# highfem/tqdne

Measured on AMD Instinct MI355X. Metric: waveforms/sec (train step + 18-step EDM sample), 3ch x 4096, higher is better.
Workload: dtype f32 (contractions on MFMA with fp32 accumulate: bf16x3, and fp16 + block-scaled-fp6 corrections on the 128/256-channel forward convs; sampler state f64)

## Files before the change

include/tqdne_hip.h:

```cpp
#ifndef TQDNE_HIP_H
#define TQDNE_HIP_H

#include <stddef.h>
#include <stdint.h>

#ifdef __cplusplus
extern "C" {
#endif

#ifndef __HIP__
typedef struct ihipStream_t* hipStream_t;
#endif

#define TQ_ABI_VERSION 8

#define TQ_ERR_ARG (-1)
#define TQ_ERR_SHAPE (-2)

#define TQ_CONV_GN 1
#define TQ_CONV_SILU 2
#define TQ_CONV_EMB 4
#define TQ_CONV_RES 8
#define TQ_CONV_STATS 16
#define TQ_CONV_DROPOUT 32
#define TQ_CONV_POLY2 64
#define TQ_CONV_CH_TILES 128
#define TQ_CONV_WIDE_TABLE 256

#define TQ_WFMT_BF16X3 0
#define TQ_WFMT_F16_MX8 1
#define TQ_WFMT_F16_MX6 2

typedef struct TqGnFold {
    const float* stats0;
    const float* stats1;
    int32_t slot0, slot1;
    const float* gamma;
    const float* beta;
    float* mean_rstd;
} TqGnFold;

typedef struct TqConvDesc {
    int32_t B, T_in, T_out;
    int32_t C_in0, C_in1;
    int32_t C_out;
    int32_t ktaps, stride, pad;
    int32_t upsample;
    int32_t flags;
    int32_t emb_stride;
    uint32_t dropout_site;
    float dropout_p;
    uint64_t dropout_seed;
    int32_t C_skip0, C_skip1;
    int32_t wfmt;
    int32_t* range_flag;
    const void* reserved1;
    int32_t t_tile;
    int32_t reserved2;
    const TqGnFold* gn_fold;
} TqConvDesc;

#define TQ_BWD_GN 1
#define TQ_BWD_SILU 2
#define TQ_BWD_DROPOUT 4
#define TQ_BWD_ACCUM 8
#define TQ_BWD_STATS 16

typedef struct TqConvBwdDesc {
    int32_t B, T;
    int32_t C_dy;
    int32_t C_dx0, C_dx1;
    int32_t ktaps;
    int32_t flags;
    uint32_t dropout_site;
    float dropout_p;
    uint64_t dropout_seed;
    int32_t wfmt;
    int32_t reserved;
    const uint32_t* dy_amax;
} TqConvBwdDesc;

int tq_abi_version(void);
int tq_build_flags(void);

size_t tq_conv_weight_pack_bytes(int C_out, int C_in, int K, int mode);
int tq_pack_conv_weight(const float* w, int C_out, int C_in, int K, int mode, void* packed, hipStream_t stream);
int tq_conv_tile_co(int C_out);
int tq_conv1d_max_cin(int wfmt, int C_out);
int tq_conv1d_max_cout(void);
size_t tq_conv1d_wide_lds_bytes(int ktaps, int t_tile, int C_out);
int tq_conv1d_gn_table_entries(int wide);
int tq_conv1d_gn_fold_max_cin(int wfmt, int t_tile, int C_out);
int tq_colsum_max_channels(void);
typedef struct TqPackJob {
    const void* src;
    void* dst;
    int32_t C_out, C_in, K, mode;
    int32_t block_begin;
    int32_t reserved;
} TqPackJob;
int tq_pack_job_blocks(int C_out, int C_in, int K, int mode);
int tq_pack_jobs(const TqPackJob* jobs_device, int njobs, int total_blocks, hipStream_t stream);

int tq_conv1d_fwd(const TqConvDesc* desc, const float* x0, const float* x1, const float* gscale, const float* gshift,
                  const void* packed_w, const float* bias, const float* emb, const float* residual, float* y,
                  float* stats_partial, hipStream_t stream);

int tq_conv1d_fwd_skip(const TqConvDesc* desc, const float* x0, const float* x1, const float* gscale, const float* gshift,
                       const void* packed_w_main_then_skip, const float* bias, const float* emb, const float* skip_x0,
                       const float* skip_x1, const float* skip_bias, float* y, float* stats_partial, hipStream_t stream);

#define TQ_KV_V_BF16 0
#define TQ_KV_V_F16 1
int tq_conv1d_fwd_qkv(const TqConvDesc* desc, const float* x, const float* gscale, const float* gshift, const void* packed_w,
                      const float* bias, float* qkv, void* kv_planes, int H, int D, int v_format, hipStream_t stream);

int tq_conv1d_bwd_data(const TqConvBwdDesc* desc, const float* dy, const void* packed_w_t, const float* x0, const float* x1,
                       const float* gscale, const float* gshift, float* dx0, float* dx1, float* gstats_partial,
                       hipStream_t stream);

size_t tq_conv1d_bwd_weight_workspace(const TqConvDesc* desc);
int tq_conv1d_bwd_weight(const TqConvDesc* desc, const float* dy, const float* x0, const float* x1, const float* gscale,
                         const float* gshift, float* dw, void* workspace, size_t ws_bytes, hipStream_t stream);
int tq_conv1d_bwd_weight_colsum(const TqConvDesc* desc, const float* dy, const float* x0, const float* x1, const float* gscale,
                                const float* gshift, float* dw, void* workspace, size_t ws_bytes, float* colsum_bc, int bc_stride,
                                float* colsum_c, float* colsum_c2, hipStream_t stream);

size_t tq_stem_conv_lds_bytes(int C_in, int C_out, int ktaps);
int tq_stem_conv_fwd(const float* x_nct, const float* in_scale, const float* w, const float* bias, float* y,
                     float* stats_partial, int B, int C_in, int T, int C_out, int ktaps, hipStream_t stream);

size_t tq_head_conv_lds_bytes(int C_in, int C_out, int ktaps);
int tq_head_conv_fwd(const float* x, const float* gscale, const float* gshift, const float* w, const float* bias,
                     const float* c_out, const float* c_skip, const float* skip_src, float* y_nct, int B, int T, int C_in,
                     int C_out, int ktaps, hipStream_t stream);

int tq_gn_finalize(const float* stats0, int C0, const float* stats1, int C1, int B, int T, const float* gamma,
                   const float* beta, float* gscale, float* gshift, float* mean_rstd, int slot0, int slot1, hipStream_t stream);

int tq_gn_bwd_finalize(const float* gstats_partial, const float* mean_rstd, const float* gamma, int B, int C, int T,
                       float* coef_a, float* coef_b, float* coef_c, float* dgamma, float* dbeta, hipStream_t stream);
int tq_gn_bwd_apply(const float* g, const float* x, const float* r, const float* coef_a, const float* coef_b,
                    const float* coef_c, float* dx, int B, int T, int C_src, int C_total, int c_offset, int accumulate,
                    hipStream_t stream);
int tq_gn_bwd_apply_colsum(const float* g, const float* x, const float* r, const float* coef_a, const float* coef_b,
                           const float* coef_c, float* dx, int B, int T, int C_src, int C_total, int c_offset, int accumulate,
                           float* colsum_bc, int bc_stride, float* colsum_c, float* colsum_c2, uint32_t* amax_out,
                           hipStream_t stream);
typedef struct TqGemmJob {
    const float* A;
    const float* B;
    float* C;
    const float* U;
    int32_t M, N, K;
    int32_t sam, sak, sbk, sbn, ldc, ldu;
    int32_t pre_b;
    int32_t tile_begin;
} TqGemmJob;
int tq_gemm_tiles(int M, int N);
int tq_gemm_f32_jobs(const TqGemmJob* jobs_device, int njobs, int total_tiles, hipStream_t stream);
int tq_fourier_features(const float* t, const float* W, float* out, int B, int half, hipStream_t stream);

#define TQ_AMAX_WAYS 16
#define TQ_AMAX_STRIDE 32
#define TQ_AMAX_WORDS (TQ_AMAX_WAYS * TQ_AMAX_STRIDE)
int tq_colsum(const float* dy, int B, int T, int C, float* out_bc, int bc_stride, float* out_c, float* out_c2,
              const float* bscale, uint32_t* amax_out, hipStream_t stream);
int tq_zero_stuff(const float* dy, float* out, int B, int T_out, int T_in, int C, hipStream_t stream);
int tq_pair_sum(const float* d_up, float* dx, int B, int T, int C, int accumulate, hipStream_t stream);
int tq_upsample_poly_wgrad_fold(const float* dw2, float* dw, int C_out, int C_in, hipStream_t stream);
int tq_stem_conv_bwd_weight(const float* dy, const float* x_nct, const float* in_scale, float* dw, int B, int C_in, int T,
                            int C_out, int ktaps, hipStream_t stream);
size_t tq_stem_head_bwd_workspace(void);
int tq_stem_conv_bwd_weight_ws(const float* dy, const float* x_nct, const float* in_scale, float* dw, int B, int C_in, int T,
                               int C_out, int ktaps, void* workspace, size_t ws_bytes, hipStream_t stream);
int tq_head_conv_bwd_ws(const float* dpred_nct, const float* c_out, const float* x, const float* gscale, const float* gshift,
                        const float* w, float* g_out, float* gstats_partial, float* dw, float* db, int B, int T, int C_in,
                        int C_out, int ktaps, void* workspace, size_t ws_bytes, hipStream_t stream);
size_t tq_head_conv_bwd_lds_bytes(int C_in, int C_out, int ktaps);
int tq_head_conv_bwd(const float* dpred_nct, const float* c_out, const float* x, const float* gscale, const float* gshift,
                     const float* w, float* g_out, float* gstats_partial, float* dw, float* db, int B, int T, int C_in,
                     int C_out, int ktaps, hipStream_t stream);

int tq_embed_fwd(const float* t, const float* cond, const float* fourier_w, const float* w0, const float* b0,
                 const float* w2, const float* b2, const float* cw0, const float* cb0, const float* cw2, const float* cb2,
                 float* emb, float* silu_emb, float* hidden ,
                 int B, int mc, int ncond, hipStream_t stream);

int tq_linear_fwd(const float* x, const float* w, const float* bias, float* out, int B, int E, int N, hipStream_t stream);

size_t tq_attention_workspace_bytes(int B, int T, int H, int D);
int tq_attention_fwd(const float* qkv, float* out, float* lse ,
                     void* workspace , int B, int T,
                     int H, int D, hipStream_t stream);
int tq_attention_fwd_presplit(const float* qkv, const void* kv_planes, float* out, int B, int T, int H, int D, int v_format,
                              hipStream_t stream);
int tq_attention_bwd(const float* qkv, const float* out, const float* dout, const float* lse, float* delta, float* dqkv, int B,
                     int T, int H, int D, hipStream_t stream);
int tq_attention_bwd_ws(const float* qkv, const float* out, const float* dout, const float* lse, float* delta, float* dqkv,
                        void* workspace, int B, int T, int H, int D, hipStream_t stream);
int tq_attention_bwd_ws_kv(const float* qkv, const float* out, const float* dout, const float* lse, float* delta, float* dqkv,
                           void* workspace, const void* kv_planes, int B, int T, int H, int D, hipStream_t stream);

int tq_attention_head_tile(int D);
size_t tq_attention_hd_lds_bytes(int D, int pass);
size_t tq_attention_hd_workspace_bytes(int B, int T, int H, int D);
int tq_attention_fwd_hd(const float* qkv, float* out, float* lse, void* workspace, int B, int T, int H, int D, hipStream_t stream);
int tq_attention_bwd_hd(const float* qkv, const float* out, const float* dout, const float* lse, float* delta, float* dqkv,
                        void* workspace, int B, int T, int H, int D, hipStream_t stream);

int tq_edm_scalars(const float* sigma, int sigma_stride, float sigma_data, float* c_in, float* c_out, float* c_skip,
                   float* c_noise, float* lweight, int B, hipStream_t stream);
int tq_cm_scalars(const float* sigma, int sigma_stride, float sigma_data, float sigma_min, float* c_out, float* c_skip,
                  int B, hipStream_t stream);
int tq_edm_noise_inject(const float* y, const float* unit_noise, const float* eps, float P_mean, float P_std,
                        float* sigma, float* x_noisy, int B, int n_per_sample, hipStream_t stream);
int tq_edm_loss(const float* pred, const float* y, const float* lweight, float* loss_out, float* dpred, int B,
                int n_per_sample, hipStream_t stream);
int tq_heun_euler(const double* x, const float* denoised, const float* sigma, const float* sigma_next, double* d_cur,
                  double* x_next, float* x32, size_t n, hipStream_t stream);
int tq_heun_correct(const double* x, const double* x_next, const float* denoised_next, const double* d_cur,
                    const float* sigma, const float* sigma_next, double* x_out, float* x32, size_t n, hipStream_t stream);
int tq_sampler_init(const double* unit_noise, const float* sigma0, double* x, float* x32, size_t n, hipStream_t stream);

int tq_heun_churn(const double* x, const double* unit_noise, const float* coef, double s_noise, double* x_hat, float* x32,
                  size_t n, hipStream_t stream);

int tq_axpy_sigma(const float* x, const float* noise, const float* sigma, float* out, int B, int n_per_sample,
                  hipStream_t stream);

int tq_scale_add2(const float* x, const float* y, const float* a, const float* c, float* out, int B, int n_per_sample,
// ... 51 lines not shown
```

tqdne_amd/_lib.py:

```python

from __future__ import annotations

import ctypes as C
import os
from typing import Optional

from . import _build

_LIB = None

c_f32p = C.c_void_p
VP = C.c_void_p
I = C.c_int
F = C.c_float
SZ = C.c_size_t

TQ_CONV_GN, TQ_CONV_SILU, TQ_CONV_EMB, TQ_CONV_RES, TQ_CONV_STATS, TQ_CONV_DROPOUT = 1, 2, 4, 8, 16, 32
TQ_CONV_POLY2 = 64
TQ_CONV_CH_TILES = 128
TQ_CONV_WIDE_TABLE = 256
TQ_WFMT_BF16X3, TQ_WFMT_F16_MX8, TQ_WFMT_F16_MX6 = 0, 1, 2
TQ_KV_V_BF16, TQ_KV_V_F16 = 0, 1
PACK_MODE = {TQ_WFMT_BF16X3: 0, TQ_WFMT_F16_MX8: 2, TQ_WFMT_F16_MX6: 3}
PACK_MODE_T = {TQ_WFMT_BF16X3: 1, TQ_WFMT_F16_MX6: 5}
# ... 22 lines not shown
WIDE_MX6 = os.environ.get("TQDNE_WIDE_MX6", "1") != "0"


def conv_max_cin(wfmt: int, C_out: int = 0) -> int:
    return load().tq_conv1d_max_cin(wfmt, C_out)


def forward_wfmt(C_out: int, sources, stride: int = 1, upsample: bool = False, k5_act: bool = False,
                 gn: Optional[bool] = None) -> int:
    v = requested_scheme()
    co_ok = C_out % 128 == 0 or (C_out % 64 == 0 and k5_act and not upsample and v == "f16mx6" and MX6_C64)
    ok = stride == 1 and co_ok and all(c % 64 == 0 for c in sources if c)
    if not ok or v == "bf16x3":
        return TQ_WFMT_BF16X3
    fmt = TQ_WFMT_F16_MX6 if v == "f16mx6" else TQ_WFMT_F16_MX8
    cin = sum(c for c in list(sources)[:2] if c)
    if gn is None or gn:
        if cin > conv_max_cin(fmt, C_out) or (cin > load().tq_conv1d_gn_table_entries(0) and not WIDE_MX6):
            return TQ_WFMT_BF16X3
    return fmt
TQ_BWD_GN, TQ_BWD_SILU, TQ_BWD_DROPOUT, TQ_BWD_ACCUM, TQ_BWD_STATS = 1, 2, 4, 8, 16
STAT_SLOT = 128
TQ_AMAX_WAYS, TQ_AMAX_STRIDE = 16, 32
TQ_AMAX_WORDS = TQ_AMAX_WAYS * TQ_AMAX_STRIDE


class TqGnFold(C.Structure):
    _fields_ = [("stats0", C.c_void_p), ("stats1", C.c_void_p), ("slot0", C.c_int32), ("slot1", C.c_int32),
                ("gamma", C.c_void_p), ("beta", C.c_void_p), ("mean_rstd", C.c_void_p)]


class TqConvDesc(C.Structure):
    _fields_ = [
        ("B", C.c_int32), ("T_in", C.c_int32), ("T_out", C.c_int32),
        ("C_in0", C.c_int32), ("C_in1", C.c_int32), ("C_out", C.c_int32),
        ("ktaps", C.c_int32), ("stride", C.c_int32), ("pad", C.c_int32),
        ("upsample", C.c_int32), ("flags", C.c_int32), ("emb_stride", C.c_int32),
        ("dropout_site", C.c_uint32), ("dropout_p", C.c_float), ("dropout_seed", C.c_uint64),
        ("C_skip0", C.c_int32), ("C_skip1", C.c_int32), ("wfmt", C.c_int32),
        ("range_flag", C.c_void_p), ("reserved1", C.c_void_p), ("t_tile", C.c_int32), ("reserved2", C.c_int32),
        ("gn_fold", C.POINTER(TqGnFold)),
    ]


class TqAdamChunk(C.Structure):
    _fields_ = [("p", C.c_void_p), ("g", C.c_void_p), ("m", C.c_void_p), ("v", C.c_void_p), ("ema", C.c_void_p),
                ("n", C.c_int32), ("reserved", C.c_int32)]


TQ_ADAM_CHUNK = 4096


class TqGemmJob(C.Structure):
    _fields_ = [("A", C.c_void_p), ("B", C.c_void_p), ("C", C.c_void_p), ("U", C.c_void_p),
                ("M", C.c_int32), ("N", C.c_int32), ("K", C.c_int32),
                ("sam", C.c_int32), ("sak", C.c_int32), ("sbk", C.c_int32), ("sbn", C.c_int32), ("ldc", C.c_int32), ("ldu", C.c_int32),
                ("pre_b", C.c_int32), ("tile_begin", C.c_int32)]


class TqPackJob(C.Structure):
    _fields_ = [("src", C.c_void_p), ("dst", C.c_void_p), ("C_out", C.c_int32), ("C_in", C.c_int32), ("K", C.c_int32),
                ("mode", C.c_int32), ("block_begin", C.c_int32), ("reserved", C.c_int32)]


class TqConvBwdDesc(C.Structure):
    _fields_ = [
        ("B", C.c_int32), ("T", C.c_int32), ("C_dy", C.c_int32), ("C_dx0", C.c_int32), ("C_dx1", C.c_int32),
        ("ktaps", C.c_int32), ("flags", C.c_int32), ("dropout_site", C.c_uint32), ("dropout_p", C.c_float),
        ("dropout_seed", C.c_uint64), ("wfmt", C.c_int32), ("reserved", C.c_int32), ("dy_amax", C.c_void_p),
    ]


_PROTOS = {
    "tq_abi_version": (I, []),
    "tq_build_flags": (I, []),
    "tq_conv_weight_pack_bytes": (SZ, [I, I, I, I]),
    "tq_pack_conv_weight": (I, [VP, I, I, I, I, VP, VP]),
    "tq_conv_tile_co": (I, [I]),
    "tq_conv1d_max_cin": (I, [I, I]),
    "tq_conv1d_max_cout": (I, []),
    "tq_conv1d_gn_table_entries": (I, [I]),
    "tq_conv1d_wide_lds_bytes": (SZ, [I, I, I]),
    "tq_conv1d_gn_fold_max_cin": (I, [I, I, I]),
    "tq_colsum_max_channels": (I, []),
    "tq_conv1d_fwd": (I, [C.POINTER(TqConvDesc)] + [VP] * 11),
    "tq_conv1d_fwd_skip": (I, [C.POINTER(TqConvDesc)] + [VP] * 13),
    "tq_stem_conv_fwd": (I, [VP] * 6 + [I] * 5 + [VP]),
    "tq_head_conv_fwd": (I, [VP] * 9 + [I] * 5 + [VP]),
    "tq_head_conv_lds_bytes": (SZ, [I, I, I]),
    "tq_stem_conv_lds_bytes": (SZ, [I, I, I]),
    "tq_head_conv_bwd_lds_bytes": (SZ, [I, I, I]),
    "tq_gn_finalize": (I, [VP, I, VP, I, I, I, VP, VP, VP, VP, VP, I, I, VP]),
    "tq_embed_fwd": (I, [VP] * 14 + [I, I, I, VP]),
    "tq_linear_fwd": (I, [VP] * 4 + [I, I, I, VP]),
    "tq_attention_fwd": (I, [VP, VP, VP, VP, I, I, I, I, VP]),
    "tq_attention_fwd_presplit": (I, [VP, VP, VP, I, I, I, I, I, VP]),
    "tq_conv1d_fwd_qkv": (I, [C.POINTER(TqConvDesc)] + [VP] * 7 + [I, I, I, VP]),
    "tq_attention_workspace_bytes": (SZ, [I, I, I, I]),
    "tq_attention_bwd": (I, [VP] * 6 + [I, I, I, I, VP]),
    "tq_attention_bwd_ws": (I, [VP] * 7 + [I, I, I, I, VP]),
    "tq_attention_bwd_ws_kv": (I, [VP] * 8 + [I, I, I, I, VP]),
    "tq_attention_head_tile": (I, [I]),
    "tq_attention_hd_lds_bytes": (SZ, [I, I]),
    "tq_attention_hd_workspace_bytes": (SZ, [I, I, I, I]),
    "tq_attention_fwd_hd": (I, [VP, VP, VP, VP, I, I, I, I, VP]),
    "tq_attention_bwd_hd": (I, [VP] * 7 + [I, I, I, I, VP]),
    "tq_edm_scalars": (I, [VP, I, F, VP, VP, VP, VP, VP, I, VP]),
    "tq_cm_scalars": (I, [VP, I, F, F, VP, VP, I, VP]),
    "tq_edm_noise_inject": (I, [VP, VP, VP, F, F, VP, VP, I, I, VP]),
    "tq_edm_loss": (I, [VP, VP, VP, VP, VP, I, I, VP]),
    "tq_heun_euler": (I, [VP] * 7 + [SZ, VP]),
    "tq_heun_correct": (I, [VP] * 8 + [SZ, VP]),
    "tq_sampler_init": (I, [VP] * 4 + [SZ, VP]),
    "tq_heun_churn": (I, [VP, VP, VP, C.c_double, VP, VP, SZ, VP]),
    "tq_axpy_sigma": (I, [VP, VP, VP, VP, I, I, VP]),
    "tq_pseudo_huber_loss": (I, [VP, VP, VP, F, VP, VP, I, I, VP]),
    "tq_mse_loss": (I, [VP, VP, VP, VP, SZ, VP]),
    "tq_scale_add2": (I, [VP, VP, VP, VP, VP, I, I, VP]),
    "tq_ddpm_step": (I, [VP, VP, VP, VP, SZ, I] + [C.c_double] * 6 + [VP]),
    "tq_vae_reparam_fwd": (I, [VP, VP, VP, VP, I, I, I, VP]),
    "tq_vae_reparam_bwd": (I, [VP, VP, VP, VP, F, I, I, I, VP]),
    "tq_concat_scale": (I, [VP, VP, VP, VP, I, I, I, I, VP]),
    "tq_envelope_fwd": (I, [VP, VP, I, I, I, I, C.c_double, C.c_double, VP]),
    "tq_envelope_inv": (I, [VP, VP, I, I, I, C.c_double, C.c_double, VP]),
    "tq_adam_ema_step": (I, [VP, I] + [C.c_double] * 8 + [VP]),
    "tq_adam_ema_step_guarded": (I, [VP, I] + [C.c_double] * 8 + [VP, VP]),
    "tq_conv1d_bwd_data": (I, [VP] * 11),
    "tq_conv1d_bwd_weight_workspace": (SZ, [VP]),
    "tq_conv1d_bwd_weight": (I, [VP] * 8 + [SZ, VP]),
    "tq_conv1d_bwd_weight_colsum": (I, [VP] * 8 + [SZ, VP, I, VP, VP, VP]),
    "tq_gn_bwd_finalize": (I, [VP, VP, VP, I, I, I, VP, VP, VP, VP, VP, VP]),
    "tq_gn_bwd_apply": (I, [VP] * 7 + [I] * 6 + [VP]),
    "tq_gn_bwd_apply_colsum": (I, [VP] * 7 + [I] * 6 + [VP, I, VP, VP, VP, VP]),
    "tq_pack_job_blocks": (I, [I, I, I, I]),
    "tq_pack_jobs": (I, [VP, I, I, VP]),
    "tq_gemm_tiles": (I, [I, I]),
    "tq_gemm_f32_jobs": (I, [VP, I, I, VP]),
    "tq_fourier_features": (I, [VP, VP, VP, I, I, VP]),
    "tq_colsum": (I, [VP, I, I, I, VP, I, VP, VP, VP, VP, VP]),
    "tq_zero_stuff": (I, [VP, VP, I, I, I, I, VP]),
    "tq_pair_sum": (I, [VP, VP, I, I, I, I, VP]),
    "tq_upsample_poly_wgrad_fold": (I, [VP, VP, I, I, VP]),
    "tq_stem_conv_bwd_weight": (I, [VP] * 4 + [I] * 5 + [VP]),
    "tq_head_conv_bwd": (I, [VP] * 10 + [I] * 5 + [VP]),
    "tq_stem_head_bwd_workspace": (SZ, []),
    "tq_stem_conv_bwd_weight_ws": (I, [VP] * 4 + [I] * 5 + [VP, SZ, VP]),
    "tq_head_conv_bwd_ws": (I, [VP] * 10 + [I] * 5 + [VP, SZ, VP]),
    "tq_boundary_max_channels": (I, []),
    "tq_nct_to_btc": (I, [VP] * 4 + [I] * 5 + [VP]),
    "tq_btc_to_nct": (I, [VP] * 5 + [I] * 5 + [VP]),
    "tq_avg_pool2_fwd": (I, [VP, VP, VP, I, I, I, VP]),
    "tq_nearest_up2_fwd": (I, [VP, VP, VP, I, I, I, VP]),
    "tq_avg_pool2_bwd": (I, [VP, VP, I, I, I, I, VP]),
}

def lib_path() -> str:
    return os.environ.get("TQDNE_HIP_LIB", _build.LIBPATH)


def load():
    global _LIB
    if _LIB is not None:
        return _LIB
    path = lib_path()
    if not os.path.exists(path):
        raise RuntimeError(
            f"{path} is missing: the tqdne_amd hot path is HIP-only (no CPU / PyTorch fallback). "
            "Build it with `python -m tqdne_amd._build` (needs hipcc, cross-compiles gfx950 without a GPU)."
        )
    lib = C.CDLL(path)
    for name, (res, args) in _PROTOS.items():
        fn = getattr(lib, name)
        fn.restype = res
        fn.argtypes = args
    if lib.tq_abi_version() != ABI_VERSION:
        raise RuntimeError("libtqdne_hip.so ABI version mismatch")
    _LIB = lib
    return lib


def exported_symbols():
    return sorted(_PROTOS)


class TqError(RuntimeError):
    pass


def check(rc: int, what: str = ""):
    if rc != 0:
        kind = {-1: "TQ_ERR_ARG", -2: "TQ_ERR_SHAPE"}.get(rc, f"hipError_t {rc}")
        raise TqError(f"libtqdne_hip: {what} failed with {kind}")
```

tqdne_amd/csrc/backward.hip:

```cpp
#include <cstdlib>
#include "common.hpp"
#include "ends_wide.hpp"
#include "../../include/tqdne_hip.h"

using namespace tq;

namespace {

typedef short s16x4 __attribute__((ext_vector_type(4)));

__device__ __forceinline__ uint2 lds_tr_read(const unsigned char* p) {
    s16x4 v = __builtin_amdgcn_ds_read_tr16_b64_v4i16((__attribute__((address_space(3))) s16x4*)(p));
    union { s16x4 s; uint2 u; } c;
    c.s = v;
    return c.u;
}

struct WgArgs {
    const float* dy;
    const float* x0;
    const float* x1;
    const float* gscale;
    const float* gshift;
    float* slab;
    int B, T_in, T_out, C0, C1, C_out;
    int flags, nsplit, units_per_split, n_ttiles, n_cotiles, n_cichunks;
    uint32_t drop_site, drop_thresh;
    float drop_scale;
    uint64_t drop_seed;
    float* cs_bc;
    int cs_stride;
    float* cs_c;
    float* cs_c2;
};

constexpr int WG_TT = 64;
constexpr int TQ_WGRAD_PLAIN_ORDER = 1 << 30;
constexpr int WG_DY_STRIDE1 = 288;
constexpr int WG_DY_STRIDE2 = 272;
template <int NCI> __device__ __forceinline__ int wg_dy_swz(int row) { return (NCI == 1 || NCI == 4) ? ((row >> 3) & 1) << 7 : 0; }
__device__ __forceinline__ int wg_x_swz(int row) { return ((row >> 3) & 1) << 5; }
__device__ __forceinline__ int wg_x_swz128(int row) { return (((row >> 1) & 1) << 5) | (((row >> 3) & 1) << 6); }
__device__ __forceinline__ int wg_x_swz256(int row) { return ((row & 3) << 5) | (((row >> 3) & 1) << 7); }

template <int KT, int STRIDE, int UPS, int NCI, bool W8 = false, bool H64 = false>
__global__ __launch_bounds__((W8 && !H64) ? 512 : 256, (W8 && !H64) ? 1 : 2) void wgrad_kernel(const WgArgs p) {
    static_assert(!W8 || NCI == 1, "W8: per-wave accumulators of a 32-channel chunk");
    static_assert(!H64 || W8, "H64: the W8 layout (two 32-channel halves of one xhat tile) with two output-channel blocks");
    constexpr int NT = (W8 && !H64) ? 512 : 256;
    constexpr int COT = H64 ? 64 : 128;
    constexpr int DYC4 = COT / 4;
    constexpr int NCX = W8 ? 2 : NCI;
    constexpr int PAD = (STRIDE == 1) ? KT / 2 : 1;
    constexpr int XR = (STRIDE == 1) ? (WG_TT + KT - 1) : (2 * WG_TT + 1);
    constexpr int WG_X_STRIDE = 64 * NCX;
    constexpr int XC4 = 8 * NCX;
    constexpr int XIT = (XR * XC4 + NT - 1) / NT;
    constexpr int DYIT = WG_TT * DYC4 / NT;
    static_assert(NCI != 4 || (KT == 1 && STRIDE == 1 && !UPS), "128-channel chunks: the 1x1 convs");
    constexpr int WG_DY_STRIDE = (NCI == 1 || NCI == 4) ? WG_DY_STRIDE1 : WG_DY_STRIDE2;
    constexpr int DY_PLANE = WG_TT * WG_DY_STRIDE;
    constexpr int X_PLANE = XR * WG_X_STRIDE;
    extern __shared__ __attribute__((aligned(16))) unsigned char lds[];
    unsigned char* dy_hi = lds;
    unsigned char* dy_lo = dy_hi + DY_PLANE;
    unsigned char* x_hi = dy_lo + DY_PLANE;
    unsigned char* x_lo = x_hi + X_PLANE;

    const int tid = threadIdx.x, lane = tid & 63;
    const int wave_id = __builtin_amdgcn_readfirstlane(tid >> 6);
    const int wave = H64 ? (wave_id & 1) : (W8 ? (wave_id & 3) : wave_id);
    const int wci = H64 ? (wave_id >> 1) : (W8 ? (wave_id >> 2) : 0);
    int ct, cc, sp;
    {
        const int bid = blockIdx.x;
        const int npairs = p.nsplit * p.n_cotiles;
        if ((npairs & 7) == 0 && !(p.flags & TQ_WGRAD_PLAIN_ORDER)) {
            const int xcd = bid & 7, j = bid >> 3;
            const int pi = (j / p.n_cichunks) * 8 + xcd;
            cc = j % p.n_cichunks;
            sp = pi / p.n_cotiles;
            ct = pi % p.n_cotiles;
        } else {
            ct = bid % p.n_cotiles;
// ... 433 lines not shown
    } else {
        hipLaunchKernelGGL((wgrad_kernel<KT, STRIDE, UPS, 1, false>), dim3(grid), dim3(256), sh, stream, a);
    }
    TQ_CHECK_LAUNCH();
    return 0;
}
}

extern "C" size_t tq_conv1d_bwd_weight_workspace(const TqConvDesc* d) {
    if (!d) return 0;
    int a, b, c, nsplit, nsplit4, ups;
    wgrad_plan(d, true, a, b, c, nsplit, ups);
    wgrad_plan(d, false, a, b, c, nsplit4, ups);
    return (size_t)(nsplit > nsplit4 ? nsplit : nsplit4) * d->ktaps * d->C_out * (d->C_in0 + d->C_in1) * sizeof(float);
}

extern "C" int tq_conv1d_bwd_weight(const TqConvDesc* d, const float* dy, const float* x0, const float* x1,
                                    const float* gscale, const float* gshift, float* dw, void* workspace, size_t ws_bytes,
                                    hipStream_t stream) {
    return tq_conv1d_bwd_weight_colsum(d, dy, x0, x1, gscale, gshift, dw, workspace, ws_bytes, nullptr, 0, nullptr, nullptr, stream);
}

extern "C" int tq_conv1d_bwd_weight_colsum(const TqConvDesc* d, const float* dy, const float* x0, const float* x1,
                                           const float* gscale, const float* gshift, float* dw, void* workspace, size_t ws_bytes,
                                           float* colsum_bc, int bc_stride, float* colsum_c, float* colsum_c2,
                                           hipStream_t stream) {
    if (!d || !dy || !x0 || !dw || !workspace) return TQ_ERR_ARG;
    if (colsum_c2 && !colsum_c) return TQ_ERR_ARG;
    if (d->C_in0 <= 0 || d->C_in0 % 32 || d->C_in1 < 0 || d->C_in1 % 32 || d->C_out <= 0 || d->C_out % 32) return TQ_ERR_SHAPE;
    if (d->C_in1 > 0 && !x1) return TQ_ERR_ARG;
    if ((d->flags & TQ_CONV_GN) && (!gscale || !gshift)) return TQ_ERR_ARG;
    if (ws_bytes < tq_conv1d_bwd_weight_workspace(d)) return TQ_ERR_ARG;
    WgArgs a;
    a.dy = dy; a.x0 = x0; a.x1 = x1; a.gscale = gscale; a.gshift = gshift; a.slab = reinterpret_cast<float*>(workspace);
    a.B = d->B; a.T_in = d->T_in; a.T_out = d->T_out; a.C0 = d->C_in0; a.C1 = d->C_in1; a.C_out = d->C_out;
    a.flags = d->flags;
    a.cs_bc = colsum_bc; a.cs_stride = bc_stride; a.cs_c = colsum_c; a.cs_c2 = colsum_c2;
    const bool wide = !(colsum_bc || colsum_c);
    wgrad_plan(d, wide, a.n_cotiles, a.n_cichunks, a.n_ttiles, a.nsplit, a.units_per_split);
    static const bool plain_order = [] { const char* e = getenv("TQDNE_WGRAD_XCD"); return e && atoi(e) == 0; }();
    if (plain_order) a.flags |= TQ_WGRAD_PLAIN_ORDER;
    a.drop_site = d->dropout_site; a.drop_seed = d->dropout_seed;
    float pdrop = d->dropout_p;
    if (!(d->flags & TQ_CONV_DROPOUT) || pdrop <= 0.f) { a.flags &= ~TQ_CONV_DROPOUT; pdrop = 0.f; }
    a.drop_thresh = (uint32_t)((double)pdrop * 4294967296.0);
    a.drop_scale = 1.0f / (1.0f - pdrop);
    int rc;
    const int nci = wgrad_nci(d);
    const bool h64 = wide && wgrad_h64(d);
    const bool w8 = wide && !h64 && wgrad_w8(d);
    if (d->stride == 2) {
        if (d->ktaps != 3) return TQ_ERR_SHAPE;
        rc = launch_wgrad<3, 2, 0>(a, nci, w8, false, stream);
    } else if (d->upsample) {
        if (d->ktaps == 5) rc = launch_wgrad<5, 1, 1>(a, nci, w8, false, stream);
        else if (d->ktaps == 3) rc = launch_wgrad<3, 1, 1>(a, nci, w8, false, stream);
        else return TQ_ERR_SHAPE;
    } else {
        if (d->ktaps == 5) rc = launch_wgrad<5, 1, 0>(a, nci, w8, h64, stream);
        else if (d->ktaps == 3) rc = launch_wgrad<3, 1, 0>(a, nci, w8, h64, stream);
        else if (d->ktaps == 1) rc = launch_wgrad<1, 1, 0>(a, nci, false, false, stream);
        else return TQ_ERR_SHAPE;
    }
    if (rc) return rc;
    const size_t n = (size_t)d->C_out * (d->C_in0 + d->C_in1);
    const dim3 rgrid((unsigned)((n + 63) / 64)), rblock(16, 16);
    if (d->ktaps == 5) hipLaunchKernelGGL(wgrad_reduce_kernel<5>, rgrid, rblock, 0, stream, a.slab, dw, a.nsplit, n);
    else if (d->ktaps == 3) hipLaunchKernelGGL(wgrad_reduce_kernel<3>, rgrid, rblock, 0, stream, a.slab, dw, a.nsplit, n);
    else hipLaunchKernelGGL(wgrad_reduce_kernel<1>, rgrid, rblock, 0, stream, a.slab, dw, a.nsplit, n);
    TQ_CHECK_LAUNCH();
    return 0;
}

namespace {
__global__ __launch_bounds__(256) void gn_bwd_finalize_kernel(const float* __restrict__ gst, const float* __restrict__ mr,
                                                              const float* __restrict__ gamma, int C, int T, int nslots,
                                                              float* __restrict__ cA, float* __restrict__ cB,
                                                              float* __restrict__ cC, float* __restrict__ dgamma,
                                                              float* __restrict__ dbeta) {
    extern __shared__ double sh[];
    const int b = blockIdx.x;
    const int Cb = C / (int)gridDim.y;
    const int c0 = (int)blockIdx.y * Cb;
    int nsub = Cb <= 128 ? (int)blockDim.x / Cb : 1;
    if (nsub > nslots) nsub = nslots;
    double* cs = sh;
    double* gp = sh + 2 * Cb * nsub;
    for (int idx = threadIdx.x; idx < Cb * nsub; idx += blockDim.x) {
        const int c = idx % Cb, sub = idx / Cb;
        const float* pp = gst + ((size_t)b * nslots * C + c0 + c) * 2;
        double s1 = 0.0, s2 = 0.0;
        int s = sub;
        for (; s + 3 * nsub < nslots; s += 4 * nsub) {
            const float2 v0 = *reinterpret_cast<const float2*>(pp + (size_t)s * C * 2);
            const float2 v1 = *reinterpret_cast<const float2*>(pp + (size_t)(s + nsub) * C * 2);
            const float2 v2 = *reinterpret_cast<const float2*>(pp + (size_t)(s + 2 * nsub) * C * 2);
            const float2 v3 = *reinterpret_cast<const float2*>(pp + (size_t)(s + 3 * nsub) * C * 2);
            s1 += ((double)v0.x + (double)v1.x) + ((double)v2.x + (double)v3.x);
            s2 += ((double)v0.y + (double)v1.y) + ((double)v2.y + (double)v3.y);
        }
        for (; s < nslots; s += nsub) {
            const float2 v = *reinterpret_cast<const float2*>(pp + (size_t)s * C * 2);
            s1 += (double)v.x; s2 += (double)v.y;
        }
        cs[2 * idx] = s1; cs[2 * idx + 1] = s2;
    }
    __syncthreads();
    if (nsub > 1) {
        double t1 = 0.0, t2 = 0.0;
        const int c = threadIdx.x;
        if (c < Cb)
            for (int sub = 0; sub < nsub; ++sub) { t1 += cs[2 * (sub * Cb + c)]; t2 += cs[2 * (sub * Cb + c) + 1]; }
        __syncthreads();
        if (c < Cb) { cs[2 * c] = t1; cs[2 * c + 1] = t2; }
        __syncthreads();
    }
    const int G = C / GN_GROUPS;
    const int ngrp = Cb / G, g0 = c0 / G;
    if ((int)threadIdx.x < ngrp) {
        const int gl = threadIdx.x, g = g0 + gl;
        const double mean = (double)mr[((size_t)b * GN_GROUPS + g) * 2], rstd = (double)mr[((size_t)b * GN_GROUPS + g) * 2 + 1];
        double p1 = 0.0, p2 = 0.0;
        for (int j = 0; j < G; ++j) {
            const int cl = gl * G + j;
            const double gm = (double)gamma[c0 + cl];
            p1 += gm * cs[2 * cl];
            p2 += gm * (cs[2 * cl + 1] - mean * cs[2 * cl]);
        }
        p2 *= rstd;
        const double n = (double)G * (double)T;
        gp[2 * gl] = -rstd * rstd * p2 / n;
        gp[2 * gl + 1] = rstd * rstd * p2 * mean / n - rstd * p1 / n;
    }
    __syncthreads();
    for (int cl = threadIdx.x; cl < Cb; cl += blockDim.x) {
        const int c = c0 + cl;
        const int g = c / G, gl = g - g0;
        const float mean = mr[((size_t)b * GN_GROUPS + g) * 2], rstd = mr[((size_t)b * GN_GROUPS + g) * 2 + 1];
        cA[(size_t)b * C + c] = rstd * gamma[c];
        cB[(size_t)b * C + c] = (float)gp[2 * gl];
        cC[(size_t)b * C + c] = (float)gp[2 * gl + 1];
        atomicAdd(dgamma + c, (float)((double)rstd * (cs[2 * cl + 1] - (double)mean * cs[2 * cl])));
        atomicAdd(dbeta + c, (float)cs[2 * cl]);
    }
}

__global__ void gn_bwd_apply_kernel(const float* __restrict__ g, const float* __restrict__ x, const float* __restrict__ r,
                                    const float* __restrict__ cA, const float* __restrict__ cB, const float* __restrict__ cC,
                                    float* __restrict__ dx, int T, int Cs, int Ctot, int coff, int accum, size_t n4) {
    const int c4n = Cs >> 2;
    for (size_t i = (size_t)blockIdx.x * blockDim.x + threadIdx.x; i < n4; i += (size_t)gridDim.x * blockDim.x) {
        const int c4 = (int)(i % c4n);
        const size_t bt = i / c4n;
        const int b = (int)(bt / T);
        const size_t ko = (size_t)b * Ctot + coff + 4 * c4;
        const float4 a = *reinterpret_cast<const float4*>(cA + ko);
        const float4 bb = *reinterpret_cast<const float4*>(cB + ko);
        const float4 cc = *reinterpret_cast<const float4*>(cC + ko);
        const float4 gv = reinterpret_cast<const float4*>(g)[i];
        const float4 xv = reinterpret_cast<const float4*>(x)[i];
        float4 o = make_float4(a.x * gv.x + bb.x * xv.x + cc.x, a.y * gv.y + bb.y * xv.y + cc.y,
                               a.z * gv.z + bb.z * xv.z + cc.z, a.w * gv.w + bb.w * xv.w + cc.w);
        if (r) { const float4 rv = reinterpret_cast<const float4*>(r)[i]; o.x += rv.x; o.y += rv.y; o.z += rv.z; o.w += rv.w; }
        if (accum) { const float4 ov = reinterpret_cast<const float4*>(dx)[i]; o.x += ov.x; o.y += ov.y; o.z += ov.z; o.w += ov.w; }
        reinterpret_cast<float4*>(dx)[i] = o;
    }
}

constexpr int AMAX_WAYS = TQ_AMAX_WAYS;
constexpr int AMAX_STRIDE = TQ_AMAX_STRIDE;

template <int NT>
__device__ __forceinline__ void colsum_finish(float* red, const float4& a, float mx, bool active, int c4n, int nrow, int c4, int tr, int C,
                                              int b, float sc, float* __restrict__ out_bc, int bc_stride, float* __restrict__ out_c,
                                              float* __restrict__ out_c2, unsigned* __restrict__ amax_out) {
    if (active) *reinterpret_cast<float4*>(red + (tr * c4n + c4) * 4) = a;
    unsigned* wmax = reinterpret_cast<unsigned*>(red + (size_t)nrow * c4n * 4);
    if (amax_out) {
        unsigned m = __float_as_uint(mx);
#pragma unroll
        for (int o = 32; o > 0; o >>= 1) m = max(m, (unsigned)__shfl_xor((int)m, o));
        if ((threadIdx.x & 63) == 0) wmax[threadIdx.x >> 6] = m;
    }
    __syncthreads();
    if (amax_out && threadIdx.x == 0) {
        unsigned m = wmax[0];
#pragma unroll
        for (int w = 1; w < NT / 64; ++w) m = max(m, wmax[w]);
        if (m != 0u) atomicMax(amax_out + (blockIdx.x % AMAX_WAYS) * AMAX_STRIDE, m);
    }
    for (int c = threadIdx.x; c < C; c += NT) {
        float s = 0.f;
        for (int r2 = 0; r2 < nrow; ++r2) s += red[(r2 * c4n + (c >> 2)) * 4 + (c & 3)];
        s *= sc;
        if (out_bc) atomicAdd(out_bc + (size_t)b * bc_stride + c, s);
        if (out_c) atomicAdd(out_c + c, s);
        if (out_c2) atomicAdd(out_c2 + c, s);
    }
}
__device__ __forceinline__ float amax4(float m, const float4& v) {
    const float t = fmaxf(fmaxf(fabsf(v.x), fabsf(v.y)), fmaxf(fabsf(v.z), fabsf(v.w)));
    const bool bad = (v.x != v.x) | (v.y != v.y) | (v.z != v.z) | (v.w != v.w);
    return bad ? __builtin_inff() : fmaxf(m, t);
}

template <int NT>
__global__ __launch_bounds__(NT) void colsum_kernel(const float* __restrict__ dy, int T, int C, float* __restrict__ out_bc,
                                                     int bc_stride, float* __restrict__ out_c, float* __restrict__ out_c2,
                                                     const float* __restrict__ bscale, unsigned* __restrict__ amax_out, int rpw) {
    extern __shared__ float red[];
    const int nsl = (T + rpw - 1) / rpw;
    const int slot = blockIdx.x % nsl, b = blockIdx.x / nsl;
    const int c4n = C >> 2;
    const int nrow = NT / c4n > 0 ? NT / c4n : 1;
    const int c4 = threadIdx.x % c4n, tr = threadIdx.x / c4n;
    float4 a = make_float4(0.f, 0.f, 0.f, 0.f);
    float mx = 0.f;
    const bool active = tr < nrow && threadIdx.x < nrow * c4n;
    if (active) {
        const int nvalid = min(rpw, T - slot * rpw);
        const float* src = dy + ((size_t)b * T + (size_t)slot * rpw) * C + 4 * c4;
        int tl = tr;
        for (; tl + 7 * nrow < nvalid; tl += 8 * nrow) {
            float4 v[8];
#pragma unroll
            for (int q = 0; q < 8; ++q) v[q] = *reinterpret_cast<const float4*>(src + (size_t)(tl + q * nrow) * C);
#pragma unroll
            for (int q = 0; q < 8; ++q) { a.x += v[q].x; a.y += v[q].y; a.z += v[q].z; a.w += v[q].w; }
            if (amax_out) {
#pragma unroll
                for (int q = 0; q < 8; ++q) mx = amax4(mx, v[q]);
            }
        }
        for (; tl < nvalid; tl += nrow) {
            const float4 v = *reinterpret_cast<const float4*>(src + (size_t)tl * C);
            a.x += v.x; a.y += v.y; a.z += v.z; a.w += v.w;
            if (amax_out) mx = amax4(mx, v);
        }
    }
    colsum_finish<NT>(red, a, mx, active, c4n, nrow, c4, tr, C, b, bscale ? bscale[b] : 1.0f, out_bc, bc_stride, out_c, out_c2, amax_out);
}

template <int NT>
__global__ __launch_bounds__(NT) void gn_bwd_apply_cs_kernel(const float* __restrict__ g, const float* __restrict__ x,
                                                              const float* __restrict__ r, const float* __restrict__ cA,
                                                              const float* __restrict__ cB, const float* __restrict__ cC,
                                                              float* __restrict__ dx, int T, int Cs, int Ctot, int coff, int accum,
                                                              float* __restrict__ out_bc, int bc_stride, float* __restrict__ out_c,
                                                              float* __restrict__ out_c2, unsigned* __restrict__ amax_out, int rpw) {
    extern __shared__ float red[];
    const int nsl = (T + rpw - 1) / rpw;
    const int slot = blockIdx.x % nsl, b = blockIdx.x / nsl;
    const int c4n = Cs >> 2;
    const int nrow = NT / c4n > 0 ? NT / c4n : 1;
    const int c4 = threadIdx.x % c4n, tr = threadIdx.x / c4n;
    float4 a = make_float4(0.f, 0.f, 0.f, 0.f);
    float mx = 0.f;
    const bool active = tr < nrow && threadIdx.x < nrow * c4n;
    if (active) {
        const int nvalid = min(rpw, T - slot * rpw);
        const size_t ko = (size_t)b * Ctot + coff + 4 * c4;
        const float4 ka = *reinterpret_cast<const float4*>(cA + ko);
        const float4 kb = *reinterpret_cast<const float4*>(cB + ko);
        const float4 kc = *reinterpret_cast<const float4*>(cC + ko);
        const size_t base = ((size_t)b * T + (size_t)slot * rpw) * Cs + 4 * c4;
        auto one = [&](const float4& gv, const float4& xv, const float4& rv, const float4& ov) -> float4 __attribute__((always_inline)) {
            float4 o = make_float4(ka.x * gv.x + kb.x * xv.x + kc.x, ka.y * gv.y + kb.y * xv.y + kc.y,
                                   ka.z * gv.z + kb.z * xv.z + kc.z, ka.w * gv.w + kb.w * xv.w + kc.w);
            o.x += rv.x; o.y += rv.y; o.z += rv.z; o.w += rv.w;
            o.x += ov.x; o.y += ov.y; o.z += ov.z; o.w += ov.w;
            return o;
        };
        const float4 z4 = make_float4(0.f, 0.f, 0.f, 0.f);
        int tl = tr;
        for (; tl + 3 * nrow < nvalid; tl += 4 * nrow) {
            float4 gv[4], xv[4], rv[4], ov[4];
#pragma unroll
            for (int q = 0; q < 4; ++q) {
                const size_t o = base + (size_t)(tl + q * nrow) * Cs;
                gv[q] = *reinterpret_cast<const float4*>(g + o);
                xv[q] = *reinterpret_cast<const float4*>(x + o);
                rv[q] = r ? *reinterpret_cast<const float4*>(r + o) : z4;
                ov[q] = accum ? *reinterpret_cast<const float4*>(dx + o) : z4;
            }
#pragma unroll
            for (int q = 0; q < 4; ++q) {
                const float4 o4 = one(gv[q], xv[q], rv[q], ov[q]);
                *reinterpret_cast<float4*>(dx + base + (size_t)(tl + q * nrow) * Cs) = o4;
                a.x += o4.x; a.y += o4.y; a.z += o4.z; a.w += o4.w;
                mx = amax4(mx, o4);
            }
        }
        for (; tl < nvalid; tl += nrow) {
            const size_t o = base + (size_t)tl * Cs;
            const float4 o4 = one(*reinterpret_cast<const float4*>(g + o), *reinterpret_cast<const float4*>(x + o),
                                  r ? *reinterpret_cast<const float4*>(r + o) : z4, accum ? *reinterpret_cast<const float4*>(dx + o) : z4);
            *reinterpret_cast<float4*>(dx + o) = o4;
            a.x += o4.x; a.y += o4.y; a.z += o4.z; a.w += o4.w;
            mx = amax4(mx, o4);
        }
    }
    colsum_finish<NT>(red, a, mx, active, c4n, nrow, c4, tr, Cs, b, 1.0f, out_bc, bc_stride, out_c, out_c2, amax_out);
}

struct CsChunk { int c0, cw; };
__device__ __forceinline__ CsChunk cs_chunk(int C, int cw) {
    const int c0 = (int)blockIdx.y * cw;
    return CsChunk{c0, min(cw, C - c0)};
}

template <int NT>
__global__ __launch_bounds__(NT) void colsum_chunk_kernel(const float* __restrict__ dy, int T, int C, int cw, float* __restrict__ out_bc,
                                                           int bc_stride, float* __restrict__ out_c, float* __restrict__ out_c2,
                                                           const float* __restrict__ bscale, unsigned* __restrict__ amax_out, int rpw) {
    extern __shared__ float red[];
    const CsChunk ck = cs_chunk(C, cw);
    const int nsl = (T + rpw - 1) / rpw;
    const int slot = blockIdx.x % nsl, b = blockIdx.x / nsl;
    const int c4n = ck.cw >> 2;
    const int nrow = NT / c4n > 0 ? NT / c4n : 1;
    const int c4 = threadIdx.x % c4n, tr = threadIdx.x / c4n;
    float4 a = make_float4(0.f, 0.f, 0.f, 0.f);
    float mx = 0.f;
    const bool active = tr < nrow && threadIdx.x < nrow * c4n;
    if (active) {
        const int nvalid = min(rpw, T - slot * rpw);
        const float* src = dy + ((size_t)b * T + (size_t)slot * rpw) * C + ck.c0 + 4 * c4;
        int tl = tr;
        for (; tl + 7 * nrow < nvalid; tl += 8 * nrow) {
            float4 v[8];
#pragma unroll
            for (int q = 0; q < 8; ++q) v[q] = *reinterpret_cast<const float4*>(src + (size_t)(tl + q * nrow) * C);
#pragma unroll
            for (int q = 0; q < 8; ++q) { a.x += v[q].x; a.y += v[q].y; a.z += v[q].z; a.w += v[q].w; }
            if (amax_out) {
#pragma unroll
                for (int q = 0; q < 8; ++q) mx = amax4(mx, v[q]);
            }
        }
        for (; tl < nvalid; tl += nrow) {
            const float4 v = *reinterpret_cast<const float4*>(src + (size_t)tl * C);
            a.x += v.x; a.y += v.y; a.z += v.z; a.w += v.w;
            if (amax_out) mx = amax4(mx, v);
        }
    }
    colsum_finish<NT>(red, a, mx, active, c4n, nrow, c4, tr, ck.cw, b, bscale ? bscale[b] : 1.0f, out_bc ? out_bc + ck.c0 : nullptr, bc_stride,
                      out_c ? out_c + ck.c0 : nullptr, out_c2 ? out_c2 + ck.c0 : nullptr, amax_out);
}

template <int NT>
__global__ __launch_bounds__(NT) void gn_bwd_apply_cs_chunk_kernel(const float* __restrict__ g, const float* __restrict__ x,
                                                                    const float* __restrict__ r, const float* __restrict__ cA,
                                                                    const float* __restrict__ cB, const float* __restrict__ cC,
                                                                    float* __restrict__ dx, int T, int Cs, int cw, int Ctot, int coff, int accum,
                                                                    float* __restrict__ out_bc, int bc_stride, float* __restrict__ out_c,
                                                                    float* __restrict__ out_c2, unsigned* __restrict__ amax_out, int rpw) {
    extern __shared__ float red[];
    const CsChunk ck = cs_chunk(Cs, cw);
    const int nsl = (T + rpw - 1) / rpw;
    const int slot = blockIdx.x % nsl, b = blockIdx.x / nsl;
    const int c4n = ck.cw >> 2;
    const int nrow = NT / c4n > 0 ? NT / c4n : 1;
    const int c4 = threadIdx.x % c4n, tr = threadIdx.x / c4n;
    float4 a = make_float4(0.f, 0.f, 0.f, 0.f);
    float mx = 0.f;
    const bool active = tr < nrow && threadIdx.x < nrow * c4n;
    if (active) {
        const int nvalid = min(rpw, T - slot * rpw);
        const size_t ko = (size_t)b * Ctot + coff + ck.c0 + 4 * c4;
        const float4 ka = *reinterpret_cast<const float4*>(cA + ko);
        const float4 kb = *reinterpret_cast<const float4*>(cB + ko);
        const float4 kc = *reinterpret_cast<const float4*>(cC + ko);
        const size_t base = ((size_t)b * T + (size_t)slot * rpw) * Cs + ck.c0 + 4 * c4;
        const float4 z4 = make_float4(0.f, 0.f, 0.f, 0.f);
        for (int tl = tr; tl < nvalid; tl += nrow) {
            const size_t o = base + (size_t)tl * Cs;
            const float4 gv = *reinterpret_cast<const float4*>(g + o), xv = *reinterpret_cast<const float4*>(x + o);
            const float4 rv = r ? *reinterpret_cast<const float4*>(r + o) : z4, ov = accum ? *reinterpret_cast<const float4*>(dx + o) : z4;
            float4 o4 = make_float4(ka.x * gv.x + kb.x * xv.x + kc.x, ka.y * gv.y + kb.y * xv.y + kc.y,
                                    ka.z * gv.z + kb.z * xv.z + kc.z, ka.w * gv.w + kb.w * xv.w + kc.w);
            o4.x += rv.x; o4.y += rv.y; o4.z += rv.z; o4.w += rv.w;
            o4.x += ov.x; o4.y += ov.y; o4.z += ov.z; o4.w += ov.w;
            *reinterpret_cast<float4*>(dx + o) = o4;
            a.x += o4.x; a.y += o4.y; a.z += o4.z; a.w += o4.w;
            mx = amax4(mx, o4);
        }
    }
    colsum_finish<NT>(red, a, mx, active, c4n, nrow, c4, tr, ck.cw, b, 1.0f, out_bc ? out_bc + ck.c0 : nullptr, bc_stride,
                      out_c ? out_c + ck.c0 : nullptr, out_c2 ? out_c2 + ck.c0 : nullptr, amax_out);
}


__global__ void zero_stuff_kernel(const float* __restrict__ dy, float* __restrict__ out, int T_out, int T_in, int C, size_t n4) {
    const int c4n = C >> 2;
    for (size_t i = (size_t)blockIdx.x * blockDim.x + threadIdx.x; i < n4; i += (size_t)gridDim.x * blockDim.x) {
        const int c4 = (int)(i % c4n);
        const size_t bu = i / c4n;
        const int u = (int)(bu % T_in);
        const size_t b = bu / T_in;
        float4 v = make_float4(0.f, 0.f, 0.f, 0.f);
        if (!(u & 1) && (u >> 1) < T_out) v = reinterpret_cast<const float4*>(dy)[(b * T_out + (u >> 1)) * c4n + c4];
        reinterpret_cast<float4*>(out)[i] = v;
    }
}

__global__ void pair_sum_kernel(const float* __restrict__ dup, float* __restrict__ dx, int T, int C, int accum, size_t n4) {
    const int c4n = C >> 2;
    for (size_t i = (size_t)blockIdx.x * blockDim.x + threadIdx.x; i < n4; i += (size_t)gridDim.x * blockDim.x) {
        const int c4 = (int)(i % c4n);
        const size_t bt = i / c4n;
        const int t = (int)(bt % T);
        const size_t b = bt / T;
        const float4 a = reinterpret_cast<const float4*>(dup)[(b * 2 * T + 2 * t) * c4n + c4];
        const float4 c = reinterpret_cast<const float4*>(dup)[(b * 2 * T + 2 * t + 1) * c4n + c4];
        float4 o = make_float4(a.x + c.x, a.y + c.y, a.z + c.z, a.w + c.w);
        if (accum) { const float4 ov = reinterpret_cast<const float4*>(dx)[i]; o.x += ov.x; o.y += ov.y; o.z += ov.z; o.w += ov.w; }
        reinterpret_cast<float4*>(dx)[i] = o;
    }
}

inline unsigned ew_grid4(size_t n4) {
    size_t g = (n4 + 255) / 256;
    return (unsigned)(g > 4096 ? 4096 : (g ? g : 1));
}
}

extern "C" int tq_gn_bwd_finalize(const float* gstats, const float* mean_rstd, const float* gamma, int B, int C, int T,
                                  float* coef_a, float* coef_b, float* coef_c, float* dgamma, float* dbeta,
                                  hipStream_t stream) {
    if (!gstats || !mean_rstd || !gamma || !coef_a || !coef_b || !coef_c || !dgamma || !dbeta) return TQ_ERR_ARG;
    if (B <= 0 || T <= 0 || C <= 0 || C % GN_GROUPS) return TQ_ERR_SHAPE;
    const int nslots = (T + STAT_SLOT - 1) / STAT_SLOT;
    const int NP = 4;
    const int Cb = C / NP;
    int nsub = Cb <= 128 ? 256 / Cb : 1;
    if (nsub > nslots) nsub = nslots;
    const size_t sh = (size_t)(2 * Cb * nsub + 2 * GN_GROUPS) * sizeof(double);
    hipLaunchKernelGGL(gn_bwd_finalize_kernel, dim3(B, NP), dim3(256), sh, stream, gstats, mean_rstd, gamma, C, T, nslots, coef_a,
                       coef_b, coef_c, dgamma, dbeta);
    TQ_CHECK_LAUNCH();
    return 0;
}

extern "C" int tq_gn_bwd_apply(const float* g, const float* x, const float* r, const float* coef_a, const float* coef_b,
                               const float* coef_c, float* dx, int B, int T, int C_src, int C_total, int c_offset, int accumulate,
                               hipStream_t stream) {
    if (!g || !x || !coef_a || !coef_b || !coef_c || !dx) return TQ_ERR_ARG;
    if (B <= 0 || T <= 0 || C_src <= 0 || C_src % 4 || c_offset % 4 || c_offset + C_src > C_total) return TQ_ERR_SHAPE;
    const size_t n4 = (size_t)B * T * (C_src / 4);
    hipLaunchKernelGGL(gn_bwd_apply_kernel, dim3(ew_grid4(n4)), dim3(256), 0, stream, g, x, r, coef_a, coef_b, coef_c, dx, T,
                       C_src, C_total, c_offset, accumulate, n4);
    TQ_CHECK_LAUNCH();
    return 0;
}

constexpr int CS_NT = 256;
struct CsTiling { int rows; };
static CsTiling colsum_tiling(int B, int T) {
    CsTiling t;
    const size_t min_wgs = 256;
    int rpw = STAT_SLOT;
    while (rpw < 4096 && (size_t)B * ((T + 2 * rpw - 1) / (2 * rpw)) >= min_wgs) rpw <<= 1;
    t.rows = rpw;
    return t;
}

constexpr int CS_CHUNK = 1024;
constexpr int CS_MAX_C = CS_CHUNK * 64;
static int colsum_chunk_width(int C, int& nchunks) {
    const int c4 = C / 4;
    nchunks = (c4 + CS_CHUNK / 4 - 1) / (CS_CHUNK / 4);
    return ((c4 + nchunks - 1) / nchunks) * 4;
}
extern "C" int tq_colsum_max_channels(void) { return CS_MAX_C; }

extern "C" int tq_colsum(const float* dy, int B, int T, int C, float* out_bc, int bc_stride, float* out_c, float* out_c2,
                         const float* bscale, uint32_t* amax_out, hipStream_t stream) {
    if (!dy || (!out_bc && !out_c && !out_c2 && !amax_out)) return TQ_ERR_ARG;
    if (B <= 0 || T <= 0 || C < 4 || C % 4 || C > CS_MAX_C) return TQ_ERR_SHAPE;
    const CsTiling tl = colsum_tiling(B, T);
    const int nsl = (T + tl.rows - 1) / tl.rows;
    if (C > CS_CHUNK) {
        int nch;
        const int cw = colsum_chunk_width(C, nch);
        const size_t shw = (size_t)(CS_NT > cw / 4 ? CS_NT : cw / 4) * 4 * sizeof(float) + (CS_NT / 64) * sizeof(unsigned);
        hipLaunchKernelGGL(colsum_chunk_kernel<CS_NT>, dim3(B * nsl, nch), dim3(CS_NT), shw, stream, dy, T, C, cw, out_bc, bc_stride, out_c, out_c2, bscale, amax_out, tl.rows);
        TQ_CHECK_LAUNCH();
        return 0;
    }
    const int c4n = C / 4;
    const int nrow = CS_NT / c4n > 0 ? CS_NT / c4n : 1;
    const size_t sh = (size_t)nrow * c4n * 4 * sizeof(float) + (CS_NT / 64) * sizeof(unsigned);
    hipLaunchKernelGGL(colsum_kernel<CS_NT>, dim3(B * nsl), dim3(CS_NT), sh, stream, dy, T, C, out_bc, bc_stride, out_c, out_c2, bscale, amax_out, tl.rows);
    TQ_CHECK_LAUNCH();
    return 0;
}

extern "C" int tq_gn_bwd_apply_colsum(const float* g, const float* x, const float* r, const float* coef_a, const float* coef_b,
                                      const float* coef_c, float* dx, int B, int T, int C_src, int C_total, int c_offset, int accumulate,
                                      float* colsum_bc, int bc_stride, float* colsum_c, float* colsum_c2, uint32_t* amax_out,
                                      hipStream_t stream) {
    if (!g || !x || !coef_a || !coef_b || !coef_c || !dx) return TQ_ERR_ARG;
    if (colsum_c2 && !colsum_c) return TQ_ERR_ARG;
    if (B <= 0 || T <= 0 || C_src <= 0 || C_src % 4 || C_src > CS_MAX_C || c_offset % 4 || c_offset + C_src > C_total) return TQ_ERR_SHAPE;
    if (!colsum_bc && !colsum_c && !amax_out)
        return tq_gn_bwd_apply(g, x, r, coef_a, coef_b, coef_c, dx, B, T, C_src, C_total, c_offset, accumulate, stream);
    const CsTiling tl = colsum_tiling(B, T);
    const int nsl = (T + tl.rows - 1) / tl.rows;
    if (C_src > CS_CHUNK) {
        int nch;
        const int cw = colsum_chunk_width(C_src, nch);
        const size_t shw = (size_t)(CS_NT > cw / 4 ? CS_NT : cw / 4) * 4 * sizeof(float) + (CS_NT / 64) * sizeof(unsigned);
        hipLaunchKernelGGL(gn_bwd_apply_cs_chunk_kernel<CS_NT>, dim3(B * nsl, nch), dim3(CS_NT), shw, stream, g, x, r, coef_a, coef_b, coef_c, dx, T,
                           C_src, cw, C_total, c_offset, accumulate, colsum_bc, bc_stride, colsum_c, colsum_c2, amax_out, tl.rows);
        TQ_CHECK_LAUNCH();
        return 0;
    }
    const int c4n = C_src / 4;
    const int nrow = CS_NT / c4n > 0 ? CS_NT / c4n : 1;
    const size_t sh = (size_t)nrow * c4n * 4 * sizeof(float) + (CS_NT / 64) * sizeof(unsigned);
    hipLaunchKernelGGL(gn_bwd_apply_cs_kernel<CS_NT>, dim3(B * nsl), dim3(CS_NT), sh, stream, g, x, r, coef_a, coef_b, coef_c, dx, T, C_src,
                       C_total, c_offset, accumulate, colsum_bc, bc_stride, colsum_c, colsum_c2, amax_out, tl.rows);
    TQ_CHECK_LAUNCH();
    return 0;
}

extern "C" int tq_zero_stuff(const float* dy, float* out, int B, int T_out, int T_in, int C, hipStream_t stream) {
    if (!dy || !out || B <= 0 || T_out <= 0 || T_in <= 0 || C % 4) return TQ_ERR_ARG;
    const size_t n4 = (size_t)B * T_in * (C / 4);
    hipLaunchKernelGGL(zero_stuff_kernel, dim3(ew_grid4(n4)), dim3(256), 0, stream, dy, out, T_out, T_in, C, n4);
    TQ_CHECK_LAUNCH();
    return 0;
}

extern "C" int tq_pair_sum(const float* d_up, float* dx, int B, int T, int C, int accumulate, hipStream_t stream) {
    if (!d_up || !dx || B <= 0 || T <= 0 || C % 4) return TQ_ERR_ARG;
    const size_t n4 = (size_t)B * T * (C / 4);
    hipLaunchKernelGGL(pair_sum_kernel, dim3(ew_grid4(n4)), dim3(256), 0, stream, d_up, dx, T, C, accumulate, n4);
    TQ_CHECK_LAUNCH();
    return 0;
}

namespace {
__global__ __launch_bounds__(256) void poly_wgrad_fold_kernel(const float* __restrict__ dw2, float* __restrict__ dw, int n) {
    const int i = blockIdx.x * 256 + threadIdx.x;
    if (i >= n) return;
    const float* a = dw2 + (size_t)i * 3;
    const float* b = dw2 + ((size_t)n + i) * 3;
    const float a0 = a[0], a1 = a[1], a2 = a[2], b0 = b[0], b1 = b[1], b2 = b[2];
    float* o = dw + (size_t)i * 5;
    o[0] = a0 + b0; o[1] = a0 + b1; o[2] = a1 + b1; o[3] = a1 + b2; o[4] = a2 + b2;
}
}

extern "C" int tq_upsample_poly_wgrad_fold(const float* dw2, float* dw, int C_out, int C_in, hipStream_t stream) {
    if (!dw2 || !dw || C_out <= 0 || C_in <= 0) return TQ_ERR_ARG;
    const int n = C_out * C_in;
    hipLaunchKernelGGL(poly_wgrad_fold_kernel, dim3((unsigned)((n + 255) / 256)), dim3(256), 0, stream, dw2, dw, n);
    TQ_CHECK_LAUNCH();
    return 0;
}

namespace {
template <int KT, int CI>
__global__ __launch_bounds__(256) void stem_wgrad_stream_kernel(const float* __restrict__ dy, const float* __restrict__ x,
                                                                const float* __restrict__ in_scale, float* __restrict__ dw,
                                                                float* __restrict__ part, int C_in, int T, int C_out, int nslots,
                                                                int nunits, int upw) {
    extern __shared__ float shm[];
    constexpr int PAD = KT / 2, TW = STAT_SLOT + KT - 1, BLK = 16;
    float* xs = shm;
    float* red = xs + CI * TW;
    const int nseg = 256 / C_out, L = STAT_SLOT / nseg;
    const int co = threadIdx.x % C_out, seg = threadIdx.x / C_out;
    float acc[CI][KT];
#pragma unroll
    for (int ci = 0; ci < CI; ++ci)
#pragma unroll
        for (int k = 0; k < KT; ++k) acc[ci][k] = 0.f;
    const int u0 = blockIdx.x * upw, u1 = min(nunits, u0 + upw);
    for (int u = u0; u < u1; ++u) {
        const int slot = u % nslots, b = u / nslots;
        const int t0 = slot * STAT_SLOT;
        const float sc = in_scale ? in_scale[b] : 1.0f;
        __syncthreads();
        for (int i = threadIdx.x; i < C_in * TW; i += 256) {
            const int c = i / TW, j = i % TW;
            const int t = t0 - PAD + j;
            xs[c * TW + j] = (t >= 0 && t < T) ? x[((size_t)b * C_in + c) * T + t] * sc : 0.f;
        }
        __syncthreads();
        const int tb = t0 + seg * L;
        for (int tl = 0; tl < L; tl += BLK) {
            float d[BLK];
#pragma unroll
            for (int j = 0; j < BLK; ++j) {
                const int tj = tb + tl + j;
                const int tc = tj < T ? tj : T - 1;
                d[j] = dy[((size_t)b * T + tc) * C_out + co] * (tj < T ? 1.f : 0.f);
            }
#pragma unroll
            for (int ci = 0; ci < CI; ++ci) {
                if (ci < C_in) {
                    float xw[BLK + KT - 1];
#pragma unroll
// ... 521 lines not shown
```

tqdne_amd/csrc/conv1d_fwd_wide.hip:

```cpp
#include "conv1d_kernel.hpp"

namespace {
template <int KT, int ACT, bool FUSE>
int dispatch_wide(const ConvArgs& a, hipStream_t s) {
    if (a.wfmt != TQ_WFMT_F16_MX6 || (a.flags & TQ_CONV_POLY2)) return TQ_ERR_SHAPE;
    if (a.C0 % 64 || a.C1 % 64 || a.sC0 % 64 || a.sC1 % 64 || a.C_out % 128) return TQ_ERR_SHAPE;
    if (a.t_tile == 32) {
        if constexpr (KT == 5 && ACT >= 2) return launch<KT, 1, 0, 4, 1, 0, ACT, FUSE, 2, false, 2, 2, CONV_GTAB_WIDE>(a, s);
        return TQ_ERR_SHAPE;
    }
    if (a.C_out % 256 == 0) return launch<KT, 1, 0, 8, 1, 0, ACT, FUSE, 2, false, 8, 2, CONV_GTAB_WIDE>(a, s);
    return launch<KT, 1, 0, 4, 1, 0, ACT, FUSE, 2, false, 8, 2, CONV_GTAB_WIDE>(a, s);
}
}

namespace tq {
int conv_launch_fwd_wide_k5(const ConvArgs& a, int act, bool fuse, hipStream_t s) {
    if (fuse) {
        if (act == 3) return dispatch_wide<5, 3, true>(a, s);
        if (act == 2) return dispatch_wide<5, 2, true>(a, s);
        return TQ_ERR_SHAPE;
    }
    if (act == 3) return dispatch_wide<5, 3, false>(a, s);
    if (act == 2) return dispatch_wide<5, 2, false>(a, s);
    if (act == 1) return dispatch_wide<5, 1, false>(a, s);
    return TQ_ERR_SHAPE;
}

int conv_launch_fwd_wide(const ConvArgs& a, int ktaps, int act, bool fuse, hipStream_t s) {
    if (ktaps == 5) return conv_launch_fwd_wide_k5(a, act, fuse, s);
    if (fuse) return TQ_ERR_SHAPE;
    return conv_launch_fwd_wide_k13(a, ktaps, act, s);
}
}

extern "C" int tq_conv1d_max_cin(int wfmt, int C_out) {
    if (C_out < 0 || C_out % 32) return 0;
    switch (wfmt) {
        case TQ_WFMT_F16_MX6:
            return (C_out % 128 == 0) ? CONV_GTAB_WIDE : (C_out % 64 == 0 ? CONV_GTAB_NARROW : 0);
        case TQ_WFMT_F16_MX8: return (C_out % 128 == 0) ? CONV_GTAB_NARROW : 0;
        case TQ_WFMT_BF16X3: return CONV_GTAB_WIDE;
        default: return 0;
    }
}

template <int KT>
static size_t wide_lds(int t_tile, int C_out) {
    if (C_out <= 0 || C_out % 128) return 0;
    if (t_tile == 32) return KT == 5 ? (size_t)ConvLds<KT, 1, 0, 4, 1, 0, 2, 2, false, 2, 2, CONV_GTAB_WIDE>::BYTES : 0;
    if (t_tile) return 0;
    return C_out % 256 == 0 ? (size_t)ConvLds<KT, 1, 0, 8, 1, 0, 2, 2, false, 8, 2, CONV_GTAB_WIDE>::BYTES
                            : (size_t)ConvLds<KT, 1, 0, 4, 1, 0, 2, 2, false, 8, 2, CONV_GTAB_WIDE>::BYTES;
}
extern "C" size_t tq_conv1d_wide_lds_bytes(int ktaps, int t_tile, int C_out) {
    return ktaps == 5 ? wide_lds<5>(t_tile, C_out) : ktaps == 3 ? wide_lds<3>(t_tile, C_out) : ktaps == 1 ? wide_lds<1>(t_tile, C_out) : 0;
}

extern "C" int tq_conv1d_gn_table_entries(int wide) { return wide ? CONV_GTAB_WIDE : CONV_GTAB_NARROW; }

extern "C" int tq_conv1d_max_cout(void) { return 3 * CONV_GTAB_NARROW; }

extern "C" int tq_conv1d_gn_fold_max_cin(int wfmt, int t_tile, int C_out) {
    if (C_out <= 0 || C_out % 32) return 0;
    int lim = 0;
    if (t_tile == 32) {
        if (wfmt == TQ_WFMT_F16_MX6) lim = C_out % 128 ? 0 : ConvLds<5, 1, 0, 4, 1, 0, 2, 2, false, 2, 2, 1024>::FOLD_MAX_CIN;
        else if (wfmt != TQ_WFMT_BF16X3) lim = 0;
        else if (C_out % 128 == 0) lim = ConvLds<5, 1, 0, 4, 1, 0, 2, 0, false, 2, 2, 1024>::FOLD_MAX_CIN;
        else if (C_out % 64 == 0) lim = ConvLds<5, 1, 0, 2, 1, 0, 2, 0, false, 2, 2, 1024>::FOLD_MAX_CIN;
        else lim = ConvLds<5, 1, 0, 1, 1, 0, 2, 0, false, 2, 2, 1024>::FOLD_MAX_CIN;
    } else if (t_tile == 0 && wfmt == TQ_WFMT_F16_MX6) {
        if (C_out % 256 == 0) lim = ConvLds<5, 1, 0, 8, 1, 0, 2, 2, false, 8, 2, 1024>::FOLD_MAX_CIN;
        else if (C_out % 128 == 0) lim = ConvLds<5, 1, 0, 4, 1, 0, 2, 2, false, 8, 2, 1024>::FOLD_MAX_CIN;
    }
    return lim / 32 * 32;
}
```

tqdne_amd/csrc/conv1d_kernel.hpp:

```cpp
#pragma once
#include <cmath>
#include <cstdlib>
#include <type_traits>

#include "common.hpp"
#include "conv_args.hpp"
#include "gn_fold.hpp"
#include <atomic>
#include "../../include/tqdne_hip.h"

using namespace tq;

#ifdef TQ_STAMP
static __device__ unsigned long long tq_stamps[12];
#ifdef TQ_STAMP_OWNER
extern "C" int tq_debug_read_stamps(unsigned long long* out, int reset) {
    hipError_t e = hipMemcpyFromSymbol(out, HIP_SYMBOL(tq_stamps), sizeof(unsigned long long) * 12);
    if (e != hipSuccess) return (int)e;
    if (reset) {
        unsigned long long z[12] = {0, 0, 0, 0, 0, 0, 0, 0, 0, 0, 0, 0};
        e = hipMemcpyToSymbol(HIP_SYMBOL(tq_stamps), z, sizeof(z));
    }
    return (int)e;
}
// ... 485 lines not shown
#pragma unroll
            for (int cbk = 0; cbk < 2; ++cbk)
                acc[cbk][tb] = __builtin_amdgcn_mfma_f32_16x16x32_f16(__builtin_bit_cast(f16x8, w[cbk * 4 + 1].u), b1v, acc[cbk][tb], 0, 0, 0);
#pragma unroll
            for (int cbk = 0; cbk < 2; ++cbk) {
                const Frag& c0 = w[cbk * 4 + 2];
                const Frag& c1 = w[cbk * 4 + 3];
                const i32x8 ac = {(int)c0.u.x, (int)c0.u.y, (int)c0.u.z, (int)c0.u.w, (int)c1.u.x, (int)c1.u.y, (int)c1.u.z, (int)c1.u.w};
#ifdef TQ_ABL_FP6TIME
                acc[cbk][tb] = __builtin_amdgcn_mfma_scale_f32_16x16x128_f8f6f4(ac, bc, acc[cbk][tb], 2, 2, 0, 127, 0, 115);
#else
                acc[cbk][tb] = __builtin_amdgcn_mfma_scale_f32_16x16x128_f8f6f4(ac, bc, acc[cbk][tb], 0, 0, 0, 127, 0, 115);
#endif
            }
        }
    };

#ifndef TQ_LDS_DEPTH
#define TQ_LDS_DEPTH 2
#endif
#ifndef TQ_LDS_DEPTH1
#define TQ_LDS_DEPTH1 1
#endif
    Frag wa[C::NW], wb[C::NW];
#ifndef TQ_LDS_DEPTH2
#define TQ_LDS_DEPTH2 1
#endif
    constexpr int LDS_DEP = SCH == 2 ? TQ_LDS_DEPTH2 : (SCH ? TQ_LDS_DEPTH1 : TQ_LDS_DEPTH);

    auto mma_stream = [&](const unsigned char* hi_plane, const unsigned char* lo_plane, int s0, auto ntaps_c, auto first_tap_c)
        __attribute__((always_inline)) {
        constexpr int NTAPS = decltype(ntaps_c)::value, K0 = decltype(first_tap_c)::value;
        constexpr int DEP = LDS_DEP, NB = LDS_DEP + 1, NS = NTAPS * TBW;
        Frag bf[NB][C::NBF];
        int b0 = tap_base(K0), b0n = b0;
#pragma unroll
        for (int t = 0; t < DEP; ++t) read_b(hi_plane, lo_plane, b0, t, bf[t]);
#pragma unroll
        for (int st = 0; st < NS; ++st) {
            const int kk = st / TBW, tb = st % TBW;
            if (tb == 0 && kk + 1 < NTAPS) b0n = tap_base(K0 + kk + 1);
            const int sn = st + DEP;
            if (sn < NS) read_b(hi_plane, lo_plane, (sn / TBW) == kk ? b0 : b0n, sn % TBW, bf[sn % NB]);
            __builtin_amdgcn_sched_barrier(0);
            if (kk & 1) mma_step(wb, bf[st % NB], tb); else mma_step(wa, bf[st % NB], tb);
            __builtin_amdgcn_sched_barrier(0);
            if (tb == TBW - 1) {
                const int nxt = (NTAPS == 1) ? (s0 + 1) : ((kk + 2 < NTAPS) ? (s0 + kk + 2) : ((kk & 1) ? (s0 + NTAPS + 1) : (s0 + NTAPS)));
                if (kk & 1) load_w(nxt, wb); else load_w(nxt, wa);
                b0 = b0n;
                __builtin_amdgcn_sched_barrier(0);
            }
        }
    };

    auto compute = [&](int chunk, int buf) __attribute__((always_inline)) {
        const unsigned char* hi_plane = lds + buf * C::BUF;
        mma_stream(hi_plane, hi_plane + C::PLANE, chunk * KT, std::integral_constant<int, KT>{}, std::integral_constant<int, 0>{});
    };

    auto compute_skip = [&](int j, int buf) __attribute__((always_inline)) {
        const unsigned char* hi_plane = lds + buf * C::BUF;
        const unsigned char* lo_plane = hi_plane + C::PLANE;
        constexpr int DEP = LDS_DEP, NB = LDS_DEP + 1;
        Frag bf[NB][C::NBF];
        const int b0 = tap_base(C::PAD);
#pragma unroll
        for (int t = 0; t < DEP; ++t) read_b(hi_plane, lo_plane, b0, t, bf[t]);
#pragma unroll
        for (int tb = 0; tb < TBW; ++tb) {
            if (tb + DEP < TBW) read_b(hi_plane, lo_plane, b0, tb + DEP, bf[(tb + DEP) % NB]);
            __builtin_amdgcn_sched_barrier(0);
            mma_step(wa, bf[tb % NB], tb);
            __builtin_amdgcn_sched_barrier(0);
        }
#pragma unroll
        for (int q = 0; q < C::NW; ++q) wa[q] = wb[q];
        load_w(nchunks * KT + j + 2, wb);
        __builtin_amdgcn_sched_barrier(0);
    };

    static_assert(!(SCH == 2 && ACT >= 1) || C::NTHR >= 256, "one table entry per thread");
    constexpr int GT_N = GTW / 1024;
    constexpr bool FOLD_LATE = SCH == 2 && ACT >= 1 && !PW && EPI == 0 && (TBW == 8 || TBW == 2);
    const bool fold_late = FOLD_LATE && p.cf_st0 != nullptr;
    float4 gt_a = make_float4(0.f, 0.f, 0.f, 0.f), gt_s = gt_a;
    int gt_i = 0;
    if constexpr (SCH == 2 && ACT >= 1) {
        const int n4 = Cin >> 2;
        gt_i = tid < n4 ? tid : n4 - 1;
        if (!fold_late) {
            gt_a = reinterpret_cast<const float4*>(p.gscale + (size_t)b * Cin)[gt_i];
            gt_s = reinterpret_cast<const float4*>(p.gshift + (size_t)b * Cin)[gt_i];
        }
    }
    float4 gt_a2 = make_float4(0.f, 0.f, 0.f, 0.f), gt_s2 = gt_a2;
    int gt_i2 = 0;
    if constexpr (SCH == 2 && ACT >= 1 && GT_N == 2) {
        static_assert(GT_N == 1 || 2 * C::NTHR * 4 >= GTW, "two table entries per thread cover the wide table");
        const int n4 = Cin >> 2;
        gt_i2 = tid + C::NTHR < n4 ? tid + C::NTHR : n4 - 1;
        gt_a2 = reinterpret_cast<const float4*>(p.gscale + (size_t)b * Cin)[gt_i2];
        gt_s2 = reinterpret_cast<const float4*>(p.gshift + (size_t)b * Cin)[gt_i2];
    }
    auto gtab_store = [&]() __attribute__((always_inline)) {
        if constexpr (SCH == 2 && ACT >= 1) {
            if constexpr (FOLD_LATE) {
                if (fold_late) {
                    gn_fold_sample<false, false>(reinterpret_cast<double*>(lds), b, p.cf_st0, p.C0, p.cf_st1, p.C1, p.T_in, p.cf_ns0, p.cf_ns1,
                                                 p.cf_gamma, p.cf_beta, const_cast<float*>(p.gscale), const_cast<float*>(p.gshift), p.cf_mean_rstd,
                                                 gtab, gtab + Cin);
                    __syncthreads();
                    return;
                }
            }
            float4* g4 = reinterpret_cast<float4*>(gtab);
            g4[gt_i] = gt_a;
            g4[(Cin >> 2) + gt_i] = gt_s;
            if constexpr (GT_N == 2) {
                g4[gt_i2] = gt_a2;
                g4[(Cin >> 2) + gt_i2] = gt_s2;
            }
            __syncthreads();
        }
    };
    if constexpr (PW) gtab_store();
    const int npass = PW ? n_ctiles : 1;
    if constexpr (PW) {
        static_assert(!PW || SCH == 2 || C::NIT == C::PRE, "PW stages a chunk in PRE iterations");
        static_assert(!PW || SCH != 2 || (C::NFULL == 1 && C::HALO_TASKS == 0), "PW, scheme 2: one 16-channel task per thread and chunk");
        if constexpr (SCH == 2) {
            float4 rr2[4][4];
#pragma unroll
            for (int c = 0; c < 4; ++c) {
                int cs2;
                const float* base2 = chunk_base2(c < nchunks ? c : nchunks - 1, cs2);
                load16(base2, cs2, tid >> 2, rr2[c]);
            }
            load_w(0, wa);
            load_w(1, wb);
#pragma unroll
            for (int c = 0; c < 4; ++c) write16(c < nchunks ? c : nchunks - 1, c, tid >> 2, rr2[c]);
            __syncthreads();
        } else {
        float4 rr[4][C::PRE], ga4[4], gs4[4];
#pragma unroll
        for (int c = 0; c < 4; ++c) {
            const int cc = c < nchunks ? c : nchunks - 1;
            int cs;
            const float* base = chunk_base(cc, cs);
#pragma unroll
            for (int it = 0; it < C::PRE; ++it) rr[c][it] = load_one(base, cs, it);
            if (ACT >= 1) {
                ga4[c] = *reinterpret_cast<const float4*>(p.gscale + (size_t)b * Cin + cc * C::CH + 4 * m);
                gs4[c] = *reinterpret_cast<const float4*>(p.gshift + (size_t)b * Cin + cc * C::CH + 4 * m);
            }
        }
        load_w(0, wa);
        load_w(1, wb);
#pragma unroll
        for (int c = 0; c < 4; ++c) {
            if (ACT >= 1) { g_a = ga4[c]; g_s = gs4[c]; }
#pragma unroll
            for (int it = 0; it < C::PRE; ++it) write_one(c < nchunks ? c : nchunks - 1, c, it, rr[c][it]);
        }
        __syncthreads();
        }
    }
    int pass = 0;
next_pass:
    if constexpr (PW) {
#pragma unroll
        for (int i = 0; i < 2; ++i)
#pragma unroll
            for (int j = 0; j < 8; ++j) acc[i][j] = f32x4{0.f, 0.f, 0.f, 0.f};
        for (int j = 0; 2 * j < nchunks; ++j) {
            pw_c0 = 2 * j;
            mma_stream(lds, lds + C::PLANE, 2 * j, std::integral_constant<int, 2>{}, std::integral_constant<int, 0>{});
        }
        if (pass + 1 < npass) wbase += (size_t)(C::MT >> 4) * C::NWB * 64;
        load_w(0, wa);
        load_w(1, wb);
        __builtin_amdgcn_sched_barrier(0);
    } else {
        stage_load(0);
        if (wave_active) {
            load_w(0, wa);
            if (KT > 1 || nskip > 0) load_w(1, wb);
        }
        gtab_store();
        if constexpr (FOLD_LATE0) {
            if (fold0_pending) {
                gn_fold_sample<false, false>(reinterpret_cast<double*>(lds), b, p.cf_st0, p.C0, p.cf_st1, p.C1, p.T_in, p.cf_ns0, p.cf_ns1, p.cf_gamma,
                                             p.cf_beta, const_cast<float*>(p.gscale), const_cast<float*>(p.gshift), p.cf_mean_rstd, gtab, gtab + Cin);
                __syncthreads();
                g_a = *reinterpret_cast<const float4*>(gtab + 4 * m);
                g_s = *reinterpret_cast<const float4*>(gtab + Cin + 4 * m);
            }
        }
        stage_write(0, 0);
        __syncthreads();
#ifdef TQ_STAMP
        unsigned long long s_load = 0, s_mma = 0, s_write = 0, s_bar = 0;
        const unsigned long long t_begin = __builtin_amdgcn_s_memtime();
        if (tid == 0 && blockIdx.x < 4096) {
            unsigned long long* tl = tq_timeline + blockIdx.x * 8;
            tl[0] = r_entry; tl[1] = __builtin_amdgcn_s_memrealtime(); tl[4] = t_entry; tl[5] = t_begin;
        }
#endif
        if constexpr (!FUSE) {
            for (int c = 0; c + 1 < nstages; ++c) {
                TQ_T(tA)
#ifndef TQ_ABL_NOSTAGE
                stage_load(c + 1);
#endif
                TQ_T(tB)
                if (wave_active) {
                    if (!FUSE || c < nchunks) compute(c, c & 1);
                    else compute_skip(c - nchunks, c & 1);
                }
                TQ_T(tC)
#ifndef TQ_ABL_NOSTAGE
                stage_write(c + 1, (c + 1) & 1);
// ... 297 lines not shown
                    for (int j = 0; j < 4; ++j) { s1[cbk][j] += v[j]; s2[cbk][j] += v[j] * xv[j]; }
                }
            }
        }
        if (p.bflags & TQ_BWD_STATS) {
#pragma unroll
            for (int cbk = 0; cbk < 2; ++cbk) {
                const int co = co_wave + cbk * 16 + 4 * (lane >> 4);
#pragma unroll
                for (int j = 0; j < 4; ++j) {
#pragma unroll
                    for (int o = 1; o < 16; o <<= 1) {
                        s1[cbk][j] += __shfl_xor(s1[cbk][j], o);
                        s2[cbk][j] += __shfl_xor(s2[cbk][j], o);
                    }
                }
                if constexpr (TBW == 8) {
                    if ((lane & 15) == 0 && slot < p.nslots) {
                        float* st = p.stats + (((size_t)b * p.nslots + slot) * Ctot + co) * 2;
                        *reinterpret_cast<float4*>(st) = make_float4(s1[cbk][0], s2[cbk][0], s1[cbk][1], s2[cbk][1]);
                        *reinterpret_cast<float4*>(st + 4) = make_float4(s1[cbk][2], s2[cbk][2], s1[cbk][3], s2[cbk][3]);
                    }
                }
            }
            if constexpr (TBW == 4) {
                __syncthreads();
                float* red = reinterpret_cast<float*>(lds) + (wm * 4 + (lane >> 4)) * 16;
                if (wn == 1 && (lane & 15) == 0) {
#pragma unroll
                    for (int cbk = 0; cbk < 2; ++cbk)
#pragma unroll
                        for (int j = 0; j < 4; ++j) { red[(cbk * 4 + j) * 2] = s1[cbk][j]; red[(cbk * 4 + j) * 2 + 1] = s2[cbk][j]; }
                }
                __syncthreads();
                if (wn == 0 && (lane & 15) == 0 && slot < p.nslots) {
#pragma unroll
                    for (int cbk = 0; cbk < 2; ++cbk) {
                        const int co = co_wave + cbk * 16 + 4 * (lane >> 4);
                        float a1[4], a2[4];
#pragma unroll
                        for (int j = 0; j < 4; ++j) { a1[j] = s1[cbk][j] + red[(cbk * 4 + j) * 2]; a2[j] = s2[cbk][j] + red[(cbk * 4 + j) * 2 + 1]; }
                        float* st = p.stats + (((size_t)b * p.nslots + slot) * Ctot + co) * 2;
                        *reinterpret_cast<float4*>(st) = make_float4(a1[0], a2[0], a1[1], a2[1]);
                        *reinterpret_cast<float4*>(st + 4) = make_float4(a1[2], a2[2], a1[3], a2[3]);
                    }
                }
            }
        }
    }
    if constexpr (PW) {
        co_wave += C::MT;
        if (++pass < npass) goto next_pass;
    }
#ifdef TQ_STAMP
    if (tid == 0 && blockIdx.x < 4096) {
        unsigned long long* tl = tq_timeline + blockIdx.x * 8;
        tl[3] = __builtin_amdgcn_s_memrealtime(); tl[7] = __builtin_amdgcn_s_memtime();
    }
#endif
}

template <int KT, int STRIDE, int UPS, int WM, int WN, int EPI, int ACT, int SCH, bool PW, int TBW, int NCB, int GTW>
struct ConvLds {
    using C = Cfg<KT, STRIDE, UPS, WM, WN, SCH, TBW, NCB>;
    static constexpr int GTAB_MAX = ((SCH == 2 && ACT >= 1) || (SCH == 0 && TBW == 2 && ACT >= 1 && !PW && EPI == 0)) ? 2 * 4 * GTW : 0;
    static constexpr int STAGE = PW ? 4 * C::BUF : C::LDS_BYTES;
    static constexpr int BYTES = STAGE + GTAB_MAX;
    static constexpr int FOLD_MAX_CIN = GTW != 1024 ? 0 : ((STAGE / 8 - 64) / 2 < 1024 ? (STAGE / 8 - 64) / 2 : 1024);
};
constexpr int TQ_LDS_WORKGROUP_MAX = 163840;

template <int KT, int STRIDE, int UPS, int WM, int WN, int EPI, int ACT, bool FUSE, int SCH = 0, bool PW = false, int TBW = 8, int NCB = 2, int GTW = 1024>
int launch(const ConvArgs& a, hipStream_t stream) {
    using C = Cfg<KT, STRIDE, UPS, WM, WN, SCH, TBW, NCB>;
    using L = ConvLds<KT, STRIDE, UPS, WM, WN, EPI, ACT, SCH, PW, TBW, NCB, GTW>;
    auto kern = conv1d_mfma_kernel<KT, STRIDE, UPS, WM, WN, EPI, ACT, FUSE, SCH, PW, TBW, NCB, GTW>;
    constexpr int GTAB_MAX = L::GTAB_MAX;
    constexpr int LDS_BYTES = L::BYTES;
    static_assert(LDS_BYTES <= TQ_LDS_WORKGROUP_MAX, "tile + coefficient table exceed the LDS a workgroup may declare");
    if (a.cf_st0 && GTW != 1024) return TQ_ERR_SHAPE;
    if (GTAB_MAX && a.cf_st0 && a.C0 + a.C1 > 1024) return TQ_ERR_SHAPE;
    if (SCH == 2 && ACT >= 1 && a.C0 + a.C1 > GTW) return TQ_ERR_SHAPE;
    if (a.cf_st0) {
        constexpr bool built = (TBW == 2 && ACT >= 1 && !PW && EPI == 0) || (SCH == 2 && ACT >= 1 && !PW && EPI == 0 && TBW == 8);
        if (!built || (size_t)(2 * (a.C0 + a.C1) + 64) * sizeof(double) > (size_t)(LDS_BYTES - GTAB_MAX)) return TQ_ERR_SHAPE;
    }
    static std::atomic<uint64_t> attr_done{0};
    int dev_ord = 0;
    (void)hipGetDevice(&dev_ord);
    const uint64_t dev_bit = 1ull << (dev_ord & 63);
    if (!(attr_done.load(std::memory_order_acquire) & dev_bit)) {
        hipError_t e = hipFuncSetAttribute(reinterpret_cast<const void*>(kern),
                                           hipFuncAttributeMaxDynamicSharedMemorySize, LDS_BYTES);
        if (e != hipSuccess) return (int)e;
        attr_done.fetch_or(dev_bit, std::memory_order_release);
    }
    const int n_ttiles = (a.T_out + C::NT - 1) / C::NT;
    const int n_ctiles = (a.C_out + C::MT - 1) / C::MT;
    const unsigned grid = (unsigned)(a.B * n_ttiles * (PW ? 1 : n_ctiles));
    hipLaunchKernelGGL(kern, dim3(grid), dim3(C::NTHR), LDS_BYTES, stream, a);
    TQ_CHECK_LAUNCH();
    return 0;
}

template <int KT, int STRIDE, int UPS, int EPI, int ACT, bool FUSE = false>
int dispatch_tile(const ConvArgs& a, hipStream_t s) {
    if (a.t_tile == 32) {
        if constexpr (KT == 5 && STRIDE == 1 && UPS == 0 && EPI == 0 && ACT >= 2) {
            if (a.flags & TQ_CONV_POLY2) return TQ_ERR_SHAPE;
            if (a.wfmt == TQ_WFMT_F16_MX6) {
                if (a.C0 % 64 || a.C1 % 64 || a.sC0 % 64 || a.sC1 % 64 || a.C_out % 128) return TQ_ERR_SHAPE;
                if (conv_wide_table(a)) return conv_launch_fwd_wide(a, KT, ACT, FUSE, s);
                return launch<KT, STRIDE, UPS, 4, 1, EPI, ACT, FUSE, 2, false, 2>(a, s);
            }
            if (a.wfmt != TQ_WFMT_BF16X3) return TQ_ERR_SHAPE;
            if (a.C_out % 128 == 0) return launch<KT, STRIDE, UPS, 4, 1, EPI, ACT, FUSE, 0, false, 2>(a, s);
            if (a.C_out % 64 == 0) return launch<KT, STRIDE, UPS, 2, 1, EPI, ACT, FUSE, 0, false, 2>(a, s);
            return launch<KT, STRIDE, UPS, 1, 1, EPI, ACT, FUSE, 0, false, 2>(a, s);
        }
        return TQ_ERR_SHAPE;
    }
    if (a.wfmt == TQ_WFMT_F16_MX6) {
        if constexpr (STRIDE == 1 && UPS == 0 && EPI == 1 && ACT == 0 && !FUSE) {
            if (a.C0 % 64 || a.C1) return TQ_ERR_SHAPE;
            if (a.C_out % 256 == 0) return launch<KT, STRIDE, UPS, 8, 1, EPI, ACT, FUSE, 2>(a, s);
            if (a.C_out % 128 == 0) return launch<KT, STRIDE, UPS, 4, 1, EPI, ACT, FUSE, 2>(a, s);
            if (a.C_out % 64 == 0) return launch<KT, STRIDE, UPS, 2, 2, EPI, ACT, FUSE, 2, false, 4>(a, s);
            return TQ_ERR_SHAPE;
        }
        if constexpr (STRIDE == 1 && EPI != 1) {
            if (a.C0 % 64 || a.C1 % 64 || a.sC0 % 64 || a.sC1 % 64) return TQ_ERR_SHAPE;
            if constexpr (UPS == 0 && EPI == 0 && ACT >= 1) {
                if (conv_wide_table(a)) return conv_launch_fwd_wide(a, KT, ACT, FUSE, s);
            }
            if constexpr (KT == 1 && UPS == 0 && ACT <= 1) {
                const int cin = a.C0 + a.C1;
                const bool pw = !(a.flags & TQ_CONV_CH_TILES);
                if (pw && a.C_out % 256 == 0 && a.C_out >= 512 && (cin == 128 || cin == 256))
                    return launch<KT, STRIDE, UPS, 8, 1, EPI, ACT, FUSE, 2, true>(a, s);
            }
            if (a.C_out % 256 == 0) return launch<KT, STRIDE, UPS, 8, 1, EPI, ACT, FUSE, 2>(a, s);
            if (a.C_out % 128 == 0) return launch<KT, STRIDE, UPS, 4, 1, EPI, ACT, FUSE, 2>(a, s);
            if constexpr (KT == 5 && UPS == 0 && EPI == 0 && ACT >= 2) {
                if (a.C_out % 64 == 0 && !(a.flags & TQ_CONV_POLY2)) return launch<KT, STRIDE, UPS, 2, 2, EPI, ACT, FUSE, 2, false, 4>(a, s);
            }
        }
        return TQ_ERR_SHAPE;
    }
    if (a.wfmt == TQ_WFMT_F16_MX8) {
        if constexpr (STRIDE == 1 && EPI != 1) {

            if (a.C0 % 64 || a.C1 % 64 || a.sC0 % 64 || a.sC1 % 64) return TQ_ERR_SHAPE;
            if constexpr (KT == 1 && UPS == 0 && ACT <= 1) {
                const int cin = a.C0 + a.C1;
                if (a.C_out % 256 == 0 && a.C_out >= 512 && (cin == 128 || cin == 256))
                    return launch<KT, STRIDE, UPS, 8, 1, EPI, ACT, FUSE, 1, true>(a, s);
            }
            if (a.C_out % 256 == 0) return launch<KT, STRIDE, UPS, 8, 1, EPI, ACT, FUSE, 1>(a, s);
            if (a.C_out % 128 == 0) return launch<KT, STRIDE, UPS, 4, 1, EPI, ACT, FUSE, 1>(a, s);
        }
        return TQ_ERR_SHAPE;
    }
    if (a.wfmt != TQ_WFMT_BF16X3) return TQ_ERR_ARG;
    if constexpr (STRIDE == 1 && UPS == 0) {
        if (a.C_out % 256 == 0) return launch<KT, STRIDE, UPS, 8, 1, EPI, ACT, FUSE>(a, s);
    }
    if (a.C_out % 128 == 0) return launch<KT, STRIDE, UPS, 4, 1, EPI, ACT, FUSE>(a, s);
// ... 28 lines not shown
```

tqdne_amd/csrc/conv1d_mfma.hip:

```cpp
#include <cmath>

#include "common.hpp"
#include "conv_args.hpp"
#include "../../include/tqdne_hip.h"

using namespace tq;

extern "C" int tq_conv_tile_co(int C_out) {
    if (C_out % 128 == 0) return 128;
    if (C_out % 64 == 0) return 64;
    return 32;
}

static int conv1d_fwd_impl(const TqConvDesc* d, const float* x0, const float* x1, const float* gscale, const float* gshift,
                           const void* wpk, const float* bias, const float* emb, const float* res, const float* skip_x0,
                           const float* skip_x1, const float* skip_bias, float* y, float* stats, hipStream_t stream,
                           unsigned char* kv_planes = nullptr, int kvH = 0, int kvD = 0, int kvTp = 0, float kvscale = 1.f, int kv_vf16 = 0);

extern "C" int tq_conv1d_fwd_qkv(const TqConvDesc* d, const float* x, const float* gscale, const float* gshift, const void* wpk,
                                 const float* bias, float* qkv, void* kv_planes, int H, int D, int v_format, hipStream_t stream) {
    if (!d || !kv_planes || H <= 0 || (D != 32 && D != 64)) return TQ_ERR_ARG;
    if (v_format != TQ_KV_V_BF16 && v_format != TQ_KV_V_F16) return TQ_ERR_ARG;
    if (d->ktaps != 1 || d->stride != 1 || d->upsample || d->C_in1 || d->C_out != 3 * H * D || (d->C_skip0 | d->C_skip1)) return TQ_ERR_SHAPE;
    if (d->flags & (TQ_CONV_EMB | TQ_CONV_RES | TQ_CONV_STATS | TQ_CONV_DROPOUT | TQ_CONV_SILU)) return TQ_ERR_ARG;
    const int Tp = (d->T_out + 63) / 64 * 64;
    const float scale = (float)(1.0 / sqrt(sqrt((double)D)));
    return conv1d_fwd_impl(d, x, nullptr, gscale, gshift, wpk, bias, nullptr, nullptr, nullptr, nullptr, nullptr, qkv, nullptr, stream,
                           reinterpret_cast<unsigned char*>(kv_planes), H, D, Tp, scale, v_format == TQ_KV_V_F16 ? 1 : 0);
}

extern "C" int tq_conv1d_fwd(const TqConvDesc* d, const float* x0, const float* x1, const float* gscale,
                             const float* gshift, const void* wpk, const float* bias, const float* emb,
                             const float* res, float* y, float* stats, hipStream_t stream) {
    if (d && (d->C_skip0 || d->C_skip1)) return TQ_ERR_ARG;
    return conv1d_fwd_impl(d, x0, x1, gscale, gshift, wpk, bias, emb, res, nullptr, nullptr, nullptr, y, stats, stream);
}

extern "C" int tq_conv1d_fwd_skip(const TqConvDesc* d, const float* x0, const float* x1, const float* gscale,
                                  const float* gshift, const void* wpk_main_then_skip, const float* bias, const float* emb,
                                  const float* skip_x0, const float* skip_x1, const float* skip_bias, float* y, float* stats,
                                  hipStream_t stream) {
    if (!d || !skip_x0 || d->C_skip0 <= 0 || d->C_skip0 % 32 || d->C_skip1 < 0 || d->C_skip1 % 32) return TQ_ERR_ARG;
    if (d->C_skip1 > 0 && !skip_x1) return TQ_ERR_ARG;
    if (d->stride != 1 || d->upsample || (d->flags & TQ_CONV_RES)) return TQ_ERR_SHAPE;
    return conv1d_fwd_impl(d, x0, x1, gscale, gshift, wpk_main_then_skip, bias, emb, nullptr, skip_x0, skip_x1, skip_bias, y,
                           stats, stream);
}

static int conv1d_fwd_impl(const TqConvDesc* d, const float* x0, const float* x1, const float* gscale, const float* gshift,
                           const void* wpk, const float* bias, const float* emb, const float* res, const float* skip_x0,
                           const float* skip_x1, const float* skip_bias, float* y, float* stats, hipStream_t stream,
                           unsigned char* kv_planes, int kvH, int kvD, int kvTp, float kvscale, int kv_vf16) {
    if (!d || !x0 || !wpk || !y) return TQ_ERR_ARG;
    if (d->C_in0 <= 0 || d->C_in0 % 32 || d->C_in1 < 0 || d->C_in1 % 32 || d->C_out <= 0 || d->C_out % 32) return TQ_ERR_SHAPE;
    if (d->C_in1 > 0 && !x1) return TQ_ERR_ARG;
    if ((d->flags & TQ_CONV_GN) && (!gscale || !gshift)) return TQ_ERR_ARG;
    if ((d->flags & TQ_CONV_EMB) && !emb) return TQ_ERR_ARG;
    if ((d->flags & TQ_CONV_RES) && !res) return TQ_ERR_ARG;
    if ((d->flags & TQ_CONV_STATS) && !stats) return TQ_ERR_ARG;
    if (d->B <= 0 || d->T_in <= 0 || d->T_out <= 0) return TQ_ERR_SHAPE;
    if (d->stride == 1) {
        const int Tsrc = d->upsample ? 2 * d->T_in : d->T_in;
        if (d->T_out != Tsrc || d->pad != d->ktaps / 2) return TQ_ERR_SHAPE;
    } else if (d->stride == 2) {
        if (d->ktaps != 3 || d->pad != 1 || d->upsample || d->T_out != (d->T_in + 2 - 3) / 2 + 1) return TQ_ERR_SHAPE;
    } else {
        return TQ_ERR_SHAPE;
    }
    ConvArgs a;
    a.x0 = x0; a.x1 = x1; a.gscale = gscale; a.gshift = gshift;
    a.wpk = reinterpret_cast<const uint4*>(wpk);
    a.bias = bias; a.emb = emb; a.res = res; a.y = y; a.stats = stats;
    a.B = d->B; a.T_in = d->T_in; a.T_out = d->T_out; a.C0 = d->C_in0; a.C1 = d->C_in1; a.C_out = d->C_out;
    a.emb_stride = d->emb_stride; a.flags = d->flags;
    const int tile = tq_conv_tile_co(d->C_out);
    a.ncob_pad = ((d->C_out + tile - 1) / tile) * tile / 16;
    a.nslots = (d->T_out + STAT_SLOT - 1) / STAT_SLOT;
    a.t_tile = 0;
    if (d->t_tile) {
        const int need = TQ_CONV_GN | TQ_CONV_SILU;
        if (d->t_tile != 32) return TQ_ERR_ARG;
        if (d->ktaps != 5 || d->stride != 1 || d->upsample || kv_planes || (d->flags & need) != need || (d->flags & TQ_CONV_POLY2))
            return TQ_ERR_SHAPE;
        a.t_tile = 32;
        a.nslots = (d->T_out + 31) / 32;
    }
    if (d->flags & TQ_CONV_POLY2) {
        if (d->ktaps != 3 || d->stride != 1 || d->upsample || (d->C_out & 63) || kv_planes || d->C_skip0 || d->C_skip1) return TQ_ERR_SHAPE;
        if ((d->flags & TQ_CONV_STATS) && d->T_out % STAT_SLOT && d->T_out % STAT_SLOT <= STAT_SLOT / 2) return TQ_ERR_SHAPE;
        a.nslots *= 2;
    }
    a.drop_site = d->dropout_site;
    a.drop_seed = d->dropout_seed;
    float pdrop = d->dropout_p;
    if (!(d->flags & TQ_CONV_DROPOUT) || pdrop <= 0.f) { a.flags &= ~TQ_CONV_DROPOUT; pdrop = 0.f; }
    if (pdrop >= 1.f) return TQ_ERR_ARG;
    a.drop_thresh = (uint32_t)((double)pdrop * 4294967296.0);
    a.drop_scale = 1.0f / (1.0f - pdrop);
    a.fx0 = a.fx1 = a.fgs = a.fgh = nullptr; a.y1 = nullptr; a.OC0 = d->C_out; a.bflags = 0;
    a.sx0 = skip_x0; a.sx1 = skip_x1; a.sbias = skip_bias; a.sC0 = d->C_skip0; a.sC1 = d->C_skip1;
    a.wfmt = d->wfmt;
    a.kv = kv_planes; a.kvH = kvH; a.kvD = kvD; a.kvTp = kvTp; a.kvscale = kvscale; a.kv_vf16 = (kv_planes && kv_vf16) ? 1 : 0;
    a.range_flag = d->range_flag;
    a.in_amax = nullptr;
    a.cf_st0 = a.cf_st1 = a.cf_gamma = a.cf_beta = nullptr; a.cf_mean_rstd = nullptr; a.cf_ns0 = a.cf_ns1 = 0;
    if (d->gn_fold) {
        const TqGnFold* f = d->gn_fold;
        if (!(d->flags & TQ_CONV_GN) || kv_planes || (a.t_tile != 32 && d->wfmt != TQ_WFMT_F16_MX6)) return TQ_ERR_SHAPE;
        if (!f->stats0 || !f->gamma || !f->beta || (d->C_in1 > 0 && !f->stats1)) return TQ_ERR_ARG;
        const int s0 = f->slot0 ? f->slot0 : STAT_SLOT, s1 = f->slot1 ? f->slot1 : STAT_SLOT;
        if ((s0 != STAT_SLOT && s0 != 32) || (s1 != STAT_SLOT && s1 != 32)) return TQ_ERR_ARG;
        if ((d->C_in0 + d->C_in1) % GN_GROUPS) return TQ_ERR_SHAPE;
        a.cf_st0 = f->stats0; a.cf_st1 = d->C_in1 > 0 ? f->stats1 : nullptr;
        a.cf_ns0 = (d->T_in + s0 - 1) / s0; a.cf_ns1 = (d->T_in + s1 - 1) / s1;
        a.cf_gamma = f->gamma; a.cf_beta = f->beta; a.cf_mean_rstd = f->mean_rstd;
    }
    if (d->reserved1) return TQ_ERR_ARG;

    if (d->stride == 2 || d->upsample) {
        if (a.flags & (TQ_CONV_GN | TQ_CONV_SILU | TQ_CONV_DROPOUT)) return TQ_ERR_SHAPE;
        return conv_launch_resample(a, d->ktaps, d->stride, stream);
    }
    if (a.kv) {
        return conv_launch_qkv(a, stream);
    }
    switch (d->ktaps) {
        case 1: return conv_launch_fwd_k1(a, stream);
        case 3: return conv_launch_fwd_k3(a, stream);
        case 5: return conv_launch_fwd_k5(a, stream);
        default: return TQ_ERR_SHAPE;
    }
}

extern "C" int tq_conv1d_bwd_data(const TqConvBwdDesc* d, const float* dy, const void* wpk_t, const float* x0,
                                  const float* x1, const float* gscale, const float* gshift, float* dx0, float* dx1,
                                  float* gstats, hipStream_t stream) {
    if (!d || !dy || !wpk_t || !dx0) return TQ_ERR_ARG;
    if (d->C_dy <= 0 || d->C_dy % 32 || d->C_dx0 <= 0 || d->C_dx0 % 32 || d->C_dx1 < 0 || d->C_dx1 % 32) return TQ_ERR_SHAPE;
    if (d->C_dx1 > 0 && !dx1) return TQ_ERR_ARG;
    const int need_x = d->flags & (TQ_BWD_GN | TQ_BWD_SILU | TQ_BWD_STATS);
    if (need_x && (!x0 || (d->C_dx1 > 0 && !x1))) return TQ_ERR_ARG;
    if ((d->flags & TQ_BWD_GN) && (!gscale || !gshift)) return TQ_ERR_ARG;
    if ((d->flags & TQ_BWD_STATS) && !gstats) return TQ_ERR_ARG;
    if (d->B <= 0 || d->T <= 0 || (d->ktaps != 1 && d->ktaps != 3 && d->ktaps != 5)) return TQ_ERR_SHAPE;
    ConvArgs a;
    a.x0 = dy; a.x1 = nullptr; a.gscale = nullptr; a.gshift = nullptr;
    a.wpk = reinterpret_cast<const uint4*>(wpk_t);
    a.bias = nullptr; a.emb = nullptr; a.res = nullptr; a.y = dx0; a.stats = gstats;
    a.B = d->B; a.T_in = d->T; a.T_out = d->T; a.C0 = d->C_dy; a.C1 = 0; a.C_out = d->C_dx0 + d->C_dx1;
    a.emb_stride = 0; a.flags = 0;
    const int tile = tq_conv_tile_co(a.C_out);
    a.ncob_pad = ((a.C_out + tile - 1) / tile) * tile / 16;
    a.nslots = (d->T + STAT_SLOT - 1) / STAT_SLOT;
    a.drop_site = d->dropout_site; a.drop_seed = d->dropout_seed;
    float pdrop = d->dropout_p;
    a.bflags = d->flags;
    if (!(d->flags & TQ_BWD_DROPOUT) || pdrop <= 0.f) { a.bflags &= ~TQ_BWD_DROPOUT; pdrop = 0.f; }
    if (pdrop >= 1.f) return TQ_ERR_ARG;
    a.drop_thresh = (uint32_t)((double)pdrop * 4294967296.0);
    a.drop_scale = 1.0f / (1.0f - pdrop);
    a.fx0 = x0; a.fx1 = x1; a.fgs = gscale; a.fgh = gshift; a.y1 = dx1; a.OC0 = d->C_dx0;
    a.sx0 = a.sx1 = a.sbias = nullptr; a.sC0 = a.sC1 = 0;
    a.wfmt = TQ_WFMT_BF16X3;
    a.in_amax = nullptr;
    a.t_tile = 0;
    if (d->wfmt == TQ_WFMT_F16_MX6) {
        if (!d->dy_amax) return TQ_ERR_ARG;
        if (d->C_dy % 64 || a.C_out % 64) return TQ_ERR_SHAPE;
        a.wfmt = TQ_WFMT_F16_MX6;
        a.in_amax = d->dy_amax;
    } else if (d->wfmt != TQ_WFMT_BF16X3) {
        return TQ_ERR_ARG;
    }
    a.kv = nullptr; a.kvH = a.kvD = a.kvTp = 0; a.kvscale = 1.f; a.kv_vf16 = 0;
    a.range_flag = nullptr;
    a.cf_st0 = a.cf_st1 = a.cf_gamma = a.cf_beta = nullptr; a.cf_mean_rstd = nullptr; a.cf_ns0 = a.cf_ns1 = 0;
    return conv_launch_dgrad(a, d->ktaps, stream);
}

namespace {
__device__ __forceinline__ void pack_mx_body(const float* __restrict__ w, int C_out, int C_in, int K, int ncob_pad,
                                             uint4* __restrict__ out, size_t gid) {
    const int nchunks = (C_in + 63) / 64;
    const size_t total = (size_t)nchunks * K * ncob_pad * 64;
    if (gid >= total) return;
    const int lane = gid & 63;
    size_t r = gid >> 6;
    const int cob = r % ncob_pad; r /= ncob_pad;
    const int tap = r % K;
    const int chunk = r / K;
    const int row = cob * 16 + (lane & 15), kq = lane >> 4;
// ... 202 lines not shown
```

tqdne_amd/engine.py:

```python

from __future__ import annotations

import ctypes as C
import os
from typing import List, Optional, Sequence, Tuple

import torch

from . import _lib
from .engine_bwd import BackwardPlan
from ._lib import (TQ_CONV_DROPOUT, TQ_CONV_EMB, TQ_CONV_GN, TQ_CONV_RES, TQ_CONV_SILU, TQ_CONV_STATS, STAT_SLOT,
                   TqConvDesc, check)


def require_device(x: torch.Tensor):
    if not x.is_cuda:
        raise RuntimeError(
            "tqdne_amd runs its hot path on MI355X HIP kernels only; got a CPU tensor. "
            "(The CPU restatement lives in oracle/ and is test infrastructure, not a fallback.)"
        )
    if x.dtype != torch.float32:
        raise TypeError("tqdne_amd expects fp32 tensors at the boundary, like the reference (precision 32)")


def _noop_launch(*_args):
    return 0


def nslots(T: int) -> int:
    return (T + STAT_SLOT - 1) // STAT_SLOT


def _p(t: Optional[torch.Tensor]) -> Optional[int]:
    return None if t is None else t.data_ptr()


class Act:

    __slots__ = ("buf", "stats", "C", "T", "grad", "gw", "slot")

    def __init__(self, buf, stats, C, T, slot=STAT_SLOT):
        self.buf, self.stats, self.C, self.T = buf, stats, C, T
        self.slot = slot
        self.grad = None
        self.gw = False


FUSE_SKIP_CO = 32
SMALL_TILE_B = 4
SMALL_TILE_WGS = 64
GN_FOLD_DEFAULT = os.environ.get("TQDNE_GN_FOLD", "0") == "1"
CONCURRENT_LANE0 = 8


class ConvRec:

    __slots__ = ("site", "desc", "srcs", "gn", "out", "stride", "upsample", "silu", "dropout", "poly")

    def __init__(self, site, desc, srcs, gn, out, stride, upsample, silu, dropout):
        self.site, self.desc, self.srcs, self.gn, self.out = site, desc, srcs, gn, out
        self.stride, self.upsample, self.silu, self.dropout = stride, upsample, silu, dropout
        self.poly = None


_SIDE_STREAMS: dict = {}


def side_stream(dev, i: int = 1) -> "torch.cuda.Stream":
    key = (str(dev), i)
    s = _SIDE_STREAMS.get(key)
    if s is None:
        s = _SIDE_STREAMS[key] = torch.cuda.Stream(device=dev)
    return s


def reserve_side_streams(dev, n: int = 3):
    if torch.device(dev).type != "cuda" or (str(dev), "reserved") in _SIDE_STREAMS or torch.cuda.is_current_stream_capturing():
        return
    _SIDE_STREAMS[(str(dev), "reserved")] = True
    import torch.distributed as dist
    if dist.is_available() and dist.is_initialized() and dist.get_backend() == "nccl":
        import warnings
        warnings.warn("tqdne_amd: the RCCL process group exists before this device's side streams made their first submission; if its "
                      "communicator is already created the backward's two streams may share a hardware queue (training step ~25 % "
                      "slower).  Call tqdne_amd.trainer.init_process_group(...) (or tqdne_amd.engine.reserve_side_streams(device)) "
                      "before torch.distributed.init_process_group.", RuntimeWarning, stacklevel=2)
    main = torch.cuda.current_stream(dev)
    z = torch.zeros(1, device=dev)
    for i in range(1, n + 1):
        s = side_stream(dev, i)
        s.wait_stream(main)
        with torch.cuda.stream(s):
            z.add_(0)
        main.wait_stream(s)


_PACK_TABLES: dict = {}


def pack_batch(lib, dev, jobs, stream, capturing=False):
    if not jobs:
        return
    key = (str(dev), tuple(jobs))
    ent = _PACK_TABLES.get(key)
    if ent is None and (capturing or len(jobs) < 2 or len(_PACK_TABLES) >= 4096):
        ent = False
    if ent is None:
        arr = (_lib.TqPackJob * len(jobs))()
        total = 0
        for jb, (src, dst, co, ci, k, mode) in zip(arr, jobs):
            jb.src, jb.dst, jb.C_out, jb.C_in, jb.K, jb.mode, jb.block_begin = src, dst, co, ci, k, mode, total
            nb = lib.tq_pack_job_blocks(co, ci, k, mode)
            if nb <= 0:
                raise ValueError(f"bad pack job {(co, ci, k, mode)}")
            total += nb
        table = torch.frombuffer(bytearray(bytes(arr)), dtype=torch.uint8).to(dev)
        ent = _PACK_TABLES[key] = (table, len(jobs), total)
    if ent is False:
        for src, dst, co, ci, k, mode in jobs:
            if mode == 4:
                _lib_copy_floats(dst, src, co, stream)
            else:
                check(lib.tq_pack_conv_weight(src, co, ci, k, mode, dst, stream), "pack")
        return
    table, n, total = ent
    check(lib.tq_pack_jobs(table.data_ptr(), n, total, stream), "pack jobs")


_HIP_RUNTIME = None


def _lib_copy_floats(dst, src, n, stream):
    global _HIP_RUNTIME
    if _HIP_RUNTIME is None:
# ... 215 lines not shown
        key = (tag, C_, T_, stats, slot)
        first = self._ckpt_pool.get(key)
        if first is None:
            first = self._ckpt_pool[key] = self._act(C_, T_, stats, slot)
            return first
        a = Act(first.buf, first.stats, C_, T_, slot)
        self.acts.append(a)
        return a

    def _site(self, name: str, conv: torch.nn.Module, pad_cin=None, pad_cout=None) -> ConvSite:
        s = ConvSite(name, conv.weight, conv.bias, self.dev, self.lib, store=self.store, pad_cin=pad_cin, pad_cout=pad_cout)
        self.conv_sites.append(s)
        return s

    def _site_pair(self, name: str, conv, tail_name: str, tail_conv):
        lib = self.lib
        co, ci, k = conv.weight.shape
        tco, tci, tk = tail_conv.weight.shape
        assert tk == 1 and tco == co
        main_bytes = lib.tq_conv_weight_pack_bytes(co, ci, k, 0)
        tail_bytes = lib.tq_conv_weight_pack_bytes(tco, tci, 1, 0)
        s = ConvSite(name, conv.weight, conv.bias, self.dev, lib, tail_bytes=tail_bytes, store=self.store)
        t = ConvSite(tail_name, tail_conv.weight, tail_conv.bias, self.dev, lib, packed=s.packed[main_bytes:])
        s.tail = t
        self.conv_sites += [s, t]
        return s, t

    def _emit(self, op, infer_op=None, nbytes=0):
        self.ops.append(op)
        self.ops_infer.append(op if infer_op is None else infer_op)
        self.op_bytes.append(nbytes)

    def _launch_bound(self, T_out: int) -> bool:
        return self.B <= SMALL_TILE_B or (self.solo and self.B * ((T_out + 127) // 128) <= SMALL_TILE_WGS)

    def _gn(self, srcs: Sequence[Act], norm: torch.nn.GroupNorm, defer: bool = False):
        C_ = sum(s.C for s in srcs)
        gscale, gshift = self._empty(self.B, C_), self._empty(self.B, C_)
        mean_rstd = self._empty(self.B, 32, 2)
        s0 = srcs[0]
        s1 = srcs[1] if len(srcs) > 1 else None
        fin = ((self.lib.tq_gn_finalize, (
            _p(s0.stats), s0.C, _p(s1.stats) if s1 else None, s1.C if s1 else 0, self.B, s0.T,
            _p(norm.weight), _p(norm.bias), _p(gscale), _p(gshift), _p(mean_rstd), s0.slot, s1.slot if s1 else 0), "gn_finalize", 0),
            4 * self.B * (2 * nslots(s0.T) * C_ + 2 * C_))
        if defer:
            self._pending_gn = dict(key=gscale.data_ptr(), fin=fin, srcs=(s0, s1), norm=norm, mean_rstd=mean_rstd)
            return gscale, gshift, mean_rstd
        self._emit(fin[0], nbytes=fin[1])
        return gscale, gshift, mean_rstd

    def _conv(self, srcs: Sequence[Act], site: ConvSite, *, gn=None, silu=False, emb_ptr=None, res: Optional[Act] = None,
              stats=True, stride=1, upsample=False, dropout_site: Optional[int] = None, launch: bool = True,
              skip: Optional[Tuple[Sequence[Act], ConvSite]] = None, qkv_planes=None, ckpt_tag: Optional[str] = None) -> Optional[Act]:
        s0 = srcs[0]
        s1 = srcs[1] if len(srcs) > 1 else None
        if s1 is not None and s1.T != s0.T:
            raise RuntimeError(f"Sizes of tensors must match except in dimension 1: lengths {s0.T} and {s1.T} at {site.name} "
                               "(the signal length must be divisible by the UNet's total down-sampling factor)")
        T_in = s0.T
        if stride == 2:
            T_out = (T_in + 2 - site.K) // 2 + 1
            pad = site.K // 2
        else:
            T_out = 2 * T_in if upsample else T_in
            pad = site.K // 2
        srcs_c = [s0.C, (s1.C if s1 else 0)] + ([a.C for a in skip[0]] if skip is not None else [])
        k5_act = site.K == 5 and gn is not None and silu and stride == 1 and not upsample and qkv_planes is None
        _check_width_limits(site.name, site.C_in, site.C_out)
        wfmt = _lib.forward_wfmt(site.C_out, srcs_c, stride, upsample, k5_act=k5_act, gn=gn is not None) if launch else 0
        small = (launch and self._launch_bound(T_out) and k5_act
                 and wfmt in (_lib.TQ_WFMT_BF16X3, _lib.TQ_WFMT_F16_MX6))
        if small and wfmt == _lib.TQ_WFMT_F16_MX6 and site.C_out % 128:
            wfmt = _lib.TQ_WFMT_BF16X3
        if launch and ckpt_tag is not None and self.ckpt:
            out = self._ckpt_act(ckpt_tag, site.C_out, T_out, stats, slot=32 if small else STAT_SLOT)
        else:
            out = self._act(site.C_out, T_out, stats, slot=32 if small else STAT_SLOT) if launch else None
        d = TqConvDesc()
        d.t_tile = 32 if small else 0
        pend = self._pending_gn
        if pend is not None and gn is not None and pend["key"] == gn[0].data_ptr():
            self._pending_gn = None
            fold_max = self.lib.tq_conv1d_gn_fold_max_cin(wfmt, 32 if small else 0, site.C_out)
            if small and wfmt != _lib.TQ_WFMT_BF16X3:
                fold_max = min(fold_max, self.lib.tq_conv1d_gn_fold_max_cin(_lib.TQ_WFMT_BF16X3, 32, site.C_out))
            fold_fits = site.C_in <= fold_max
            fold_default = (GN_FOLD_DEFAULT and not small and k5_act and wfmt == _lib.TQ_WFMT_F16_MX6 and self.scheme == "auto"
                            and getattr(self.m, "_conv_scheme", "auto") == "auto" and fold_fits)
            if fold_default and launch and not self.ckpt:
                fn, fargs, fname, ffl = pend["fin"][0]
                self._fold_default_ops.append((len(self.ops), fn, d))
                self._emit((_noop_launch, fargs, fname + " (folded into its consumer)", ffl), nbytes=0)
            if launch and ((small and fold_fits) or fold_default) and not self.ckpt:
                f = _lib.TqGnFold()
                ps0, ps1 = pend["srcs"]
                f.stats0, f.stats1 = _p(ps0.stats), (_p(ps1.stats) if ps1 is not None else None)
                f.slot0, f.slot1 = ps0.slot, (ps1.slot if ps1 is not None else 0)
                f.gamma, f.beta, f.mean_rstd = _p(pend["norm"].weight), _p(pend["norm"].bias), _p(pend["mean_rstd"])
                self._keep.append(f)
                d.gn_fold = C.pointer(f)
                self.gn_folded += 1
            else:
                self._emit(pend["fin"][0], nbytes=pend["fin"][1])
        d.B, d.T_in, d.T_out = self.B, T_in, T_out
        d.C_in0, d.C_in1, d.C_out = s0.C, (s1.C if s1 else 0), site.C_out
        assert d.C_in0 + d.C_in1 == site.C_in, (site.name, d.C_in0, d.C_in1, site.C_in)
        d.ktaps, d.stride, d.pad, d.upsample = site.K, stride, pad, int(upsample)
        flags = 0
        if gn is not None:
            flags |= TQ_CONV_GN
        if silu:
            flags |= TQ_CONV_SILU
        if emb_ptr is not None:
            flags |= TQ_CONV_EMB
        if res is not None:
            flags |= TQ_CONV_RES
            assert res.C == site.C_out and res.T == T_out
        if stats:
            flags |= TQ_CONV_STATS
        if site.K == 1 and self._launch_bound(T_out):
            flags |= _lib.TQ_CONV_CH_TILES
        d.flags = flags
        d.emb_stride = self.emb_total
        d.wfmt = wfmt
        if launch:
            site.pack_mode = _lib.PACK_MODE[d.wfmt]
            if skip is not None:
                skip[1].pack_mode = site.pack_mode
            self._wfmt_sites.append((d, [site] + ([skip[1]] if skip is not None else []), d.wfmt))
            if stats:
                d.range_flag = self.range_flag.data_ptr()
        d.dropout_site = dropout_site or 0
        d.dropout_p = 0.0
        d.dropout_seed = 0
        if dropout_site is not None:
            self.dropout_descs.append(d)
        self._keep.append(d)
        flops = 2 * site.C_in * site.C_out * site.K * T_out * self.B
        nbytes = 4 * self.B * (T_in * site.C_in + T_out * site.C_out + (T_out * site.C_out if res is not None else 0))
        if skip is not None:
            ksrcs, ksite = skip
            k0, k1 = ksrcs[0], (ksrcs[1] if len(ksrcs) > 1 else None)
            assert res is None and k0.T == T_out and ksite.C_out == site.C_out
            d.C_skip0, d.C_skip1 = k0.C, (k1.C if k1 else 0)
            self._emit((self.lib.tq_conv1d_fwd_skip, (
                C.byref(d), _p(s0.buf), _p(s1.buf) if s1 else None, _p(gn[0]) if gn else None, _p(gn[1]) if gn else None,
                _p(site.packed), _p(site.bias), emb_ptr, _p(k0.buf), _p(k1.buf) if k1 else None, _p(ksite.bias),
                _p(out.buf), _p(out.stats)),
                "conv:" + site.name + "+skip", flops + 2 * ksite.C_in * site.C_out * T_out * self.B),
                nbytes=nbytes + 4 * self.B * T_out * ksite.C_in)
        elif launch:
            op = (self.lib.tq_conv1d_fwd, (
                C.byref(d), _p(s0.buf), _p(s1.buf) if s1 else None, _p(gn[0]) if gn else None, _p(gn[1]) if gn else None,
                _p(site.packed), _p(site.bias_pad if site.bias_pad is not None else site.bias), emb_ptr, _p(res.buf) if res else None,
                _p(out.buf), _p(out.stats)), "conv:" + site.name, flops)
            infer_op = None
            if (upsample and site.K == 5 and (T_in % STAT_SLOT == 0 or T_in % STAT_SLOT > STAT_SLOT // 2) and site.C_out % 32 == 0 and gn is None and res is None
                    and emb_ptr is None and os.environ.get("TQDNE_POLYPHASE_UPSAMPLE", "1") != "0"):
                infer_op = self._polyphase_op(site, d, s0, s1, out, flops)
                if s1 is None:
                    op = infer_op
            if qkv_planes is not None:
                ws, H_, D_ = qkv_planes
                d.range_flag = self.range_flag.data_ptr()
                infer_op = (self.lib.tq_conv1d_fwd_qkv, (
                    C.byref(d), _p(s0.buf), _p(gn[0]) if gn else None, _p(gn[1]) if gn else None, _p(site.packed), _p(site.bias),
                    _p(out.buf), _p(ws), H_, D_, self.kv_v_format), "conv:" + site.name + "+split", flops)
                self._vfmt_ops.append(len(self.ops_infer))
            self._emit(op, infer_op, nbytes=nbytes)
        self.last_rec = ConvRec(site, d, list(srcs), gn, out, stride, upsample, silu, dropout_site is not None)
# ... 144 lines not shown
            entry = (name, 2 * B * T * cin * co * K, 4 * B * T * (cin + co))
        if trace is not None:
            trace.append(entry + (e0, _recorded_event()))

    def _run_head(self, head, epilogue, stream, trace, what, name):
        B, T, fin, co, K = self.B, self.final.T, self.final, head.out_channels, head.kernel_size[0]
        c_out, c_skip, skip_src = epilogue or (None, None, None)
        io = co * (1 if epilogue is None else 2)
        e0 = _recorded_event() if trace is not None else None
        if self.out_mode == "head":
            gn = self.head_gn or (None, None)
            check(self.lib.tq_head_conv_fwd(_p(fin.buf), _p(gn[0]), _p(gn[1]), _p(head.weight), _p(head.bias), _p(c_out), _p(c_skip),
                                            _p(skip_src), _p(self.out_nct), B, T, fin.C, co, K, stream), what)
            entry = (name, 2 * B * T * fin.C * co * K, 4 * B * T * (fin.C + io))
        elif self.out_mode == "wide":
            check(self.lib.tq_btc_to_nct(_p(self.head_btc.buf), _p(c_out), _p(c_skip), _p(skip_src), _p(self.out_nct), B, T,
                                         self.head_btc.C, 0, co, stream), "head epilogue (btc_to_nct)")
            entry = ("btc_to_nct:" + name, 0, 4 * B * T * (self.head_btc.C + io))
        else:
            self.out_nct.copy_(self.head_btc.buf.permute(0, 2, 1))
            entry = ("output layout flip", 0, 4 * B * T * (fin.C + io))
        if trace is not None:
            trace.append(entry + (e0, _recorded_event()))

    def _arm_dropout(self, p: float, seed: int, descs=None, flag: int = TQ_CONV_DROPOUT):
        for d in self.dropout_descs if descs is None else descs:
            if p > 0.0:
                d.flags |= flag
                d.dropout_p, d.dropout_seed = p, seed
            else:
                d.flags &= ~flag

    def _run_ops(self, ops, stream, trace):
        probe = self._probe
        if trace is None and (probe is None or torch.cuda.is_current_stream_capturing()):
            for fn, args, what, _ in ops:
                rc = fn(*args, stream)
                if rc:
                    check(rc, what)
            return
        for i, (fn, args, what, fl) in enumerate(ops):
            timed = trace is not None or i == probe.idx
            a = _recorded_event() if timed else None
            rc = fn(*args, stream)
            if trace is not None:
                trace.append((what, fl, self.op_bytes[i], a, _recorded_event()))
            elif timed:
                probe.events.append((a, _recorded_event()))
            if rc:
                check(rc, what)

    def _res_block(self, x, rb, name: str) -> Act:
        srcs = list(x) if isinstance(x, tuple) else [x]
        emb_ptr = self.emb_all.data_ptr() + 4 * self.emb_offsets[id(rb)] if hasattr(rb, "emb_layers") else None
        g1 = self._gn(srcs, rb.in_layers[0], defer=not self.ckpt)
        i_conv1 = len(self.ops)
        h1 = self._conv(srcs, self._site(name + ".in_layers.2", rb.in_layers[2]), gn=g1, silu=True, emb_ptr=emb_ptr, ckpt_tag="h1")
        rec1 = self.last_rec
        i_gn2 = len(self.ops)
        g2 = self._gn([h1], rb.out_layers[0], defer=not self.ckpt)
        recompute = list(range(i_conv1, len(self.ops))) if self.ckpt else None
        rec_sk = None
        conv2 = rb.out_layers[3]
        self._site_counter += 1
        if isinstance(rb.skip_connection, torch.nn.Identity):
            assert len(srcs) == 1
            out = self._conv([h1], self._site(name + ".out_layers.3", conv2), gn=g2, silu=True, res=srcs[0],
                             dropout_site=self._site_counter)
        elif conv2.weight.shape[2] == 5 and conv2.weight.shape[0] % FUSE_SKIP_CO == 0 and all(a.C % 32 == 0 for a in srcs):
            site2, site_sk = self._site_pair(name + ".out_layers.3", conv2, name + ".skip_connection", rb.skip_connection)
            self._conv(srcs, site_sk, stats=False, launch=False)
            rec_sk = self.last_rec
            out = self._conv([h1], site2, gn=g2, silu=True, dropout_site=self._site_counter, skip=(srcs, site_sk))
        else:
            res = self._conv(srcs, self._site(name + ".skip_connection", rb.skip_connection), stats=False)
            rec_sk = self.last_rec
            out = self._conv([h1], self._site(name + ".out_layers.3", conv2), gn=g2, silu=True, res=res,
                             dropout_site=self._site_counter)
        self.tape.append(("res", dict(rb=rb, srcs=srcs, g1=g1, g2=g2, h1=h1, out=out, rec1=rec1, rec2=self.last_rec,
                                      rec_sk=rec_sk, recompute=recompute)))
        return out

    def _attention(self, x: Act, ab, name: str) -> Act:
        g = self._gn([x], ab.norm)
        D = ab.channels // ab.num_heads
        hd = D not in (32, 64, 128)
        if hd and not self.lib.tq_attention_head_tile(D):
            raise NotImplementedError(f"attention head dim {D}: kernels exist for multiples of 8 from 8 to 256 "
                                      "(larger heads need another kernel structure: their K / V tiles do not fit the LDS)")
        ws_bytes = self.lib.tq_attention_hd_workspace_bytes if hd else self.lib.tq_attention_workspace_bytes
        ws = self._attn_workspace(ws_bytes(self.B, x.T, ab.num_heads, D), "_attn_ws_hd" if hd else "_attn_ws")
        split = (ws, ab.num_heads, D) if D in (32, 64) else None
        i_qkv = len(self.ops)
        qkv = self._conv([x], self._site(name + ".qkv", ab.qkv), gn=g, silu=False, stats=False, qkv_planes=split, ckpt_tag="qkv")
        rec_qkv = self.last_rec
        att = self._ckpt_act("att", ab.channels, x.T, False) if self.ckpt else self._act(ab.channels, x.T, False)
        if self.ckpt:
            lse = self._ckpt_pool.get(("lse", ab.num_heads, x.T))
            if lse is None:
                lse = self._ckpt_pool[("lse", ab.num_heads, x.T)] = self._empty(self.B, ab.num_heads, x.T)
        else:
            lse = self._empty(self.B, ab.num_heads, x.T)
        flops = 4 * ab.channels * x.T * x.T * self.B
        fwd = self.lib.tq_attention_fwd_hd if hd else self.lib.tq_attention_fwd
        ws_fwd = ws if (split is not None or self._launch_bound(x.T)) else None
        op = (fwd, (_p(qkv.buf), _p(att.buf), _p(lse), _p(ws_fwd), self.B, x.T, ab.num_heads, D), "attention", flops)
        if split is not None and not self.ckpt:
            self._attn_train_ops.append((len(self.ops), len(self.tape), ws.numel()))
        infer_op = None
        if split is not None:
            infer_op = (self.lib.tq_attention_fwd_presplit, (_p(qkv.buf), _p(ws), _p(att.buf), self.B, x.T, ab.num_heads, D,
                                                             self.kv_v_format), "attention", flops)
            self._vfmt_ops.append(len(self.ops_infer))
        self._emit(op, infer_op, nbytes=4 * self.B * x.T * 4 * ab.channels)
        recompute = list(range(i_qkv, len(self.ops))) if self.ckpt else None
        out = self._conv([att], self._site(name + ".proj_out", ab.proj_out), res=x)
        entry = dict(ab=ab, x=x, g=g, qkv=qkv, att=att, lse=lse, out=out, rec_qkv=rec_qkv, rec_proj=self.last_rec, D=D,
                     recompute=recompute)
        if self.ckpt and split is not None:
            entry["kv_ws"], entry["kv_always"] = ws, True
        self.tape.append(("attn", entry))
        return out

    def _attn_workspace(self, nbytes: int, slot: str = "_attn_ws"):
        ws = getattr(self, slot)
        if ws is None or ws.numel() != nbytes:
            ws = torch.zeros(nbytes, dtype=torch.uint8, device=self.dev)
            self._keep.append(ws)
            setattr(self, slot, ws)
        return ws

    def install_probe(self, name_prefix: str = "conv:"):
        idx = max((i for i, op in enumerate(self.ops) if op[2].startswith(name_prefix)), key=lambda i: self.ops[i][3])
        self._probe = Probe(idx, self.ops[idx][2], self.ops[idx][3])
        return self._probe

    def _set_scheme_bf16x3(self):
        for d, sites, _pref in self._wfmt_sites:
            d.wfmt = _lib.TQ_WFMT_BF16X3
            for st in sites:
                st.pack_mode = 0
        for i, fn, d in self._fold_default_ops:
            for ops in (self.ops, self.ops_infer):
                _f, a_, w_, fl_ = ops[i]
                ops[i] = (fn, a_, "gn_finalize", fl_)
            d.gn_fold = None
        self._fold_default_ops = []
        if self.emb_desc is not None:
            self.emb_desc.wfmt = _lib.TQ_WFMT_BF16X3
            self.emb_pack_mode = 0
        self.set_kv_v_format(_lib.TQ_KV_V_BF16)
        self.scheme = "bf16x3"
        self.plan_epoch += 1

    def enable_block_kv(self):
        if self._block_kv:
            return
        for i, ti, nbytes in self._attn_train_ops:
            ws = torch.zeros(nbytes, dtype=torch.uint8, device=self.dev)
            self._keep.append(ws)
            fn, args, *rest = self.ops[i]
            self.ops[i] = (fn, args[:3] + (ws.data_ptr(),) + args[4:], *rest)
            self.tape[ti][1]["kv_ws"] = ws
        self._block_kv = True

    def set_kv_v_format(self, fmt: int):
        if fmt != self.kv_v_format:
# ... 261 lines not shown
```

tqdne_amd/engine_bwd.py:

```python

from __future__ import annotations

import ctypes as C
import math
from typing import Dict, List

import torch

from . import _lib
from ._lib import (PACK_MODE_T, TQ_AMAX_WORDS, TQ_BWD_ACCUM, TQ_BWD_DROPOUT, TQ_BWD_GN, TQ_BWD_SILU, TQ_BWD_STATS, TQ_WFMT_BF16X3, TQ_WFMT_F16_MX6, STAT_SLOT,
                   TqConvBwdDesc, TqConvDesc, check)


TAIL_WORDS = 2


def _p(t):
    return None if t is None else t.data_ptr()


BWD_STREAMS = int(__import__("os").environ.get("TQDNE_BWD_STREAMS", "2"))

DGRAD_MX6_C64 = __import__("os").environ.get("TQDNE_DGRAD_MX6_C64", "0") == "1"
N_AMAX = 160


def _copy_floats(dst, src, n, stream):
    from .engine import _lib_copy_floats
    _lib_copy_floats(dst, src, n, stream)
    return 0


def _nslots(T):
    return (T + STAT_SLOT - 1) // STAT_SLOT


class BackwardPlan:
    def __init__(self, eng):
        self.e = eng
        self.lib = eng.lib
        self.B, self.dev = eng.B, eng.dev
        self.m = eng.m
        self._keep = []
        self.ops: List = []
        self.bwd_dropout_descs: List[TqConvBwdDesc] = []
        self._scratch: Dict = {}
        self.op_flops: Dict[int, int] = {}
        self._trace = None
        self._wgrad_ops = []
        self.ws_bytes = 0
        self._grad_writer = {}
        self.head_op = self.stem_op = None
        self.dx_op = None
        self.last_dx = None
        self.wide_head = eng.wide_head
        self.wide_stem = eng.wide_stem
        self.stem_cp = eng.x_btc.C if eng.wide_stem else 32
        self.stem_generic = False
        self.stem_x_btc = self.dw_stem32 = None
        self._side_evs = {}
        self._fire_cache = None
        self._gemm_levels = None
        self._layout_gradients()
        for a in eng.acts:
            a.gw = False
        self._build()
        self._finish_workspace()
        eng.enable_block_kv()

    def _finish_workspace(self):
        self.ws = torch.empty(max(self.ws_bytes, 16), dtype=torch.uint8, device=self.dev)
        for i in self._wgrad_ops:
            self.ops[i][1][7] = self.ws.data_ptr()
            self.ops[i][1][8] = self.ws.numel()

    def _empty(self, *shape):
        t = torch.empty(*shape, dtype=torch.float32, device=self.dev)
        self._keep.append(t)
        return t

    def scratch(self, tag, *shape):
        key = (tag,) + tuple(shape)
        t = self._scratch.get(key)
        if t is None:
            t = self._empty(self.B, *shape)
            self._scratch[key] = t
        return t

    def grad(self, act):
        if act.grad is None:
            act.grad = self._empty(self.B, act.T, act.C)
        return act.grad

    def _readiness_keys(self):
        e, m = self.e, self.m
        n = len(e.tape)
        key = {}

        def mark(ps, k):
            for p in ps:
                if p is not None:
                    key.setdefault(id(p), k)

        head = [m.out] if hasattr(m, "out") else [m.output_layer]
        for mod in head:
            mark(mod.parameters(), 0)
# ... 47 lines not shown
        total += self.B * e.emb_total
        total = (total + 63) // 64 * 64
        off_amax = total
        total += N_AMAX * TQ_AMAX_WORDS
        self.flat = torch.zeros(total, dtype=torch.float32, device=self.dev)
        self.amax = self.flat[off_amax:off_amax + N_AMAX * TQ_AMAX_WORDS].view(torch.int32)
        self._amax_slot = {}
        self.dgrad_descs = []
        self._mx6_dgrads = []
        self.gview = {id(p): self.flat[offs[id(p)]:offs[id(p)] + p.numel()].view_as(p) for p in swept + emb_w + emb_b + tail}
        self.demb_all = self.flat[self.off_demb:self.off_demb + self.B * e.emb_total].view(self.B, e.emb_total)
        o = self.off_emb
        self.g_emb_w = self.flat[o:o + e.emb_total * e.E].view(e.emb_total, e.E)
        self.g_emb_b = self.flat[o + e.emb_total * e.E:o + e.emb_total * e.E + e.emb_total]
        self.offs = offs
        self._ready = {}
        self._swept_ids = {id(p) for p in swept}

    END = 1 << 30

    def plan_buckets(self, bucket_elems: int):
        spans = []
        for p in self.param_order:
            o = self.offs[id(p)]
            r = self._ready.get(id(p), self.END) if id(p) in self._swept_ids else self.END
            if r >= len(self.ops):
                r = self.END
            if not p.requires_grad:
                r = -1
            spans.append((o, o + p.numel(), r))
        spans.sort()
        buckets, lo, ready = [], 0, -1
        for o, hi, r in spans:
            ready = max(ready, r)
            if hi - lo >= bucket_elems:
                hi_al = min((hi + 63) // 64 * 64, self.n_grad)
                buckets.append((lo, hi_al, ready))
                lo = hi_al
        if lo < self.n_grad:
            buckets.append((lo, self.n_grad, max(ready, spans[-1][2]) if buckets else ready))
        out, run_max = [], -1
        for lo_, hi_, r in buckets:
            run_max = max(run_max, r)
            out.append((lo_, hi_, run_max))
        return out

    def amax_ptr(self, dy_ptr: int, create: bool = True):
        i = self._amax_slot.get(dy_ptr)
        if i is None:
            if not create or len(self._amax_slot) >= N_AMAX:
                return None
            i = self._amax_slot[dy_ptr] = len(self._amax_slot)
        return self.amax.data_ptr() + 4 * TQ_AMAX_WORDS * i

    def g(self, param):
        self._ready[id(param)] = len(self.ops)
        return self.gview[id(param)]

    def gv(self, param):
        return self.gview[id(param)]

    def _wgrad(self, rec, dy, bias_colsum=True, colsum=None, dw=None):
        lib, site = self.lib, rec.site
        need = lib.tq_conv1d_bwd_weight_workspace(C.byref(rec.desc))
        self.ws_bytes = max(self.ws_bytes, need)
        self._wgrad_ops.append(len(self.ops))
        s0 = rec.srcs[0]
        s1 = rec.srcs[1] if len(rec.srcs) > 1 else None
        if colsum is None and bias_colsum and site.bias is not None:
            colsum = (None, 0, site.bias, None)
        if colsum is not None:
            self._colsum_pass(dy, rec.out.T if rec.out is not None else rec.desc.T_out, site.C_out, *colsum, site.name)
            self._wgrad_ops[-1] = len(self.ops)
        self.op_flops[len(self.ops)] = 2 * site.C_in * site.C_out * site.K * rec.desc.T_out * self.B
        self.ops.append([lib.tq_conv1d_bwd_weight_colsum, [C.byref(rec.desc), _p(dy), _p(s0.buf), _p(s1.buf) if s1 else None,
                                                           _p(rec.gn[0]) if rec.gn else None, _p(rec.gn[1]) if rec.gn else None,
                                                           _p(dw) if dw is not None else _p(self.g(site.weight)), None, 0, None, 0, None,
                                                           None], "wgrad:" + site.name])

    def _colsum_pass(self, dy, T_dy, C_dy, bc, stride, c1, c2, name):
        lib = self.lib
        amax = self.amax_ptr(dy.data_ptr())
        wr = self._grad_writer.get(dy.data_ptr())
        if wr is not None and wr[0][0] is lib.tq_gn_bwd_apply:
            op = wr[0]
            op[0] = lib.tq_gn_bwd_apply_colsum
            op[1] = op[1] + [bc, stride, _p(self.g(c1)) if c1 is not None else None, _p(self.g(c2)) if c2 is not None else None, amax]
            op[2] = "gn_bwd_apply+colsum:" + name
        else:
            self.ops.append([lib.tq_colsum, [_p(dy), self.B, T_dy, C_dy, bc, stride,
                                             _p(self.g(c1)) if c1 is not None else None, _p(self.g(c2)) if c2 is not None else None, None, amax],
                             "colsum:" + name])

    def _dgrad(self, rec, dy, T, dsts, accumulate, chain=True, stats=True, amax_of=None):
        lib, site = self.lib, rec.site
        amax = self.amax_ptr((amax_of if amax_of is not None else dy).data_ptr(), create=False)
        cin_ok = site.C_in % 128 == 0 or (site.C_in % 64 == 0 and DGRAD_MX6_C64)
        mx6 = (_lib.requested_scheme() == "f16mx6"
               and amax is not None and site.C_out % 64 == 0 and cin_ok
               and self.e.scheme == "auto" and getattr(self.m, "_conv_scheme", "auto") == "auto")
        want = 5 if mx6 else 1
        if site.packed_t is None:
            nb = max(lib.tq_conv_weight_pack_bytes(site.C_out, site.C_in, site.K, 1),
                     lib.tq_conv_weight_pack_bytes(site.C_out, site.C_in, site.K, 5) if site.C_out % 64 == 0 else 0)
            site.packed_t = torch.empty(nb, dtype=torch.uint8, device=self.dev)
            site.pack_mode_t = want
            self.e.dgrad_sites.append(site)
        elif site.pack_mode_t != want:
            raise RuntimeError(f"{site.name}: data gradient planned twice with different weight formats")
        d = TqConvBwdDesc()
        d.wfmt = TQ_WFMT_F16_MX6 if mx6 else TQ_WFMT_BF16X3
        d.dy_amax = amax if mx6 else None
        self.dgrad_descs.append(d)
        if mx6:
            self._mx6_dgrads.append((d, site))
        d.B, d.T, d.C_dy = self.B, T, site.C_out
        d.C_dx0 = dsts[0].shape[2]
        d.C_dx1 = dsts[1].shape[2] if len(dsts) > 1 else 0
        assert d.C_dx0 + d.C_dx1 == site.C_in
        d.ktaps = site.K
        f = TQ_BWD_ACCUM if accumulate else 0
        gst = None
        s0 = rec.srcs[0]
        s1 = rec.srcs[1] if len(rec.srcs) > 1 else None
        if chain:
            if rec.gn is not None:
                f |= TQ_BWD_GN
                if stats:
                    f |= TQ_BWD_STATS
                    gst = self._empty(self.B, _nslots(T), site.C_in, 2)
            if rec.silu:
                f |= TQ_BWD_SILU
            if rec.dropout:
                self.bwd_dropout_descs.append(d)
        d.flags = f
        d.dropout_site = rec.desc.dropout_site
        self._keep.append(d)
        self.op_flops[len(self.ops)] = 2 * site.C_in * site.C_out * site.K * (rec.desc.T_out if rec.stride == 2 else T) * self.B
        self.ops.append([lib.tq_conv1d_bwd_data, [C.byref(d), _p(dy), _p(site.packed_t), _p(s0.buf) if chain else None,
                                                  _p(s1.buf) if (chain and s1) else None,
                                                  _p(rec.gn[0]) if (chain and rec.gn) else None,
                                                  _p(rec.gn[1]) if (chain and rec.gn) else None, _p(dsts[0]),
                                                  _p(dsts[1]) if len(dsts) > 1 else None, _p(gst)], "dgrad:" + site.name])
        for t_ in dsts:
            self._wrote(t_)
        return gst

    def _gn_bwd(self, gst, gn, norm, T, Ctot):
        ca, cb, cc = self._empty(self.B, Ctot), self._empty(self.B, Ctot), self._empty(self.B, Ctot)
        self.ops.append([self.lib.tq_gn_bwd_finalize, [_p(gst), _p(gn[2]), _p(norm.weight), self.B, Ctot, T, _p(ca), _p(cb), _p(cc),
                                                       _p(self.g(norm.weight)), _p(self.g(norm.bias))], "gn_bwd_finalize"])
        return ca, cb, cc

    def _gn_apply(self, G, act, coef, Ctot, coff, r=None):
        dx = self.grad(act)
        self.ops.append([self.lib.tq_gn_bwd_apply, [_p(G), _p(act.buf), _p(r), _p(coef[0]), _p(coef[1]), _p(coef[2]), _p(dx), self.B,
                                                    act.T, act.C, Ctot, coff, int(act.gw)], "gn_bwd_apply"])
        self._wrote(dx)
        act.gw = True

    def _wrote(self, grad_tensor):
        self._grad_writer[grad_tensor.data_ptr()] = (self.ops[-1],)

    def _build(self):
        e, m, lib, B = self.e, self.m, self.lib, self.B
        final = e.final
        head = m.out[2]
        from .engine import _check_head_bwd_limits
        if not self.wide_head:
            _check_head_bwd_limits(final.C, m.out_channels, head.kernel_size[0])
        Gh = self.scratch("G", final.T, final.C)
        nws = lib.tq_stem_head_bwd_workspace()
        self._ws_head = torch.empty(nws, dtype=torch.uint8, device=self.dev)
        self._ws_stem = torch.empty(nws, dtype=torch.uint8, device=self.dev)
        if self.wide_head:
            gst = self._wide_head_bwd(e.head_rec, head, final, Gh, m.out_channels)
        else:
            gst = self._empty(B, _nslots(final.T), final.C, 2)
            self.head_op = [lib.tq_head_conv_bwd_ws, [None, None, _p(final.buf), _p(e.head_gn[0]), _p(e.head_gn[1]), _p(head.weight), _p(Gh),
                                                      _p(gst), _p(self.g(head.weight)), _p(self.g(head.bias)), B, final.T, final.C,
                                                      m.out_channels, head.kernel_size[0], _p(self._ws_head), nws], "head bwd"]
        coef = self._gn_bwd(gst, e.head_gn, m.out[0], final.T, final.C)
        self._gn_apply(Gh, final, coef, final.C, 0)
        for kind, t in reversed(e.tape):
            getattr(self, "_bwd_" + kind)(t)
        stem = m.input_blocks[0][0]
        so = e.stem_out
        self.stem_op = [lib.tq_stem_conv_bwd_weight_ws, [_p(so.grad), None, None, _p(self.g(stem.weight)), B, m.in_channels, so.T,
                                                         stem.out_channels, stem.kernel_size[0], _p(self._ws_stem), nws], "stem wgrad"]
        self._ready[id(stem.weight)] = self.END
        self._stem_gradients(stem, self.wide_stem or stem.out_channels * m.in_channels * stem.kernel_size[0] > 2048, "wgrad:stem (generic)")

    def _stem_gradients(self, stem, generic: bool, what: str):
        e, lib, B, so = self.e, self.lib, self.B, self.e.stem_out
        assert so.gw
        self.stem_generic = generic
        if generic:
            K, Cp = stem.kernel_size[0], self.stem_cp
            if self.wide_stem:
                self.stem_x_btc = e.x_btc.buf
            else:
                self.stem_x_btc = self._empty(B, so.T, Cp)
                self.stem_x_btc.zero_()
            d = TqConvDesc()
            d.B, d.T_in, d.T_out, d.C_in0, d.C_in1, d.C_out = B, so.T, so.T, Cp, 0, stem.out_channels
            d.ktaps, d.stride, d.pad, d.upsample, d.flags = K, 1, K // 2, 0, 0
            self._keep.append(d)
            self.dw_stem32 = self._empty(stem.out_channels, Cp, K)
            self.ws_bytes = max(self.ws_bytes, lib.tq_conv1d_bwd_weight_workspace(C.byref(d)))
            self._wgrad_ops.append(len(self.ops))
            self.ops.append([lib.tq_conv1d_bwd_weight, [C.byref(d), _p(so.grad), _p(self.stem_x_btc), None, None, None,
                                                        _p(self.dw_stem32), None, 0], what])
        self.ops.append([lib.tq_colsum, [_p(so.grad), B, so.T, so.C, None, 0, _p(self.g(stem.bias)), None, None, None], "colsum:stem"])

    def _wide_head_bwd(self, rec, head, final, Gh, co):
        site, Cp = rec.site, rec.site.C_out
        self.dF = self._empty(self.B, final.T, Cp)
        self.head_op = [self.lib.tq_nct_to_btc, [None, None, None, _p(self.dF), self.B, co, 0, final.T, Cp], "head dF (nct_to_btc)"]
        if self.offs[id(head.bias)] % 64 or Cp > 64 or id(head.bias) not in self._swept_ids:
            raise RuntimeError(f"{site.name}: the padded bias gradient ({Cp} column sums) needs the 64-float alignment gap behind the bias "
                               "gradient in the flat buffer (_layout_gradients)")
        self._colsum_pass(self.dF, final.T, Cp, None, 0, head.bias, None, site.name)
        self.dw_head_pad = self._empty(Cp, site.C_in, site.K)
        self._wgrad(rec, self.dF, bias_colsum=False, dw=self.dw_head_pad)
        self.ops.append([_copy_floats, [_p(self.g(head.weight)), _p(self.dw_head_pad), head.weight.numel()], "wgrad:rows:" + site.name])
        return self._dgrad(rec, self.dF, final.T, [Gh], accumulate=False)

    def _recompute(self, t):
        for i in t.get("recompute") or ():
            fn, args, what, _fl = self.e.ops[i]
            self.ops.append([fn, list(args), "recompute:" + what])

    def _bwd_res(self, t):
        self._recompute(t)
        rb, srcs, h1, out = t["rb"], t["srcs"], t["h1"], t["out"]
        rec1, rec2, rec_sk = t["rec1"], t["rec2"], t["rec_sk"]
        B, T, Co = self.B, out.T, out.C
        assert out.gw, "gradient of a block output must be complete before its backward"
        dout = out.grad
        self._wgrad(rec2, dout, colsum=(None, 0, rec2.site.bias, rec_sk.site.bias if rec_sk is not None else None))
        G2 = self.scratch("G", T, Co)
        gst2 = self._dgrad(rec2, dout, T, [G2], accumulate=False)
        coef2 = self._gn_bwd(gst2, t["g2"], rb.out_layers[0], T, Co)
        h1.gw = False
        self._gn_apply(G2, h1, coef2, Co, 0)
        dh1 = h1.grad
        emb_dst = None
        if hasattr(rb, "emb_layers"):
            emb_dst = self.demb_all.data_ptr() + 4 * self.e.emb_offsets[id(rb)]
        self._wgrad(rec1, dh1, colsum=(emb_dst, self.e.emb_total, rec1.site.bias, None))
        Ctot = sum(s.C for s in srcs)
        G1 = [self.scratch("G1_%d" % i, T, s.C) for i, s in enumerate(srcs)]
        gst1 = self._dgrad(rec1, dh1, T, G1, accumulate=False)
        coef1 = self._gn_bwd(gst1, t["g1"], rb.in_layers[0], T, Ctot)
        if rec_sk is None:
            self._gn_apply(G1[0], srcs[0], coef1, Ctot, 0, r=dout)
        else:
            self._wgrad(rec_sk, dout, bias_colsum=False)
            acc = srcs[0].gw
            assert all(s.gw == acc for s in srcs)
            self._dgrad(rec_sk, dout, T, [self.grad(s) for s in srcs], accumulate=acc, chain=False)
            for s in srcs:
                s.gw = True
            coff = 0
            for Gs, s in zip(G1, srcs):
                self._gn_apply(Gs, s, coef1, Ctot, coff)
                coff += s.C

    def _bwd_attn(self, t):
        self._recompute(t)
        ab, x, qkv, att, out = t["ab"], t["x"], t["qkv"], t["att"], t["out"]
        B, T, Cc = self.B, x.T, x.C
        assert out.gw
        dout = out.grad
        self._wgrad(t["rec_proj"], dout)
        datt = self.grad(att)
        self._dgrad(t["rec_proj"], dout, T, [datt], accumulate=False, chain=False)
        dqkv = self.grad(qkv)
        delta = self._empty(B, ab.num_heads, T)
        self.op_flops[len(self.ops)] = 2 * 4 * ab.channels * T * T * B
        Tp = (T + 63) // 64 * 64
        ws = self.scratch("attn_bwd_ws", 4 * ab.num_heads * Tp * t["D"]) if t["D"] in (32, 64) else None
        if ws is not None:
            e, lib = self.e, self.lib

            def attn_bwd(qkv_p, att_p, datt_p, lse_p, delta_p, dqkv_p, ws_p, B_, T_, H_, D_, stream, _t=t):
                kv = _t.get("kv_ws") if (e._last.get("block_kv") or _t.get("kv_always")) else None
                if kv is not None:
                    return lib.tq_attention_bwd_ws_kv(qkv_p, att_p, datt_p, lse_p, delta_p, dqkv_p, ws_p, kv.data_ptr(), B_, T_, H_, D_, stream)
                return lib.tq_attention_bwd_ws(qkv_p, att_p, datt_p, lse_p, delta_p, dqkv_p, ws_p, B_, T_, H_, D_, stream)
            fn = attn_bwd
        else:
            fn = self.lib.tq_attention_bwd_ws if t["D"] in (32, 64, 128) else self.lib.tq_attention_bwd_hd
        self.ops.append([fn, [_p(qkv.buf), _p(att.buf), _p(datt), _p(t["lse"]), _p(delta), _p(dqkv), _p(ws),
                              B, T, ab.num_heads, t["D"]], "attention bwd"])
        self._wrote(dqkv)
        self._wgrad(t["rec_qkv"], dqkv)
        G = self.scratch("G", T, Cc)
        gst = self._dgrad(t["rec_qkv"], dqkv, T, [G], accumulate=False)
        coef = self._gn_bwd(gst, t["g"], ab.norm, T, Cc)
        self._gn_apply(G, x, coef, Cc, 0, r=dout)

    def _bwd_down(self, t):
        x, out, rec = t["x"], t["out"], t["rec"]
        assert out.gw
        dout = out.grad
        self._wgrad(rec, dout)
        dyz = self.scratch("dyz", x.T, out.C)
        self.ops.append([self.lib.tq_zero_stuff, [_p(dout), _p(dyz), self.B, out.T, x.T, out.C], "zero_stuff"])
        self._dgrad(rec, dyz, x.T, [self.grad(x)], accumulate=x.gw, chain=False, amax_of=dout)
        x.gw = True

    def _bwd_up_poly(self, t):
        from .engine import ConvRec
        lib = self.lib
        x, out, rec = t["x"], t["out"], t["rec"]
        ps, d2 = rec.poly
        site = rec.site
        assert out.gw and len(rec.srcs) == 1
        dout = out.grad
        self._colsum_pass(dout, out.T, site.C_out, None, 0, site.bias, None, site.name)
        dw = TqConvDesc()
        dw.B, dw.T_in, dw.T_out, dw.C_in0, dw.C_in1, dw.C_out = self.B, x.T, x.T, x.C, 0, 2 * site.C_out
        dw.ktaps, dw.stride, dw.pad, dw.upsample, dw.flags = 3, 1, 1, 0, 0
        self._keep.append(dw)
        dW2 = self._empty(2 * site.C_out, site.C_in, 3)
        self.ws_bytes = max(self.ws_bytes, lib.tq_conv1d_bwd_weight_workspace(C.byref(dw)))
        self._wgrad_ops.append(len(self.ops))
        self.op_flops[len(self.ops)] = 2 * site.C_in * 2 * site.C_out * 3 * x.T * self.B
        self.ops.append([lib.tq_conv1d_bwd_weight_colsum, [C.byref(dw), _p(dout), _p(x.buf), None, None, None, _p(dW2), None, 0,
                                                           None, 0, None, None], "wgrad:" + site.name + "+polyphase"])
        self.ops.append([lib.tq_upsample_poly_wgrad_fold, [_p(dW2), _p(self.g(site.weight)), site.C_out, site.C_in],
                         "wgrad:fold:" + site.name])
        rec2 = ConvRec(ps, d2, rec.srcs, None, None, 1, False, False, False)
        self._dgrad(rec2, dout, x.T, [self.grad(x)], accumulate=x.gw, chain=False)
        x.gw = True

# ... 288 lines not shown
```

tqdne_amd/ops.py:

```python

from __future__ import annotations

import ctypes as C
from typing import Optional, Tuple

import torch

from . import _lib
from ._lib import (TQ_CONV_DROPOUT, TQ_CONV_EMB, TQ_CONV_GN, TQ_CONV_RES, TQ_CONV_SILU, TQ_CONV_STATS, STAT_SLOT,
                   TqConvDesc, check)


def _stream(dev):
    return torch.cuda.current_stream(dev).cuda_stream


def _p(t):
    return None if t is None else t.data_ptr()


def nslots(T):
    return (T + STAT_SLOT - 1) // STAT_SLOT


# ... 233 lines not shown
    if silu:
        f |= TQ_CONV_SILU
    if dropout_p > 0:
        f |= TQ_CONV_DROPOUT
    d.flags = f
    d.dropout_site, d.dropout_p, d.dropout_seed = dropout_site, dropout_p, dropout_seed
    ws = torch.empty(lib.tq_conv1d_bwd_weight_workspace(C.byref(d)), dtype=torch.uint8, device=dy.device)
    dw = torch.empty(C_out, C_in, K, device=dy.device) if out is None else out
    if colsum is not None:
        bc, c1 = colsum
        check(lib.tq_conv1d_bwd_weight_colsum(C.byref(d), _p(dy), _p(x0), _p(x1), _p(gscale), _p(gshift), _p(dw), _p(ws), ws.numel(),
                                              _p(bc), C_out if bc is not None else 0, _p(c1), None, _stream(dy.device)),
              "conv1d_bwd_weight_colsum")
        return dw
    check(lib.tq_conv1d_bwd_weight(C.byref(d), _p(dy), _p(x0), _p(x1), _p(gscale), _p(gshift), _p(dw), _p(ws), ws.numel(),
                                   _stream(dy.device)), "conv1d_bwd_weight")
    return dw


def gn_bwd_finalize(gstats, mean_rstd, gamma, T):
    lib = _lib.load()
    B, _, Cn, _ = gstats.shape
    dev = gamma.device
    a, b, c = (torch.empty(B, Cn, device=dev) for _ in range(3))
    dg, db = torch.zeros(Cn, device=dev), torch.zeros(Cn, device=dev)
    check(lib.tq_gn_bwd_finalize(_p(gstats), _p(mean_rstd), _p(gamma), B, Cn, T, _p(a), _p(b), _p(c), _p(dg), _p(db),
                                 _stream(dev)), "gn_bwd_finalize")
    return a, b, c, dg, db


def gn_bwd_apply(g, x, coefs, c_total, c_offset=0, r=None, accumulate_into=None):
    lib = _lib.load()
    B, T, Cs = g.shape
    dx = accumulate_into if accumulate_into is not None else torch.empty_like(g)
    check(lib.tq_gn_bwd_apply(_p(g), _p(x), _p(r), _p(coefs[0]), _p(coefs[1]), _p(coefs[2]), _p(dx), B, T, Cs, c_total, c_offset,
                              int(accumulate_into is not None), _stream(g.device)), "gn_bwd_apply")
    return dx


def colsum(dy, per_sample=True, total=True, bscale=None, amax=None, out=None):
    lib = _lib.load()
    B, T, Cn = dy.shape
    if out is not None:
        obc, oc, oc2 = out
        check(lib.tq_colsum(_p(dy), B, T, Cn, _p(obc), Cn, _p(oc), _p(oc2), _p(bscale), _p(amax), _stream(dy.device)), "colsum")
        return obc, oc, oc2
    obc = torch.zeros(B, Cn, device=dy.device) if per_sample else None
    oc = torch.zeros(Cn, device=dy.device) if total else None
    check(lib.tq_colsum(_p(dy), B, T, Cn, _p(obc), Cn, _p(oc), None, _p(bscale), _p(amax), _stream(dy.device)), "colsum")
    return obc, oc


def amax_bits(dy):
    lib = _lib.load()
    B, T, Cn = dy.shape
    out = torch.zeros(_lib.TQ_AMAX_WORDS, dtype=torch.int32, device=dy.device)
    check(lib.tq_colsum(_p(dy), B, T, Cn, None, 0, None, None, None, _p(out), _stream(dy.device)), "colsum (amax)")
    return out


def amax_value(block) -> float:
    return float(block.max().view(torch.float32).item()) if block.numel() > 1 else float(block.view(torch.float32).item())


def gn_bwd_apply_colsum(g, x, coefs, c_total, c_offset=0, r=None, accumulate_into=None, per_sample=True, total=True, amax=None, out=None):
    lib = _lib.load()
    B, T, Cs = g.shape
    if out is not None:
        dx, obc, oc, oc2 = out
        dx = dx if dx is not None else (accumulate_into if accumulate_into is not None else torch.empty_like(g))
        check(lib.tq_gn_bwd_apply_colsum(_p(g), _p(x), _p(r), _p(coefs[0]), _p(coefs[1]), _p(coefs[2]), _p(dx), B, T, Cs, c_total, c_offset,
                                         int(accumulate_into is not None), _p(obc), Cs, _p(oc), _p(oc2), _p(amax), _stream(g.device)),
              "gn_bwd_apply_colsum")
        return dx, obc, oc, oc2
    dx = accumulate_into if accumulate_into is not None else torch.empty_like(g)
    obc = torch.zeros(B, Cs, device=g.device) if per_sample else None
    oc = torch.zeros(Cs, device=g.device) if total else None
    check(lib.tq_gn_bwd_apply_colsum(_p(g), _p(x), _p(r), _p(coefs[0]), _p(coefs[1]), _p(coefs[2]), _p(dx), B, T, Cs, c_total, c_offset,
                                     int(accumulate_into is not None), _p(obc), Cs, _p(oc), None, _p(amax), _stream(g.device)),
          "gn_bwd_apply_colsum")
    return dx, obc, oc


def zero_stuff(dy, T_in):
    lib = _lib.load()
    B, T_out, Cn = dy.shape
    out = torch.empty(B, T_in, Cn, device=dy.device)
    check(lib.tq_zero_stuff(_p(dy), _p(out), B, T_out, T_in, Cn, _stream(dy.device)), "zero_stuff")
    return out


def pair_sum(d_up, accumulate_into=None):
    lib = _lib.load()
    B, T2, Cn = d_up.shape
    dx = accumulate_into if accumulate_into is not None else torch.empty(B, T2 // 2, Cn, device=d_up.device)
    check(lib.tq_pair_sum(_p(d_up), _p(dx), B, T2 // 2, Cn, int(accumulate_into is not None), _stream(d_up.device)), "pair_sum")
    return dx


def avg_pool2(x, stats=True, out=None):
    lib = _lib.load()
    B, T_in, Cn = x.shape
    if out is not None:
        y, st = out
    else:
        y = torch.empty(B, T_in // 2, Cn, device=x.device)
        st = torch.empty(B, nslots(T_in // 2), Cn, 2, device=x.device) if stats else None
    check(lib.tq_avg_pool2_fwd(_p(x), _p(y), _p(st), B, T_in, Cn, _stream(x.device)), "avg_pool2")
    return y, st


def nearest_up2(x, stats=True, out=None):
    lib = _lib.load()
    B, T_in, Cn = x.shape
    if out is not None:
        y, st = out
    else:
        y = torch.empty(B, 2 * T_in, Cn, device=x.device)
        st = torch.empty(B, nslots(2 * T_in), Cn, 2, device=x.device) if stats else None
    check(lib.tq_nearest_up2_fwd(_p(x), _p(y), _p(st), B, T_in, Cn, _stream(x.device)), "nearest_up2")
    return y, st


def avg_pool2_bwd(dy, T_in, accumulate_into=None):
    lib = _lib.load()
    B, T_out, Cn = dy.shape
    assert T_in // 2 == T_out
    dx = accumulate_into if accumulate_into is not None else torch.empty(B, T_in, Cn, device=dy.device)
    check(lib.tq_avg_pool2_bwd(_p(dy), _p(dx), B, T_in, Cn, int(accumulate_into is not None), _stream(dy.device)), "avg_pool2_bwd")
    return dx


def stem_conv_bwd_weight(dy, x_nct, wshape, in_scale=None, workspace=True):
    lib = _lib.load()
    B, Cin, T = x_nct.shape
    Cout, _, K = wshape
    dw = torch.zeros(Cout, Cin, K, device=dy.device)
    ws = torch.empty(lib.tq_stem_head_bwd_workspace(), dtype=torch.uint8, device=dy.device) if workspace else None
    check(lib.tq_stem_conv_bwd_weight_ws(_p(dy), _p(x_nct), _p(in_scale), _p(dw), B, Cin, T, Cout, K, _p(ws), 0 if ws is None else ws.numel(),
                                         _stream(dy.device)), "stem wgrad")
    return dw


def head_conv_bwd(dpred_nct, x, weight, gscale=None, gshift=None, c_out=None, stats=True, workspace=True, out=None):
    lib = _lib.load()
    B, T, Cin = x.shape
    Cout, _, K = weight.shape
    if out is not None:
        g, st, dw, db = out
    else:
        g = torch.empty_like(x)
        st = torch.empty(B, nslots(T), Cin, 2, device=x.device) if stats else None
        dw, db = torch.zeros_like(weight), torch.zeros(Cout, device=x.device)
    ws = torch.empty(lib.tq_stem_head_bwd_workspace(), dtype=torch.uint8, device=x.device) if workspace else None
    check(lib.tq_head_conv_bwd_ws(_p(dpred_nct), _p(c_out), _p(x), _p(gscale), _p(gshift), _p(weight.contiguous()), _p(g), _p(st),
                                  _p(dw), _p(db), B, T, Cin, Cout, K, _p(ws), 0 if ws is None else ws.numel(), _stream(x.device)), "head bwd")
    return g, st, dw, db
```

Baseline: 347.4.

## Fold GroupNorm finalize into K=1 QKV conv and backward apply kernels

Adds a kernel that recomputes the GroupNorm backward coefficients from partial stats inside each apply block, removing the separate finalize launch. That path is behind an env flag that defaults off. The forward GN-fold path is extended to K=1 convs such as the attention QKV projection, and the forward GN fold is now on by default. Attention's GroupNorm is deferred so it can be folded into the following conv. The cost is redundant per-block reduction of the stats partials and larger LDS use.

```diff
diff --git a/include/tqdne_hip.h b/include/tqdne_hip.h
--- a/include/tqdne_hip.h
+++ b/include/tqdne_hip.h
@@ -91,6 +91,7 @@
 size_t tq_conv1d_wide_lds_bytes(int ktaps, int t_tile, int C_out);
 int tq_conv1d_gn_table_entries(int wide);
 int tq_conv1d_gn_fold_max_cin(int wfmt, int t_tile, int C_out);
+int tq_conv1d_qkv_gn_fold_max_cin(int wfmt, int flags, int C_in, int C_out);
 int tq_colsum_max_channels(void);
 typedef struct TqPackJob {
     const void* src;
@@ -147,6 +148,10 @@
                            const float* coef_c, float* dx, int B, int T, int C_src, int C_total, int c_offset, int accumulate,
                            float* colsum_bc, int bc_stride, float* colsum_c, float* colsum_c2, uint32_t* amax_out,
                            hipStream_t stream);
+int tq_gn_bwd_apply_fold(const float* g, const float* x, const float* r, const float* gstats_partial, const float* mean_rstd,
+                         const float* gamma, float* dgamma, float* dbeta, float* coef_a, float* coef_b, float* coef_c, float* dx,
+                         int B, int T, int C_src, int C_total, int c_offset, int accumulate, float* colsum_bc, int bc_stride,
+                         float* colsum_c, float* colsum_c2, uint32_t* amax_out, hipStream_t stream);
 typedef struct TqGemmJob {
     const float* A;
     const float* B;
diff --git a/tqdne_amd/_lib.py b/tqdne_amd/_lib.py
--- a/tqdne_amd/_lib.py
+++ b/tqdne_amd/_lib.py
@@ -128,6 +128,7 @@
     "tq_conv1d_gn_table_entries": (I, [I]),
     "tq_conv1d_wide_lds_bytes": (SZ, [I, I, I]),
     "tq_conv1d_gn_fold_max_cin": (I, [I, I, I]),
+    "tq_conv1d_qkv_gn_fold_max_cin": (I, [I, I, I, I]),
     "tq_colsum_max_channels": (I, []),
     "tq_conv1d_fwd": (I, [C.POINTER(TqConvDesc)] + [VP] * 11),
     "tq_conv1d_fwd_skip": (I, [C.POINTER(TqConvDesc)] + [VP] * 13),
@@ -178,6 +179,7 @@
     "tq_gn_bwd_finalize": (I, [VP, VP, VP, I, I, I, VP, VP, VP, VP, VP, VP]),
     "tq_gn_bwd_apply": (I, [VP] * 7 + [I] * 6 + [VP]),
     "tq_gn_bwd_apply_colsum": (I, [VP] * 7 + [I] * 6 + [VP, I, VP, VP, VP, VP]),
+    "tq_gn_bwd_apply_fold": (I, [VP] * 12 + [I] * 6 + [VP, I, VP, VP, VP, VP]),
     "tq_pack_job_blocks": (I, [I, I, I, I]),
     "tq_pack_jobs": (I, [VP, I, I, VP]),
     "tq_gemm_tiles": (I, [I, I]),
diff --git a/tqdne_amd/csrc/backward.hip b/tqdne_amd/csrc/backward.hip
--- a/tqdne_amd/csrc/backward.hip
+++ b/tqdne_amd/csrc/backward.hip
@@ -1,5 +1,6 @@
 #include <cstdlib>
 #include "common.hpp"
+#include "gn_bwd_fold.hpp"
 #include "ends_wide.hpp"
 #include "../../include/tqdne_hip.h"
 
@@ -599,67 +600,14 @@
     const int b = blockIdx.x;
     const int Cb = C / (int)gridDim.y;
     const int c0 = (int)blockIdx.y * Cb;
-    int nsub = Cb <= 128 ? (int)blockDim.x / Cb : 1;
-    if (nsub > nslots) nsub = nslots;
-    double* cs = sh;
-    double* gp = sh + 2 * Cb * nsub;
-    for (int idx = threadIdx.x; idx < Cb * nsub; idx += blockDim.x) {
-        const int c = idx % Cb, sub = idx / Cb;
-        const float* pp = gst + ((size_t)b * nslots * C + c0 + c) * 2;
-        double s1 = 0.0, s2 = 0.0;
-        int s = sub;
-        for (; s + 3 * nsub < nslots; s += 4 * nsub) {
-            const float2 v0 = *reinterpret_cast<const float2*>(pp + (size_t)s * C * 2);
-            const float2 v1 = *reinterpret_cast<const float2*>(pp + (size_t)(s + nsub) * C * 2);
-            const float2 v2 = *reinterpret_cast<const float2*>(pp + (size_t)(s + 2 * nsub) * C * 2);
-            const float2 v3 = *reinterpret_cast<const float2*>(pp + (size_t)(s + 3 * nsub) * C * 2);
-            s1 += ((double)v0.x + (double)v1.x) + ((double)v2.x + (double)v3.x);
-            s2 += ((double)v0.y + (double)v1.y) + ((double)v2.y + (double)v3.y);
-        }
-        for (; s < nslots; s += nsub) {
-            const float2 v = *reinterpret_cast<const float2*>(pp + (size_t)s * C * 2);
-            s1 += (double)v.x; s2 += (double)v.y;
-        }
-        cs[2 * idx] = s1; cs[2 * idx + 1] = s2;
-    }
-    __syncthreads();
-    if (nsub > 1) {
-        double t1 = 0.0, t2 = 0.0;
-        const int c = threadIdx.x;
-        if (c < Cb)
-            for (int sub = 0; sub < nsub; ++sub) { t1 += cs[2 * (sub * Cb + c)]; t2 += cs[2 * (sub * Cb + c) + 1]; }
-        __syncthreads();
-        if (c < Cb) { cs[2 * c] = t1; cs[2 * c + 1] = t2; }
-        __syncthreads();
-    }
-    const int G = C / GN_GROUPS;
-    const int ngrp = Cb / G, g0 = c0 / G;
-    if ((int)threadIdx.x < ngrp) {
-        const int gl = threadIdx.x, g = g0 + gl;
-        const double mean = (double)mr[((size_t)b * GN_GROUPS + g) * 2], rstd = (double)mr[((size_t)b * GN_GROUPS + g) * 2 + 1];
-        double p1 = 0.0, p2 = 0.0;
-        for (int j = 0; j < G; ++j) {
-            const int cl = gl * G + j;
-            const double gm = (double)gamma[c0 + cl];
-            p1 += gm * cs[2 * cl];
-            p2 += gm * (cs[2 * cl + 1] - mean * cs[2 * cl]);
-        }
-        p2 *= rstd;
-        const double n = (double)G * (double)T;
-        gp[2 * gl] = -rstd * rstd * p2 / n;
-        gp[2 * gl + 1] = rstd * rstd * p2 * mean / n - rstd * p1 / n;
-    }
-    __syncthreads();
-    for (int cl = threadIdx.x; cl < Cb; cl += blockDim.x) {
-        const int c = c0 + cl;
-        const int g = c / G, gl = g - g0;
-        const float mean = mr[((size_t)b * GN_GROUPS + g) * 2], rstd = mr[((size_t)b * GN_GROUPS + g) * 2 + 1];
-        cA[(size_t)b * C + c] = rstd * gamma[c];
-        cB[(size_t)b * C + c] = (float)gp[2 * gl];
-        cC[(size_t)b * C + c] = (float)gp[2 * gl + 1];
-        atomicAdd(dgamma + c, (float)((double)rstd * (cs[2 * cl + 1] - (double)mean * cs[2 * cl])));
-        atomicAdd(dbeta + c, (float)cs[2 * cl]);
-    }
+    gn_bwd_fold_channels(sh, b, c0, Cb, gn_bwd_nsub(C, nslots), gst, mr, gamma, C, T, nslots,
+                         [&](int c, float a, float bx, float cc, float dg, float db) __attribute__((always_inline)) {
+                             cA[(size_t)b * C + c] = a;
+                             cB[(size_t)b * C + c] = bx;
+                             cC[(size_t)b * C + c] = cc;
+                             atomicAdd(dgamma + c, dg);
+                             atomicAdd(dbeta + c, db);
+                         });
 }
 
 __global__ void gn_bwd_apply_kernel(const float* __restrict__ g, const float* __restrict__ x, const float* __restrict__ r,
@@ -818,6 +766,108 @@
         }
     }
     colsum_finish<NT>(red, a, mx, active, c4n, nrow, c4, tr, Cs, b, 1.0f, out_bc, bc_stride, out_c, out_c2, amax_out);
+}
+
+template <int NT, bool CS>
+__global__ __launch_bounds__(NT) void gn_bwd_apply_fold_kernel(const float* __restrict__ g, const float* __restrict__ x,
+                                                                const float* __restrict__ r, const float* __restrict__ gst,
+                                                                const float* __restrict__ mr, const float* __restrict__ gamma,
+                                                                float* __restrict__ dgamma, float* __restrict__ dbeta,
+                                                                float* __restrict__ oA, float* __restrict__ oB, float* __restrict__ oC,
+                                                                float* __restrict__ dx, int T, int Cs, int Ctot, int coff, int accum,
+                                                                float* __restrict__ out_bc, int bc_stride, float* __restrict__ out_c,
+                                                                float* __restrict__ out_c2, unsigned* __restrict__ amax_out, int rpw) {
+    extern __shared__ __attribute__((aligned(16))) float lds_f[];
+    float* tab = lds_f;
+    float* red = lds_f + 3 * Cs;
+    const int nsl = (T + rpw - 1) / rpw;
+    const int slot = blockIdx.x % nsl, b = blockIdx.x / nsl;
+    const int c4n = Cs >> 2;
+    const int nrow = NT / c4n > 0 ? NT / c4n : 1;
+    const int c4 = threadIdx.x % c4n, tr = threadIdx.x / c4n;
+    const bool active = tr < nrow && threadIdx.x < nrow * c4n;
+    const int nvalid = min(rpw, T - slot * rpw);
+    const size_t base = ((size_t)b * T + (size_t)slot * rpw) * Cs + 4 * (active ? c4 : 0);
+    const float4 z4 = make_float4(0.f, 0.f, 0.f, 0.f);
+    float4 gv0[4], xv0[4], rv0[4], ov0[4];
+#pragma unroll
+    for (int q = 0; q < 4; ++q) {
+        const int row = min(tr + q * nrow, nvalid - 1);
+        const size_t o = base + (size_t)row * Cs;
+        gv0[q] = *reinterpret_cast<const float4*>(g + o);
+        xv0[q] = *reinterpret_cast<const float4*>(x + o);
+        rv0[q] = r ? *reinterpret_cast<const float4*>(r + o) : z4;
+        ov0[q] = accum ? *reinterpret_cast<const float4*>(dx + o) : z4;
+    }
+    {
+        const int G = Ctot / GN_GROUPS;
+        const int ca = (coff / G) * G, cb = ((coff + Cs + G - 1) / G) * G;
+        const int nslots = (T + STAT_SLOT - 1) / STAT_SLOT;
+        const bool first = slot == 0;
+        gn_bwd_fold_channels(reinterpret_cast<double*>(red), b, ca, cb - ca, gn_bwd_nsub(Ctot, nslots), gst, mr, gamma, Ctot, T, nslots,
+                             [&](int c, float a, float bx, float cc, float dg, float db) __attribute__((always_inline)) {
+                                 if (c < coff || c >= coff + Cs) return;
+                                 tab[c - coff] = a;
+                                 tab[Cs + c - coff] = bx;
+                                 tab[2 * Cs + c - coff] = cc;
+                                 if (first) {
+                                     atomicAdd(dgamma + c, dg);
+                                     atomicAdd(dbeta + c, db);
+                                     if (oA) { oA[(size_t)b * Ctot + c] = a; oB[(size_t)b * Ctot + c] = bx; oC[(size_t)b * Ctot + c] = cc; }
+                                 }
+                             });
+        __syncthreads();
+    }
+    float4 a = z4;
+    float mx = 0.f;
+    if (active) {
+        const float4 ka = *reinterpret_cast<const float4*>(tab + 4 * c4);
+        const float4 kb = *reinterpret_cast<const float4*>(tab + Cs + 4 * c4);
+        const float4 kc = *reinterpret_cast<const float4*>(tab + 2 * Cs + 4 * c4);
+        auto one = [&](const float4& gv, const float4& xv, const float4& rv, const float4& ov) -> float4 __attribute__((always_inline)) {
+            float4 o = make_float4(ka.x * gv.x + kb.x * xv.x + kc.x, ka.y * gv.y + kb.y * xv.y + kc.y,
+                                   ka.z * gv.z + kb.z * xv.z + kc.z, ka.w * gv.w + kb.w * xv.w + kc.w);
+            o.x += rv.x; o.y += rv.y; o.z += rv.z; o.w += rv.w;
+            o.x += ov.x; o.y += ov.y; o.z += ov.z; o.w += ov.w;
+            return o;
+        };
+        int tl = tr;
+        if (tl + 3 * nrow < nvalid) {
+#pragma unroll
+            for (int q = 0; q < 4; ++q) {
+                const float4 o4 = one(gv0[q], xv0[q], rv0[q], ov0[q]);
+                *reinterpret_cast<float4*>(dx + base + (size_t)(tl + q * nrow) * Cs) = o4;
+                if (CS) { a.x += o4.x; a.y += o4.y; a.z += o4.z; a.w += o4.w; mx = amax4(mx, o4); }
+            }
+            tl += 4 * nrow;
+        }
+        for (; tl + 3 * nrow < nvalid; tl += 4 * nrow) {
+            float4 gv[4], xv[4], rv[4], ov[4];
+#pragma unroll
+            for (int q = 0; q < 4; ++q) {
+                const size_t o = base + (size_t)(tl + q * nrow) * Cs;
+                gv[q] = *reinterpret_cast<const float4*>(g + o);
+                xv[q] = *reinterpret_cast<const float4*>(x + o);
+                rv[q] = r ? *reinterpret_cast<const float4*>(r + o) : z4;
+                ov[q] = accum ? *reinterpret_cast<const float4*>(dx + o) : z4;
+            }
+#pragma unroll
+            for (int q = 0; q < 4; ++q) {
+                const float4 o4 = one(gv[q], xv[q], rv[q], ov[q]);
+                *reinterpret_cast<float4*>(dx + base + (size_t)(tl + q * nrow) * Cs) = o4;
+                if (CS) { a.x += o4.x; a.y += o4.y; a.z += o4.z; a.w += o4.w; mx = amax4(mx, o4); }
+            }
+        }
+        for (; tl < nvalid; tl += nrow) {
+            const size_t o = base + (size_t)tl * Cs;
+            const float4 o4 = one(*reinterpret_cast<const float4*>(g + o), *reinterpret_cast<const float4*>(x + o),
+                                  r ? *reinterpret_cast<const float4*>(r + o) : z4, accum ? *reinterpret_cast<const float4*>(dx + o) : z4);
+            *reinterpret_cast<float4*>(dx + o) = o4;
+            if (CS) { a.x += o4.x; a.y += o4.y; a.z += o4.z; a.w += o4.w; mx = amax4(mx, o4); }
+        }
+    }
+    if constexpr (CS)
+        colsum_finish<NT>(red, a, mx, active, c4n, nrow, c4, tr, Cs, b, 1.0f, out_bc, bc_stride, out_c, out_c2, amax_out);
 }
 
 struct CsChunk { int c0, cw; };
@@ -950,9 +1000,7 @@
     const int nslots = (T + STAT_SLOT - 1) / STAT_SLOT;
     const int NP = 4;
     const int Cb = C / NP;
-    int nsub = Cb <= 128 ? 256 / Cb : 1;
-    if (nsub > nslots) nsub = nslots;
-    const size_t sh = (size_t)(2 * Cb * nsub + 2 * GN_GROUPS) * sizeof(double);
+    const size_t sh = gn_bwd_fold_scratch(Cb, gn_bwd_nsub(C, nslots), C) * sizeof(double);
     hipLaunchKernelGGL(gn_bwd_finalize_kernel, dim3(B, NP), dim3(256), sh, stream, gstats, mean_rstd, gamma, C, T, nslots, coef_a,
                        coef_b, coef_c, dgamma, dbeta);
     TQ_CHECK_LAUNCH();
@@ -1038,6 +1086,40 @@
     const size_t sh = (size_t)nrow * c4n * 4 * sizeof(float) + (CS_NT / 64) * sizeof(unsigned);
     hipLaunchKernelGGL(gn_bwd_apply_cs_kernel<CS_NT>, dim3(B * nsl), dim3(CS_NT), sh, stream, g, x, r, coef_a, coef_b, coef_c, dx, T, C_src,
                        C_total, c_offset, accumulate, colsum_bc, bc_stride, colsum_c, colsum_c2, amax_out, tl.rows);
+    TQ_CHECK_LAUNCH();
+    return 0;
+}
+
+constexpr int GN_BWD_FOLD_MAX_CTOT = 2 * CS_CHUNK;
+extern "C" int tq_gn_bwd_apply_fold(const float* g, const float* x, const float* r, const float* gstats_partial, const float* mean_rstd,
+                                    const float* gamma, float* dgamma, float* dbeta, float* coef_a, float* coef_b, float* coef_c,
+                                    float* dx, int B, int T, int C_src, int C_total, int c_offset, int accumulate, float* colsum_bc,
+                                    int bc_stride, float* colsum_c, float* colsum_c2, uint32_t* amax_out, hipStream_t stream) {
+    if (!g || !x || !gstats_partial || !mean_rstd || !gamma || !dgamma || !dbeta || !dx) return TQ_ERR_ARG;
+    if ((coef_a || coef_b || coef_c) && !(coef_a && coef_b && coef_c)) return TQ_ERR_ARG;
+    if (colsum_c2 && !colsum_c) return TQ_ERR_ARG;
+    if (B <= 0 || T <= 0 || C_src <= 0 || C_src % 4 || c_offset < 0 || c_offset % 4 || c_offset + C_src > C_total) return TQ_ERR_SHAPE;
+    if (C_total % GN_GROUPS) return TQ_ERR_SHAPE;
+    if (C_src > CS_CHUNK || C_total > GN_BWD_FOLD_MAX_CTOT) return TQ_ERR_SHAPE;
+    const CsTiling tl = colsum_tiling(B, T);
+    const int nsl = (T + tl.rows - 1) / tl.rows;
+    const int c4n = C_src / 4;
+    const int nrow = CS_NT / c4n > 0 ? CS_NT / c4n : 1;
+    const int G = C_total / GN_GROUPS;
+    const int ca = (c_offset / G) * G, cb = ((c_offset + C_src + G - 1) / G) * G;
+    const int nslots = (T + STAT_SLOT - 1) / STAT_SLOT;
+    const size_t red_bytes = (size_t)nrow * c4n * 4 * sizeof(float) + (CS_NT / 64) * sizeof(unsigned);
+    const size_t fold_bytes = gn_bwd_fold_scratch(cb - ca, gn_bwd_nsub(C_total, nslots), C_total) * sizeof(double);
+    const size_t sh = (size_t)3 * C_src * sizeof(float) + (red_bytes > fold_bytes ? red_bytes : fold_bytes);
+    if (sh > 64 * 1024) return TQ_ERR_SHAPE;
+    if (colsum_bc || colsum_c || amax_out)
+        hipLaunchKernelGGL((gn_bwd_apply_fold_kernel<CS_NT, true>), dim3(B * nsl), dim3(CS_NT), sh, stream, g, x, r, gstats_partial, mean_rstd,
+                           gamma, dgamma, dbeta, coef_a, coef_b, coef_c, dx, T, C_src, C_total, c_offset, accumulate, colsum_bc, bc_stride,
+                           colsum_c, colsum_c2, amax_out, tl.rows);
+    else
+        hipLaunchKernelGGL((gn_bwd_apply_fold_kernel<CS_NT, false>), dim3(B * nsl), dim3(CS_NT), sh, stream, g, x, r, gstats_partial, mean_rstd,
+                           gamma, dgamma, dbeta, coef_a, coef_b, coef_c, dx, T, C_src, C_total, c_offset, accumulate, nullptr, 0, nullptr,
+                           nullptr, nullptr, tl.rows);
     TQ_CHECK_LAUNCH();
     return 0;
 }
diff --git a/tqdne_amd/csrc/conv1d_fwd_wide.hip b/tqdne_amd/csrc/conv1d_fwd_wide.hip
--- a/tqdne_amd/csrc/conv1d_fwd_wide.hip
+++ b/tqdne_amd/csrc/conv1d_fwd_wide.hip
@@ -76,3 +76,13 @@
     }
     return lim / 32 * 32;
 }
+
+extern "C" int tq_conv1d_qkv_gn_fold_max_cin(int wfmt, int flags, int C_in, int C_out) {
+    if (wfmt != TQ_WFMT_F16_MX6 || (flags & TQ_CONV_WIDE_TABLE) || C_in <= 0 || C_in % 64 || C_out <= 0 || C_out % 128) return 0;
+    int lim;
+    if (!(flags & TQ_CONV_CH_TILES) && C_out % 256 == 0 && C_out >= 512 && (C_in == 128 || C_in == 256))
+        lim = ConvLds<1, 1, 0, 8, 1, 2, 1, 2, true, 8, 2, 1024>::FOLD_MAX_CIN;
+    else if (C_out % 256 == 0) lim = ConvLds<1, 1, 0, 8, 1, 2, 1, 2, false, 8, 2, 1024>::FOLD_MAX_CIN;
+    else lim = ConvLds<1, 1, 0, 4, 1, 2, 1, 2, false, 8, 2, 1024>::FOLD_MAX_CIN;
+    return lim / 32 * 32;
+}
diff --git a/tqdne_amd/csrc/conv1d_kernel.hpp b/tqdne_amd/csrc/conv1d_kernel.hpp
--- a/tqdne_amd/csrc/conv1d_kernel.hpp
+++ b/tqdne_amd/csrc/conv1d_kernel.hpp
@@ -591,14 +591,16 @@
 
     static_assert(!(SCH == 2 && ACT >= 1) || C::NTHR >= 256, "one table entry per thread");
     constexpr int GT_N = GTW / 1024;
-    constexpr bool FOLD_LATE = SCH == 2 && ACT >= 1 && !PW && EPI == 0 && (TBW == 8 || TBW == 2);
+    constexpr bool FOLD_LATE = SCH == 2 && ACT >= 1 && !PW && EPI != 1 && (TBW == 8 || TBW == 2);
     const bool fold_late = FOLD_LATE && p.cf_st0 != nullptr;
+    constexpr bool FOLD_PW = SCH == 2 && ACT >= 1 && PW;
+    const bool fold_pw = FOLD_PW && p.cf_st0 != nullptr;
     float4 gt_a = make_float4(0.f, 0.f, 0.f, 0.f), gt_s = gt_a;
     int gt_i = 0;
     if constexpr (SCH == 2 && ACT >= 1) {
         const int n4 = Cin >> 2;
         gt_i = tid < n4 ? tid : n4 - 1;
-        if (!fold_late) {
+        if (!fold_late && !fold_pw) {
             gt_a = reinterpret_cast<const float4*>(p.gscale + (size_t)b * Cin)[gt_i];
             gt_s = reinterpret_cast<const float4*>(p.gshift + (size_t)b * Cin)[gt_i];
         }
@@ -633,7 +635,9 @@
             __syncthreads();
         }
     };
-    if constexpr (PW) gtab_store();
+    if constexpr (PW) {
+        if (!fold_pw) gtab_store();
+    }
     const int npass = PW ? n_ctiles : 1;
     if constexpr (PW) {
         static_assert(!PW || SCH == 2 || C::NIT == C::PRE, "PW stages a chunk in PRE iterations");
@@ -648,6 +652,14 @@
             }
             load_w(0, wa);
             load_w(1, wb);
+            if constexpr (FOLD_PW) {
+                if (fold_pw) {
+                    gn_fold_sample<false, false>(reinterpret_cast<double*>(lds), b, p.cf_st0, p.C0, p.cf_st1, p.C1, p.T_in, p.cf_ns0, p.cf_ns1,
+                                                 p.cf_gamma, p.cf_beta, const_cast<float*>(p.gscale), const_cast<float*>(p.gshift), p.cf_mean_rstd,
+                                                 gtab, gtab + Cin);
+                    __syncthreads();
+                }
+            }
 #pragma unroll
             for (int c = 0; c < 4; ++c) write16(c < nchunks ? c : nchunks - 1, c, tid >> 2, rr2[c]);
             __syncthreads();
@@ -1111,7 +1123,7 @@
     if (GTAB_MAX && a.cf_st0 && a.C0 + a.C1 > 1024) return TQ_ERR_SHAPE;
     if (SCH == 2 && ACT >= 1 && a.C0 + a.C1 > GTW) return TQ_ERR_SHAPE;
     if (a.cf_st0) {
-        constexpr bool built = (TBW == 2 && ACT >= 1 && !PW && EPI == 0) || (SCH == 2 && ACT >= 1 && !PW && EPI == 0 && TBW == 8);
+        constexpr bool built = (TBW == 2 && ACT >= 1 && !PW && EPI == 0) || (SCH == 2 && ACT >= 1 && EPI != 1 && TBW == 8);
         if (!built || (size_t)(2 * (a.C0 + a.C1) + 64) * sizeof(double) > (size_t)(LDS_BYTES - GTAB_MAX)) return TQ_ERR_SHAPE;
     }
     static std::atomic<uint64_t> attr_done{0};
diff --git a/tqdne_amd/csrc/conv1d_mfma.hip b/tqdne_amd/csrc/conv1d_mfma.hip
--- a/tqdne_amd/csrc/conv1d_mfma.hip
+++ b/tqdne_amd/csrc/conv1d_mfma.hip
@@ -106,7 +106,8 @@
     a.cf_st0 = a.cf_st1 = a.cf_gamma = a.cf_beta = nullptr; a.cf_mean_rstd = nullptr; a.cf_ns0 = a.cf_ns1 = 0;
     if (d->gn_fold) {
         const TqGnFold* f = d->gn_fold;
-        if (!(d->flags & TQ_CONV_GN) || kv_planes || (a.t_tile != 32 && d->wfmt != TQ_WFMT_F16_MX6)) return TQ_ERR_SHAPE;
+        if (!(d->flags & TQ_CONV_GN) || (a.t_tile != 32 && d->wfmt != TQ_WFMT_F16_MX6)) return TQ_ERR_SHAPE;
+        if (kv_planes && (d->flags & TQ_CONV_WIDE_TABLE)) return TQ_ERR_SHAPE;
         if (!f->stats0 || !f->gamma || !f->beta || (d->C_in1 > 0 && !f->stats1)) return TQ_ERR_ARG;
         const int s0 = f->slot0 ? f->slot0 : STAT_SLOT, s1 = f->slot1 ? f->slot1 : STAT_SLOT;
         if ((s0 != STAT_SLOT && s0 != 32) || (s1 != STAT_SLOT && s1 != 32)) return TQ_ERR_ARG;
diff --git a/tqdne_amd/csrc/gn_bwd_fold.hpp b/tqdne_amd/csrc/gn_bwd_fold.hpp
--- /dev/null
+++ b/tqdne_amd/csrc/gn_bwd_fold.hpp
@@ -0,0 +1,80 @@
+#pragma once
+#include "common.hpp"
+
+namespace tq {
+
+__host__ __device__ inline int gn_bwd_nsub(int C, int nslots) {
+    const int Cb = C / 4;
+    int nsub = Cb <= 128 ? 256 / Cb : 1;
+    if (nsub > nslots) nsub = nslots;
+    return nsub;
+}
+
+__host__ __device__ inline size_t gn_bwd_fold_scratch(int n, int nsub, int C) {
+    return (size_t)2 * ((size_t)n * nsub + (nsub > 1 ? n : 0) + n / (C / GN_GROUPS));
+}
+
+template <class Emit>
+__device__ __forceinline__ void gn_bwd_fold_channels(double* sh, int b, int ca, int n, int nsub, const float* __restrict__ gst,
+                                                     const float* __restrict__ mr, const float* __restrict__ gamma, int C, int T,
+                                                     int nslots, Emit emit) {
+    const int tid = threadIdx.x, nthr = blockDim.x;
+    double* cs = sh;
+    double* tot = nsub > 1 ? sh + 2 * (size_t)n * nsub : sh;
+    double* gp = tot + 2 * (size_t)n;
+    for (int idx = tid; idx < n * nsub; idx += nthr) {
+        const int c = idx % n, sub = idx / n;
+        const float* pp = gst + ((size_t)b * nslots * C + ca + c) * 2;
+        double s1 = 0.0, s2 = 0.0;
+        int s = sub;
+        for (; s + 3 * nsub < nslots; s += 4 * nsub) {
+            const float2 v0 = *reinterpret_cast<const float2*>(pp + (size_t)s * C * 2);
+            const float2 v1 = *reinterpret_cast<const float2*>(pp + (size_t)(s + nsub) * C * 2);
+            const float2 v2 = *reinterpret_cast<const float2*>(pp + (size_t)(s + 2 * nsub) * C * 2);
+            const float2 v3 = *reinterpret_cast<const float2*>(pp + (size_t)(s + 3 * nsub) * C * 2);
+            s1 += ((double)v0.x + (double)v1.x) + ((double)v2.x + (double)v3.x);
+            s2 += ((double)v0.y + (double)v1.y) + ((double)v2.y + (double)v3.y);
+        }
+        for (; s < nslots; s += nsub) {
+            const float2 v = *reinterpret_cast<const float2*>(pp + (size_t)s * C * 2);
+            s1 += (double)v.x; s2 += (double)v.y;
+        }
+        cs[2 * idx] = s1; cs[2 * idx + 1] = s2;
+    }
+    __syncthreads();
+    if (nsub > 1) {
+        for (int c = tid; c < n; c += nthr) {
+            double t1 = 0.0, t2 = 0.0;
+            for (int sub = 0; sub < nsub; ++sub) { t1 += cs[2 * (sub * n + c)]; t2 += cs[2 * (sub * n + c) + 1]; }
+            tot[2 * c] = t1; tot[2 * c + 1] = t2;
+        }
+        __syncthreads();
+    }
+    const int G = C / GN_GROUPS;
+    const int ngrp = n / G, g0 = ca / G;
+    if (tid < ngrp) {
+        const int gl = tid, g = g0 + gl;
+        const double mean = (double)mr[((size_t)b * GN_GROUPS + g) * 2], rstd = (double)mr[((size_t)b * GN_GROUPS + g) * 2 + 1];
+        double p1 = 0.0, p2 = 0.0;
+        for (int j = 0; j < G; ++j) {
+            const int cl = gl * G + j;
+            const double gm = (double)gamma[ca + cl];
+            p1 += gm * tot[2 * cl];
+            p2 += gm * (tot[2 * cl + 1] - mean * tot[2 * cl]);
+        }
+        p2 *= rstd;
+        const double nn = (double)G * (double)T;
+        gp[2 * gl] = -rstd * rstd * p2 / nn;
+        gp[2 * gl + 1] = rstd * rstd * p2 * mean / nn - rstd * p1 / nn;
+    }
+    __syncthreads();
+    for (int cl = tid; cl < n; cl += nthr) {
+        const int c = ca + cl;
+        const int g = c / G, gl = g - g0;
+        const float mean = mr[((size_t)b * GN_GROUPS + g) * 2], rstd = mr[((size_t)b * GN_GROUPS + g) * 2 + 1];
+        emit(c, rstd * gamma[c], (float)gp[2 * gl], (float)gp[2 * gl + 1],
+             (float)((double)rstd * (tot[2 * cl + 1] - (double)mean * tot[2 * cl])), (float)tot[2 * cl]);
+    }
+}
+
+}
diff --git a/tqdne_amd/engine.py b/tqdne_amd/engine.py
--- a/tqdne_amd/engine.py
+++ b/tqdne_amd/engine.py
@@ -49,7 +49,7 @@
 FUSE_SKIP_CO = 32
 SMALL_TILE_B = 4
 SMALL_TILE_WGS = 64
-GN_FOLD_DEFAULT = os.environ.get("TQDNE_GN_FOLD", "0") == "1"
+GN_FOLD_DEFAULT = os.environ.get("TQDNE_GN_FOLD", "1") != "0"
 CONCURRENT_LANE0 = 8
 
 
@@ -431,11 +431,17 @@
         pend = self._pending_gn
         if pend is not None and gn is not None and pend["key"] == gn[0].data_ptr():
             self._pending_gn = None
-            fold_max = self.lib.tq_conv1d_gn_fold_max_cin(wfmt, 32 if small else 0, site.C_out)
+            k1_gn = site.K == 1 and not silu and stride == 1 and not upsample and skip is None and s1 is None
+            lb = self._launch_bound(T_out)
+            if k1_gn:
+                fold_max = self.lib.tq_conv1d_qkv_gn_fold_max_cin(wfmt, _lib.TQ_CONV_CH_TILES if lb else 0, site.C_in, site.C_out)
+            else:
+                fold_max = self.lib.tq_conv1d_gn_fold_max_cin(wfmt, 32 if small else 0, site.C_out)
             if small and wfmt != _lib.TQ_WFMT_BF16X3:
                 fold_max = min(fold_max, self.lib.tq_conv1d_gn_fold_max_cin(_lib.TQ_WFMT_BF16X3, 32, site.C_out))
             fold_fits = site.C_in <= fold_max
-            fold_default = (GN_FOLD_DEFAULT and not small and k5_act and wfmt == _lib.TQ_WFMT_F16_MX6 and self.scheme == "auto"
+            fold_default = (((GN_FOLD_DEFAULT and k5_act) or (k1_gn and (GN_FOLD_DEFAULT or lb))) and not small
+                            and wfmt == _lib.TQ_WFMT_F16_MX6 and self.scheme == "auto"
                             and getattr(self.m, "_conv_scheme", "auto") == "auto" and fold_fits)
             if fold_default and launch and not self.ckpt:
                 fn, fargs, fname, ffl = pend["fin"][0]
@@ -746,7 +752,7 @@
         return out
 
     def _attention(self, x: Act, ab, name: str) -> Act:
-        g = self._gn([x], ab.norm)
+        g = self._gn([x], ab.norm, defer=not self.ckpt)
         D = ab.channels // ab.num_heads
         hd = D not in (32, 64, 128)
         if hd and not self.lib.tq_attention_head_tile(D):
diff --git a/tqdne_amd/engine_bwd.py b/tqdne_amd/engine_bwd.py
--- a/tqdne_amd/engine_bwd.py
+++ b/tqdne_amd/engine_bwd.py
@@ -3,6 +3,7 @@
 
 import ctypes as C
 import math
+import os
 from typing import Dict, List
 
 import torch
@@ -22,6 +23,8 @@
 BWD_STREAMS = int(__import__("os").environ.get("TQDNE_BWD_STREAMS", "2"))
 
 DGRAD_MX6_C64 = __import__("os").environ.get("TQDNE_DGRAD_MX6_C64", "0") == "1"
+GN_BWD_FOLD = os.environ.get("TQDNE_GN_BWD_FOLD", "0") == "1"
+GN_BWD_FOLD_MAX_SRC, GN_BWD_FOLD_MAX_TOTAL = 1024, 2048
 N_AMAX = 160
 
 
@@ -235,7 +238,11 @@
         lib = self.lib
         amax = self.amax_ptr(dy.data_ptr())
         wr = self._grad_writer.get(dy.data_ptr())
-        if wr is not None and wr[0][0] is lib.tq_gn_bwd_apply:
+        if wr is not None and wr[0][0] is lib.tq_gn_bwd_apply_fold and wr[0][2] == "gn_bwd_apply_fold":
+            op = wr[0]
+            op[1] = op[1][:-5] + [bc, stride, _p(self.g(c1)) if c1 is not None else None, _p(self.g(c2)) if c2 is not None else None, amax]
+            op[2] = "gn_bwd_apply_fold+colsum:" + name
+        elif wr is not None and wr[0][0] is lib.tq_gn_bwd_apply:
             op = wr[0]
             op[0] = lib.tq_gn_bwd_apply_colsum
             op[1] = op[1] + [bc, stride, _p(self.g(c1)) if c1 is not None else None, _p(self.g(c2)) if c2 is not None else None, amax]
@@ -299,7 +306,11 @@
             self._wrote(t_)
         return gst
 
-    def _gn_bwd(self, gst, gn, norm, T, Ctot):
+    def _gn_bwd(self, gst, gn, norm, T, Ctot, widths=None):
+        widths = widths or [Ctot]
+        if (GN_BWD_FOLD and Ctot % 32 == 0 and Ctot <= GN_BWD_FOLD_MAX_TOTAL
+                and all(w % 4 == 0 and w <= GN_BWD_FOLD_MAX_SRC for w in widths)):
+            return dict(gst=gst, mean_rstd=gn[2], norm=norm)
         ca, cb, cc = self._empty(self.B, Ctot), self._empty(self.B, Ctot), self._empty(self.B, Ctot)
         self.ops.append([self.lib.tq_gn_bwd_finalize, [_p(gst), _p(gn[2]), _p(norm.weight), self.B, Ctot, T, _p(ca), _p(cb), _p(cc),
                                                        _p(self.g(norm.weight)), _p(self.g(norm.bias))], "gn_bwd_finalize"])
@@ -307,6 +318,15 @@
 
     def _gn_apply(self, G, act, coef, Ctot, coff, r=None):
         dx = self.grad(act)
+        if isinstance(coef, dict):
+            norm = coef["norm"]
+            self.ops.append([self.lib.tq_gn_bwd_apply_fold, [_p(G), _p(act.buf), _p(r), _p(coef["gst"]), _p(coef["mean_rstd"]), _p(norm.weight),
+                                                             _p(self.g(norm.weight)), _p(self.g(norm.bias)), None, None, None, _p(dx),
+                                                             self.B, act.T, act.C, Ctot, coff, int(act.gw), None, 0, None, None, None],
+                             "gn_bwd_apply_fold"])
+            self._wrote(dx)
+            act.gw = True
+            return
         self.ops.append([self.lib.tq_gn_bwd_apply, [_p(G), _p(act.buf), _p(r), _p(coef[0]), _p(coef[1]), _p(coef[2]), _p(dx), self.B,
                                                     act.T, act.C, Ctot, coff, int(act.gw)], "gn_bwd_apply"])
         self._wrote(dx)
@@ -405,7 +425,7 @@
         Ctot = sum(s.C for s in srcs)
         G1 = [self.scratch("G1_%d" % i, T, s.C) for i, s in enumerate(srcs)]
         gst1 = self._dgrad(rec1, dh1, T, G1, accumulate=False)
-        coef1 = self._gn_bwd(gst1, t["g1"], rb.in_layers[0], T, Ctot)
+        coef1 = self._gn_bwd(gst1, t["g1"], rb.in_layers[0], T, Ctot, widths=[s.C for s in srcs])
         if rec_sk is None:
             self._gn_apply(G1[0], srcs[0], coef1, Ctot, 0, r=dout)
         else:
diff --git a/tqdne_amd/ops.py b/tqdne_amd/ops.py
--- a/tqdne_amd/ops.py
+++ b/tqdne_amd/ops.py
@@ -339,6 +339,20 @@
     return dx, obc, oc
 
 
+def gn_bwd_apply_fold(g, x, gstats, mean_rstd, gamma, dgamma, dbeta, c_total, c_offset=0, r=None, accumulate_into=None, coefs=None,
+                      per_sample=False, total=False, amax=None):
+    lib = _lib.load()
+    B, T, Cs = g.shape
+    dx = accumulate_into if accumulate_into is not None else torch.empty_like(g)
+    obc = torch.zeros(B, Cs, device=g.device) if per_sample else None
+    oc = torch.zeros(Cs, device=g.device) if total else None
+    ca, cb, cc = coefs if coefs is not None else (None, None, None)
+    check(lib.tq_gn_bwd_apply_fold(_p(g), _p(x), _p(r), _p(gstats), _p(mean_rstd), _p(gamma), _p(dgamma), _p(dbeta), _p(ca), _p(cb), _p(cc),
+                                   _p(dx), B, T, Cs, c_total, c_offset, int(accumulate_into is not None), _p(obc), Cs, _p(oc), None,
+                                   _p(amax), _stream(g.device)), "gn_bwd_apply_fold")
+    return dx, obc, oc
+
+
 def zero_stuff(dy, T_in):
     lib = _lib.load()
     B, T_out, Cn = dy.shape
```

Measured after the change: 349.7, median of 6. Within noise of the previous version (+0.7%).
